# Zhongxu-Wang/ArtSpeech

Measured on AMD Instinct MI355X. Metric: mel frames/sec (whole job; per-GPU = value / n_gpus), acoustic-model inference path, batch 32 x 200-frame utterances, higher is better.
Workload: dtype f32 (f16x3 split-operand MFMA, fp32 accumulate)

## Files before the change

artspeech_amd/_lib.py:

```python
import ctypes
import os

import torch

_HERE = os.path.dirname(os.path.abspath(__file__))
LIB_PATH = os.environ.get("AS_LIB_PATH") or os.path.join(_HERE, "lib", "libartspeech_hip.so")
_lib = None

c_p = ctypes.c_void_p
c_i = ctypes.c_int
c_sz = ctypes.c_size_t
c_f = ctypes.c_float

_SIGNATURES = {
    "as_abi_version": (c_i, []),
    "as_device_status": (c_i, [c_i]),
    "as_device_status_raise_for_test": (c_i, [c_i, c_p]),
    "as_set_range_probe": (c_i, [c_i]),
    "as_prof_enable": (c_i, [c_i]),
    "as_prof_collect": (c_i, [c_p, c_p, c_p, c_p, c_i]),
    "as_prof_hint": (c_i, [ctypes.c_double, ctypes.c_double]),
    "as_prof_bracket_overhead": (c_i, [c_p, c_p]),
    "as_prof_mfma_sustained": (c_i, [c_p, c_p, c_p]),
    "as_mas_workspace_bytes": (c_sz, [c_i, c_i, c_i]),
    "as_mas_f32": (c_i, [c_p, c_p, c_p, c_i, c_i, c_i, c_i, c_p, c_p, c_p, c_p, c_sz, c_p]),
    "as_softmax_mas_f32": (c_i, [c_p, c_p, c_p, c_i, c_i, c_i, c_i, c_i, c_p, c_p, c_p, c_p, c_p, c_sz, c_p]),
}

AS_MAX_TAPS = 25
AS_ABI_VERSION = 10
AS_PROSODY_DIM, AS_PROSODY_TRACKS, AS_PROSODY_DUR, AS_PROSODY_GAIN, AS_PROSODY_OFFSET = 25, 12, 0, 1, 13


class ConvGemmArgs(ctypes.Structure):
    _fields_ = [("Wh", ctypes.c_void_p), ("W", ctypes.c_void_p), ("X", ctypes.c_void_p), ("Xh", ctypes.c_void_p), ("Y", ctypes.c_void_p),
                ("Yh", ctypes.c_void_p), ("bias", ctypes.c_void_p), ("res", ctypes.c_void_p), ("meta", ctypes.c_void_p),
                ("ws", ctypes.c_void_p), ("ws_bytes", ctypes.c_size_t),
                ("M", ctypes.c_int32), ("N", ctypes.c_int32), ("K", ctypes.c_int32), ("T", ctypes.c_int32),
                ("Kp", ctypes.c_int32),
                ("ldx", ctypes.c_int32), ("ldy", ctypes.c_int32), ("ldr", ctypes.c_int32),
                ("act", ctypes.c_int32), ("div_sqrt2", ctypes.c_int32), ("in_act", ctypes.c_int32),
                ("transpose_out", ctypes.c_int32), ("yh_lrelu", ctypes.c_int32), ("n_prod", ctypes.c_int32),
                ("dh", ctypes.c_int32 * AS_MAX_TAPS), ("dw", ctypes.c_int32 * AS_MAX_TAPS),
                ("in_slope", ctypes.c_float), ("act_slope", ctypes.c_float), ("acc_scale", ctypes.c_float),
                ("n_groups", ctypes.c_int32), ("group_cols", ctypes.c_int32), ("range_probe", ctypes.c_int32), ("status", ctypes.c_void_p),
                ("Xh2", ctypes.c_void_p), ("K2", ctypes.c_int32), ("src_col", ctypes.c_void_p), ("N_in", ctypes.c_int32), ("ileave_u", ctypes.c_int32),
                ("slab_tr", ctypes.c_int32), ("n_valid", ctypes.c_void_p)]


_SIGNATURES.update({
    "as_make_meta": (c_i, [c_p, c_p, c_i, c_i, c_i, c_p, c_p]),
    "as_conv_gemm_f32": (c_i, [ctypes.POINTER(ConvGemmArgs), c_p]),
    "as_conv_gemm_workspace_bytes": (c_sz, [ctypes.POINTER(ConvGemmArgs)]),
    "as_conv_gemm_multi_f32": (c_i, [ctypes.POINTER(ConvGemmArgs), c_i, c_p]),
    "as_conv_gemm_multi_tile": (c_i, [ctypes.POINTER(ConvGemmArgs), c_i]),
    "as_conv_gemm_multi_workspace_bytes": (c_sz, [ctypes.POINTER(ConvGemmArgs)]),
    "as_conv_gemm_plan": (c_i, [ctypes.POINTER(ConvGemmArgs), ctypes.POINTER(ctypes.c_int32), ctypes.POINTER(ctypes.c_int32),
                                ctypes.POINTER(ctypes.c_int32)]),
    "as_split_f16x2_bytes": (c_sz, [c_i, c_i]),
    "as_split_f16x2_f32": (c_i, [c_p, c_i, c_i, c_i, c_i, c_f, c_p, c_p]),
    "as_prep_weight_f16x2_bytes": (c_sz, [c_i, c_i, c_i, c_i]),
    "as_prep_weight_f16x2_host": (c_i, [c_p, c_i, c_i, c_i, c_i, c_p, c_p]),
    "as_prep_weight_f16x2_sc_bytes": (c_sz, [c_i, c_i, c_i, c_i, c_i]),
    "as_prep_weight_f16x2_sc_host": (c_i, [c_p, c_p, c_i, c_i, c_i, c_i, c_i, c_p, c_p]),
    "as_embed_groups_f32": (c_i, [c_p, c_i, c_p, c_p, c_i, c_i, c_i, c_i, c_f, c_p, c_i, c_p]),
    "as_channel_layernorm_groups_f32": (c_i, [c_p, c_i, c_i, c_i, c_p, c_p, c_p, c_p, c_i, c_f, c_i, c_p, c_i, c_p]),
    "as_channel_layernorm_split_f32": (c_i, [c_p, c_i, c_i, c_i, c_p, c_p, c_p, c_p, c_i, c_f, c_i, c_p, c_p]),
    "as_relpos_attention_groups_f32": (c_i, [c_p, c_i, c_i, c_i, c_i, c_p, c_p, c_p, c_p, c_i, c_p, c_i, c_i, c_p, c_i, c_p]),
    "as_embed_f32": (c_i, [c_p, c_p, c_i, c_i, c_i, c_f, c_p, c_i, c_p]),
    "as_channel_layernorm_f32": (c_i, [c_p, c_i, c_i, c_i, c_p, c_p, c_f, c_i, c_p, c_i, c_p]),
    "as_adain_f32": (c_i, [c_p, c_i, c_i, c_p, c_i, c_p, c_i, c_p, c_i, c_i, c_p, c_p, c_p, c_i, c_p]),
    "as_adain_split_f32": (c_i, [c_p, c_i, c_i, c_p, c_i, c_p, c_i, c_i, c_i, c_p, c_p]),
    "as_linear_rows_f32": (c_i, [c_p, c_i, c_p, c_p, c_i, c_i, c_i, c_p, c_i, c_p]),
    "as_durations_f32": (c_i, [c_p, c_p, c_p, c_i, c_p, c_p, c_p, c_i, c_p]),
    "as_expand_f32": (c_i, [c_p, c_i, c_i, c_p, c_i, c_i, c_p, c_i, c_p]),
    "as_ref_features_f32": (c_i, [c_p, c_i, c_i, c_p, c_p, c_i, c_i, c_p, c_p, c_i, c_p]),
    "as_crop_f32": (c_i, [c_p, c_i, c_p, c_i, c_p, c_i, c_p, c_i, c_i, c_i, c_p]),
    "as_rows_to_images_f32": (c_i, [c_p, c_i, c_p, c_i, c_i, c_p, c_p, c_i, c_i, c_p]),
    "as_stem_pool_image_f32": (c_i, [c_p, c_p, c_p, c_i, c_p, c_p, c_i, c_i, c_p, c_i, c_p, c_i, c_i, c_i, c_i, c_p, c_i, c_p]),
    "as_dwconv_down_f32": (c_i, [c_p, c_i, c_p, c_p, c_i, c_p, c_i, c_p, c_p, c_i, c_p, c_p, c_i, c_i, c_i, c_i, c_i, c_p]),
    "as_frame_signal_f32": (c_i, [c_p, c_p, c_p, c_i, c_i, c_i, c_i, c_p, c_i, c_p]),
    "as_spec_power_f32": (c_i, [c_p, c_i, c_i, c_i, c_p, c_i, c_p]),
    "as_log_norm_f32": (c_i, [c_p, c_i, c_i, c_i, c_f, c_f, c_f, c_p, c_i, c_p]),
    "as_xl_attention_f32": (c_i, [c_p, c_i, c_i, c_i, c_p, c_i, c_p, c_p, c_f, c_p, c_i, c_i, c_p, c_i, c_p]),
    "as_glu_dwconv_bn_swish_f32": (c_i, [c_p, c_i, c_i, c_p, c_i, c_p, c_p, c_p, c_i, c_p, c_i, c_p]),
    "as_lstm_step0_f32": (c_i, [c_p, c_i, c_i, c_i, c_p, c_i, c_p]),
    "as_bn_lrelu_maxpool_rows_f32": (c_i, [c_p, c_i, c_p, c_i, c_i, c_i, c_i, c_p, c_p, c_f, c_p, c_i, c_i, c_i, c_p]),
    "as_avgpool_down_f32": (c_i, [c_p, c_i, c_p, c_p, c_i, c_p, c_i, c_p, c_p, c_i, c_i, c_p, c_i, c_i, c_i, c_i, c_p]),
    "as_im2col_valid_f32": (c_i, [c_p, c_i, c_p, c_p, c_i, c_p, c_i, c_p, c_p, c_i, c_i, c_i, c_i, c_i, c_i, c_i, c_p]),
    "as_dwconv_down_image_f32": (c_i, [c_p, c_i, c_p, c_p, c_i, c_p, c_p, c_i, c_p, c_p, c_i, c_i, c_i, c_i, c_i, c_p, c_i, c_p]),
    "as_avgpool_down_image_f32": (c_i, [c_p, c_i, c_p, c_p, c_i, c_p, c_i, c_p, c_p, c_i, c_i, c_p, c_i, c_i, c_i, c_i, c_p, c_i, c_i, c_p]),
    "as_im2col_valid_image_f32": (c_i, [c_p, c_i, c_p, c_p, c_p, c_p, c_i, c_i, c_i, c_i, c_i, c_p, c_p]),
    "as_mean_pool_f32": (c_i, [c_p, c_i, c_p, c_i, c_i, c_i, c_p, c_i, c_p]),
    "as_relpos_attention_f32": (c_i, [c_p, c_i, c_i, c_i, c_i, c_p, c_p, c_p, c_i, c_i, c_p, c_i, c_p]),
    "as_relpos_attention_image_f32": (c_i, [c_p, c_i, c_p, c_i, c_i, c_i, c_i, c_p, c_p, c_p, c_p, c_i, c_p, c_i, c_i, c_p, c_i, c_p, c_p]),
    "as_relpos_attention_image_lds_bytes": (c_i, [c_i]),
    "as_bilstm_f32": (c_i, [c_p, c_i, c_p, c_i, c_i, c_p]),
    "as_bilstm_cluster_bytes": (ctypes.c_size_t, [c_i, c_i]),
    "as_bilstm_cluster_f32": (c_i, [c_p, c_i, c_p, c_i, c_i, c_i, c_p, ctypes.c_size_t, c_p]),
    "as_interleave_phases_f32": (c_i, [c_p, c_i, c_p, c_i, c_i, c_i, c_p, c_i, c_p]),
    "as_mean3_f32": (c_i, [c_p, c_p, c_p, c_i, c_i, c_i, c_p, c_i, c_p]),
})


class LnArgs(ctypes.Structure):
    _fields_ = [("gamma", c_p), ("beta", c_p), ("gamma2", c_p), ("beta2", c_p), ("n_split", ctypes.c_int32), ("eps", ctypes.c_float),
                ("relu", ctypes.c_int32), ("yh", c_p)]


class AdainArgs(ctypes.Structure):
    _fields_ = [("x", c_p), ("ldx", ctypes.c_int32), ("C", ctypes.c_int32), ("gb", c_p), ("gb_off", c_p), ("ldgb", ctypes.c_int32),
                ("gb_sc", ctypes.c_int32), ("col_off", c_p), ("src_off", c_p), ("U", ctypes.c_int32), ("N", ctypes.c_int32),
                ("lrelu", ctypes.c_int32), ("yh", c_p), ("pool_w", c_p), ("pool_b", c_p), ("x_up", c_p), ("ld_up", ctypes.c_int32),
                ("col_w", c_p)]


class DownArgs(ctypes.Structure):
    _fields_ = [("kind", ctypes.c_int32), ("x", c_p), ("ldx", ctypes.c_int32), ("in_off", c_p), ("in_w", c_p), ("Hin", ctypes.c_int32),
                ("y", c_p), ("ldy", ctypes.c_int32), ("out_off", c_p), ("out_w", c_p), ("Hout", ctypes.c_int32), ("w", c_p), ("bias", c_p),
                ("kh", ctypes.c_int32), ("pool_h", ctypes.c_int32), ("Kp", ctypes.c_int32), ("res", c_p), ("ldr", ctypes.c_int32),
                ("B", ctypes.c_int32), ("C", ctypes.c_int32), ("max_out", ctypes.c_int32), ("lrelu", ctypes.c_int32), ("yh", c_p),
                ("n_out", ctypes.c_int32)]


class ResPairArgs(ctypes.Structure):
    _fields_ = [("x", c_p), ("ldx", ctypes.c_int32), ("y", c_p), ("ldy", ctypes.c_int32), ("w1", c_p), ("w2", c_p), ("b1", c_p), ("b2", c_p),
                ("scale1", ctypes.c_float), ("scale2", ctypes.c_float), ("C", ctypes.c_int32), ("N", ctypes.c_int32), ("k", ctypes.c_int32),
                ("dil", ctypes.c_int32), ("slope", ctypes.c_float), ("col_off", c_p), ("B", ctypes.c_int32), ("max_w", ctypes.c_int32),
                ("add1", c_p), ("add2", c_p), ("ld_add", ctypes.c_int32), ("out_div", ctypes.c_float), ("yh", c_p), ("yh_slope", ctypes.c_float),
                ("x_u", ctypes.c_int32), ("x_bias", c_p)]


class ModelCfg(ctypes.Structure):
    _fields_ = [("hidden_dim", ctypes.c_int32), ("dim_in", ctypes.c_int32), ("style_dim", ctypes.c_int32), ("n_mels", ctypes.c_int32),
                ("n_token", ctypes.c_int32), ("reserved", ctypes.c_int32), ("stats", ctypes.c_float * 24)]


class Batch(ctypes.Structure):
    _fields_ = [("B", ctypes.c_int32), ("tok_lens", ctypes.POINTER(ctypes.c_int32)), ("ref_lens", ctypes.POINTER(ctypes.c_int32)),
                ("frames", ctypes.POINTER(ctypes.c_int32))]


class ForwardIO(ctypes.Structure):
    _fields_ = [("tokens", c_p), ("mel", c_p), ("ld_mel", ctypes.c_int32), ("f0_raw", c_p), ("ema_raw", c_p), ("ld_ema", ctypes.c_int32),
                ("forced_dur", c_p), ("mel_out", c_p), ("ld_out", ctypes.c_int32), ("duration", c_p), ("dur_i", c_p), ("frame_off", c_p),
                ("style", c_p), ("feat12", c_p), ("ld_feat", ctypes.c_int32), ("t_en", c_p), ("a_en", c_p), ("ld_en", ctypes.c_int32),
                ("F0", c_p), ("N", c_p), ("EMA", c_p), ("ld_pred", ctypes.c_int32), ("frame_cap", ctypes.c_int32), ("segs", c_p),
                ("voices", c_p), ("ld_voice", ctypes.c_int32), ("n_voices", ctypes.c_int32), ("voice_idx", c_p),
                ("prosody", c_p), ("ld_prosody", ctypes.c_int32)]


class HostIO(ctypes.Structure):
    _fields_ = [("tokens", c_p), ("mel", c_p), ("ld_mel", ctypes.c_int32), ("f0_raw", c_p), ("ema_raw", c_p), ("ld_ema", ctypes.c_int32),
                ("forced_dur", c_p), ("mel_out", c_p), ("ld_out", ctypes.c_int32), ("frame_cap", ctypes.c_int32), ("frame_off", c_p),
                ("voices", c_p), ("ld_voice", ctypes.c_int32), ("n_voices", ctypes.c_int32), ("voice_idx", c_p),
                ("prosody", c_p), ("ld_prosody", ctypes.c_int32)]


class TokenProsody(ctypes.Structure):
    _fields_ = [("rows", c_p), ("ld", ctypes.c_int32), ("smooth", ctypes.c_int32)]


(AS_MOD_FORWARD_A, AS_MOD_FORWARD_B, AS_MOD_ENCODER, AS_MOD_STYLE, AS_MOD_DURATION, AS_MOD_ARTS, AS_MOD_DECODER, AS_MOD_FORWARD_B_CAP,
 AS_MOD_VOICE, AS_MOD_FORWARD_A_VOICE) = range(10)
_pB, _pIO = ctypes.POINTER(Batch), ctypes.POINTER(ForwardIO)
_SIGNATURES.update({
    "as_adain_image_f32": (c_i, [ctypes.POINTER(AdainArgs), c_p]),
    "as_conv_gemm_multi_post_f32": (c_i, [ctypes.POINTER(ConvGemmArgs), ctypes.POINTER(AdainArgs), ctypes.POINTER(ctypes.c_int32),
                                          ctypes.POINTER(LnArgs), c_i, c_p]),
    "as_down_multi_f32": (c_i, [ctypes.POINTER(DownArgs), c_i, c_p]),
    "as_down_strip_rule": (c_i, [c_i, c_i, c_i, c_i, c_i, ctypes.POINTER(ctypes.c_int32), ctypes.POINTER(ctypes.c_int32)]),
    "as_respair_f32": (c_i, [ctypes.POINTER(ResPairArgs), c_p]),
    "as_xl_attention_image_f32": (c_i, [c_p, c_i, c_p, c_p, c_i, c_i, c_i, ctypes.c_float, c_p, c_i, c_i, c_p, c_i, c_p, c_p]),
    "as_mean3_image_f32": (c_i, [c_p, c_p, c_p, c_i, c_i, c_i, ctypes.c_float, c_p, c_p]),
    "as_conv_post_f32": (c_i, [c_p, c_i, c_i, c_i, c_p, c_p, c_i, ctypes.c_float, c_i, c_p, c_p, c_p]),
    "as_rows_image_f32": (c_i, [c_p, c_i, c_i, c_i, c_p, c_p]),
    "as_project_cols_f32": (c_i, [c_p, c_i, c_i, c_i, c_p, c_p, c_i, c_p, c_i, c_p]),
    "as_pointwise_small_f32": (c_i, [c_p, c_i, c_i, c_i, c_p, c_p, c_i, c_p, c_i, c_p, c_p, c_i, c_p, c_p]),
    "as_model_create": (c_i, [c_p, c_sz, ctypes.POINTER(ModelCfg), ctypes.POINTER(c_p)]),
    "as_model_destroy": (c_i, [c_p]),
    "as_plan_create": (c_i, [c_p, ctypes.POINTER(c_p)]),
    "as_plan_destroy": (c_i, [c_p]),
    "as_plan_set_serial": (c_i, [c_p, c_i]),
    "as_plan_set_merge": (c_i, [c_p, c_i]),
    "as_plan_set_timing": (c_i, [c_p, c_i]),
    "as_plan_set_operand_mode": (c_i, [c_p, c_i]),
    "as_plan_set_token_prosody": (c_i, [c_p, ctypes.POINTER(TokenProsody)]),
    "as_plan_phase_ms": (c_i, [c_p, ctypes.POINTER(ctypes.c_float), c_i]),
    "as_plan_set_layout_cap": (c_i, [c_p, c_i]),
    "as_plan_layout_flushes": (c_i, [c_p]),
    "as_plan_layout_count": (c_i, [c_p]),
    "as_plan_reset_layouts": (c_i, [c_p]),
    "as_bilstm_cluster_test_hooks": (c_i, [c_i, c_i]),
    "as_module_workspace_bytes": (c_sz, [c_p, c_p, c_i, _pB]),
    "as_encoder_forward": (c_i, [c_p, c_p, c_i, _pB, c_p, c_p, c_i, c_p, c_sz, c_p]),
    "as_style_forward": (c_i, [c_p, c_p, _pB, c_p, c_i, c_p, c_p, c_i, c_p, c_i, c_p, c_p, c_sz, c_p]),
    "as_duration_forward": (c_i, [c_p, c_p, _pB, c_p, c_p, c_i, c_p, c_p, c_sz, c_p]),
    "as_voice_dim": (c_i, [c_p]),
    "as_voice_forward": (c_i, [c_p, c_p, _pB, c_p, c_i, c_p, c_p, c_i, c_p, c_i, c_p, c_sz, c_p]),
    "as_arts_forward": (c_i, [c_p, c_p, _pB, c_p, c_i, c_p, c_p, c_p, c_p, c_i, c_p, c_sz, c_p]),
    "as_decoder_forward": (c_i, [c_p, c_p, _pB, c_p, c_i, c_p, c_p, c_p, c_p, c_i, c_p, c_i, c_p, c_sz, c_p]),
    "as_forward_test_begin": (c_i, [c_p, c_p, _pB, _pIO, c_p, c_sz, c_p]),
    "as_forward_test_finish": (c_i, [c_p, c_p, _pB, _pIO, c_p, c_sz, c_p, c_sz, c_p]),
    "as_forward_test": (c_i, [c_p, c_p, _pB, _pIO, c_p, c_sz, c_p, c_sz, ctypes.POINTER(ctypes.c_int32), c_p]),
    "as_lanes_create": (c_i, [c_p, c_i, ctypes.POINTER(c_p)]),
    "as_lanes_destroy": (c_i, [c_p]),
    "as_lanes_count": (c_i, [c_p]),
    "as_lanes_next": (c_i, [c_p]),
    "as_lanes_stream": (c_p, [c_p, c_i]),
    "as_lanes_submit": (c_i, [c_p, _pB, _pIO, ctypes.POINTER(ctypes.c_int32), ctypes.POINTER(ctypes.c_int32)]),
    "as_lanes_wait": (c_i, [c_p, c_i]),
    "as_lanes_set_coalesce": (c_i, [c_p, c_i]),
    "as_lanes_set_debug": (c_i, [c_p, c_i]),
    "as_lanes_submit_host": (c_i, [c_p, _pB, ctypes.POINTER(HostIO), ctypes.POINTER(ctypes.c_int32)]),
    "as_model_get_cfg": (c_i, [c_p, c_p]),
    "as_lanes_flush": (c_i, [c_p]),
    "as_lanes_merged_calls": (ctypes.c_int64, [c_p, c_i]),
    "as_lanes_set_graph_cap": (c_i, [c_p, c_i]),
    "as_lanes_set_layout_cap": (c_i, [c_p, c_i]),
    "as_lanes_reserve": (c_i, [c_p, c_sz, c_sz]),
    "as_lanes_stats": (c_i, [c_p, c_i, ctypes.POINTER(ctypes.c_int64)]),
})



class VocoderCfg(ctypes.Structure):
    _fields_ = [("num_mels", ctypes.c_int32), ("upsample_initial_channel", ctypes.c_int32), ("n_stages", ctypes.c_int32),
                ("upsample_rates", ctypes.c_int32 * 8), ("upsample_kernel_sizes", ctypes.c_int32 * 8), ("n_stacks", ctypes.c_int32),
                ("resblock_kernel_sizes", ctypes.c_int32 * 4), ("resblock_dilations", (ctypes.c_int32 * 4) * 4), ("n_dilations", ctypes.c_int32)]


class VocoderIO(ctypes.Structure):
    _fields_ = [("mel", c_p), ("ld_mel", ctypes.c_int32), ("wav", c_p), ("pcm", c_p)]


class VocoderCap(ctypes.Structure):
    _fields_ = [("off", c_p), ("mult", ctypes.c_int32), ("cap", ctypes.c_int32), ("max_len", ctypes.c_int32), ("sample_off", c_p)]


_pI32 = ctypes.POINTER(ctypes.c_int32)
_SIGNATURES.update({
    "as_vocoder_cap_workspace_bytes": (c_sz, [c_p, c_p, c_i, c_i, c_i]),
    "as_vocoder_forward_cap": (c_i, [c_p, c_p, c_i, ctypes.POINTER(VocoderCap), ctypes.POINTER(VocoderIO), c_p, c_sz, c_p]),
    "as_vocoder_cap_geometry": (c_i, [c_p, c_i, c_i, c_i, c_i, c_i, _pI32, c_p, c_p, c_p, c_p]),
    "as_split_f16x2_cap_f32": (c_i, [c_p, c_i, c_i, c_i, c_p, c_i, ctypes.c_float, c_p, c_p]),
    "as_mean3_cap_f32": (c_i, [c_p, c_p, c_p, c_i, c_i, c_i, c_p, c_p, c_i, c_p]),
    "as_mean3_image_cap_f32": (c_i, [c_p, c_p, c_p, c_i, c_i, c_i, c_p, ctypes.c_float, c_p, c_p]),
    "as_interleave_phases_cap_f32": (c_i, [c_p, c_i, c_p, c_i, c_i, c_i, c_p, c_p, c_i, c_p]),
    "as_conv_post_pcm_cap_f32": (c_i, [c_p, c_i, c_i, c_i, c_p, c_p, c_i, ctypes.c_float, c_i, c_p, c_p, c_p, c_p, c_p]),
    "as_conv_post_pcm_f32": (c_i, [c_p, c_i, c_i, c_i, c_p, c_p, c_i, ctypes.c_float, c_i, c_p, c_p, c_p, c_p]),
# ... 183 lines not shown
```

artspeech_amd/csrc/conv_gemm_h3.hip:

```cpp
#include "conv_gemm.h"
#include <cstring>
#include <type_traits>

typedef __attribute__((address_space(3))) void lds_void;

template <int I, int N, typename F>
static __device__ __forceinline__ void h3_for(F&& f)
{
    if constexpr (I < N) {
        f(std::integral_constant<int, I>{});
        h3_for<I + 1, N>(f);
    }
}

template <int WM, int WN, int WK, int KT, int NS, int NP, int TM = 2>
struct H3Cfg {
    static constexpr int QP = NP == 1 ? 2 : 4;
    static constexpr int BM = 32 * TM * WM, BN = 64 * WN;
    static constexpr int KBS = WK * KT;
    static constexpr int A_BLK = QP * BM * 16, B_BLK = QP * BN * 16;
    static constexpr int A_ST = KBS * A_BLK;
    static constexpr int STAGE = KBS * (A_BLK + B_BLK);
    static constexpr int RED = (WK - 1) * WM * WN * 32 * TM * 64 * 4;
    static constexpr int LDS = NS * STAGE > RED ? NS * STAGE : RED;
// ... 399 lines not shown
}

int as_split_f16x2_launch(const float* x, int ldx, int K, int N, int lrelu, float slope, uint16_t* xh, hipStream_t stream,
                          const int32_t* n_valid)
{
    if ((double)K * ldx * 4.0 >= 2147483648.0) return AS_EINVAL;
    hipLaunchKernelGGL(split_f16x2_kernel, dim3(as_cdiv(N + 1, 1024), 2 * as_kbx(K)), dim3(256), 0, stream, x, ldx, K, N, n_valid, lrelu, slope,
                       reinterpret_cast<u32x4_t*>(xh));
    AS_CHECK_LAUNCH();
    return AS_OK;
}

extern "C" int as_split_f16x2_f32(const float* x, int ldx, int K, int N, int in_act, float in_slope, uint16_t* xh, as_stream_t stream)
{
    return as_split_f16x2_cap_f32(x, ldx, K, N, nullptr, in_act, in_slope, xh, stream);
}

extern "C" int as_split_f16x2_cap_f32(const float* x, int ldx, int K, int N, const int32_t* n_valid, int in_act, float in_slope, uint16_t* xh,
                                      as_stream_t stream)
{
    if (!x || !xh || K <= 0 || N < 0 || ldx < N || (in_act != 0 && in_act != 2) || !(fabsf(in_slope) <= 3.0e38f)) return AS_EINVAL;
    if ((reinterpret_cast<uintptr_t>(xh) & 15) != 0) return AS_EINVAL;
    if (N == 0) return AS_OK;
    AsProfScope prof__(AS_CLS_OTHER, 0, 8.0 * K * (double)N, (hipStream_t)stream);
    return as_split_f16x2_launch(x, ldx, K, N, in_act == 2, in_slope, xh, (hipStream_t)stream, n_valid);
}

extern "C" size_t as_prep_weight_f16x2_sc_bytes(int G, int Cout, int Cin, int T, int Cin2)
{
    if (G <= 0 || Cout <= 0 || Cin <= 0 || T <= 0 || Cin2 < 0) return 0;
    return (size_t)G * ((size_t)T * as_kbx(Cin) + (Cin2 ? as_kbx(Cin2) : 0)) * 4 * (size_t)Cout * 16;
}
extern "C" size_t as_prep_weight_f16x2_bytes(int G, int Cout, int Cin, int T) { return as_prep_weight_f16x2_sc_bytes(G, Cout, Cin, T, 0); }

extern "C" int as_prep_weight_f16x2_sc_host(const float* w, const float* w2, int G, int Cout, int Cin, int T, int Cin2, uint16_t* wh,
                                            float* scale_out)
{
    if (!w || !wh || !scale_out || G <= 0 || Cout <= 0 || Cin <= 0 || T <= 0 || Cin2 < 0 || ((Cin2 > 0) != (w2 != nullptr))) return AS_EINVAL;
    const size_t n = (size_t)G * Cout * Cin * T, n2 = (size_t)G * Cout * Cin2;
    float mx = 0.f;
    for (size_t i = 0; i < n + n2; ++i) {
        const float x = i < n ? w[i] : w2[i - n];
        const float v = x < 0 ? -x : x;
        if (!(v <= 3.0e38f)) return AS_EINVAL;
        mx = v > mx ? v : mx;
    }
    int e = 0;
    float scale = 1.0f;
    if (mx > 0.f) {
        frexpf(mx, &e);
        scale = ldexpf(1.0f, 14 - e);
    }
    const int KBx = as_kbx(Cin), KBx2 = Cin2 ? as_kbx(Cin2) : 0;
    const size_t blocks = (size_t)T * KBx + KBx2;
    const size_t total = as_prep_weight_f16x2_sc_bytes(G, Cout, Cin, T, Cin2) / 2;
    for (size_t i = 0; i < total; ++i) wh[i] = 0;
    auto put = [&](size_t block, int k, int m, float x) {
        const _Float16 h = (_Float16)x;
        const _Float16 l = (_Float16)(x - (float)h);
        const int kh = (k >> 3) & 1, e8 = k & 7;
        const size_t base = block * 4 * (size_t)Cout * 8;
        uint16_t hb, lb;
        __builtin_memcpy(&hb, &h, 2);
        __builtin_memcpy(&lb, &l, 2);
        wh[base + ((size_t)(0 * 2 + kh) * Cout + m) * 8 + e8] = hb;
        wh[base + ((size_t)(1 * 2 + kh) * Cout + m) * 8 + e8] = lb;
    };
    for (int g = 0; g < G; ++g)
        for (int m = 0; m < Cout; ++m) {
            for (int k = 0; k < Cin; ++k)
                for (int t = 0; t < T; ++t) put((size_t)g * blocks + (size_t)t * KBx + (k >> 4), k, m, w[(((size_t)g * Cout + m) * Cin + k) * T + t] * scale);
            for (int k = 0; k < Cin2; ++k) put((size_t)g * blocks + (size_t)T * KBx + (k >> 4), k, m, w2[((size_t)g * Cout + m) * Cin2 + k] * scale);
        }
    *scale_out = scale;
    return AS_OK;
}
extern "C" int as_prep_weight_f16x2_host(const float* w, int G, int Cout, int Cin, int T, uint16_t* wh, float* scale_out)
{
    return as_prep_weight_f16x2_sc_host(w, nullptr, G, Cout, Cin, T, 0, wh, scale_out);
}

template <bool UP>
__global__ void __launch_bounds__(256)
adain_image_kernel(const AsAdainArgs a)
{
    const int lane = threadIdx.x & 63, wave = __builtin_amdgcn_readfirstlane(threadIdx.x >> 6);
    const int kb = blockIdx.x * 2 + (wave >> 1), kh = wave & 1, u = blockIdx.y;
    const int C = a.C;
    if (kb >= as_kbx(C)) return;
    const size_t NX = operand_image::rows(a.N);
    u32x4_t* xs = reinterpret_cast<u32x4_t*>(a.yh);
    const size_t plane = operand_image::row_of(kb, 0, kh, 0, NX);
    if (u == 0 && lane == 0) oi_zero_column(xs, plane, a.N, NX);
    const int o0 = a.col_off[u], L = a.col_w ? a.col_w[u] : a.col_off[u + 1] - o0;
    if (L <= 0) return;
    const int s0 = a.src_off ? a.src_off[u] : o0;
    const size_t gbase = a.gb_off ? (size_t)a.gb_off[u] : (size_t)u * a.ldgb;
    const int c0 = kb * 16 + kh * 8;
    float g1[8], bt[8], w0[8], w1[8], w2[8], pb[8];
#pragma unroll
    for (int r = 0; r < 8; ++r) {
        const int c = c0 + r < C ? c0 + r : C - 1;
        g1[r] = 1.0f + a.gb[gbase + (size_t)c * a.gb_sc];
        bt[r] = a.gb[gbase + (size_t)(C + c) * a.gb_sc];
        if (UP) { w0[r] = a.pool_w[c * 3 + 0]; w1[r] = a.pool_w[c * 3 + 1]; w2[r] = a.pool_w[c * 3 + 2]; pb[r] = a.pool_b[c]; }
    }
    const float* xr0 = a.x + s0;
    const size_t at0 = plane + (UP ? 2 * (size_t)o0 : (size_t)o0);
    float mean[8], rstd[8];
    auto resident = [&](auto rv_) {
        constexpr int RV = decltype(rv_)::value;
        float v[8][RV];
#pragma unroll
        for (int r = 0; r < 8; ++r) {
            const float* xr = xr0 + (size_t)(c0 + r < C ? c0 + r : C - 1) * a.ldx;
#pragma unroll
            for (int j = 0; j < RV; ++j) v[r][j] = xr[min(lane + 64 * j, L - 1)];
        }
#pragma unroll
        for (int r = 0; r < 8; ++r) {
            float sacc = 0.f;
#pragma unroll
            for (int j = 0; j < RV; ++j)
                if (lane + 64 * j < L) sacc += v[r][j];
            mean[r] = as_wave_sum(sacc) / (float)L;
        }
#pragma unroll
        for (int r = 0; r < 8; ++r) {
            float vacc = 0.f;
#pragma unroll
            for (int j = 0; j < RV; ++j)
                if (lane + 64 * j < L) { const float d = __fsub_rn(v[r][j], mean[r]); vacc = __fmaf_rn(d, d, vacc); }
            rstd[r] = 1.0f / sqrtf(as_wave_sum(vacc) / (float)L + 1e-5f);
        }
        if (UP && a.x_up) {
#pragma unroll
            for (int r = 0; r < 8; ++r) {
                if (c0 + r >= C) continue;
                float* ur = a.x_up + (size_t)(c0 + r) * a.ld_up + 2 * o0;
#pragma unroll
                for (int j = 0; j < RV; ++j) {
                    const int i = lane + 64 * j;
                    if (i < L) { ur[2 * i] = v[r][j]; ur[2 * i + 1] = v[r][j]; }
                }
            }
        }
#pragma unroll
        for (int r = 0; r < 8; ++r)
#pragma unroll
            for (int j = 0; j < RV; ++j)
                v[r][j] = (c0 + r < C && lane + 64 * j < L) ? as_adain_val(v[r][j], mean[r], rstd[r], g1[r], bt[r], a.lrelu) : 0.f;
#pragma unroll
        for (int j = 0; j < RV; ++j) {
            const int i = lane + 64 * j;
            if (64 * j >= L) break;
            if (!UP) {
                float t[8];
#pragma unroll
                for (int r = 0; r < 8; ++r) t[r] = v[r][j];
                u32x4_t h, l;
                split2(t, h, l);
                if (i < L) oi_store(xs, at0 + i, NX, h, l);
            } else {
                float e0[8], e1[8];
#pragma unroll
                for (int r = 0; r < 8; ++r) {
                    const float dn = __shfl_down(v[r][j], 1);
                    const float wr = j + 1 < RV ? __shfl(v[r][j + 1 < RV ? j + 1 : j], 0) : 0.f;
                    const float an = i + 1 < L ? (lane == 63 ? wr : dn) : 0.f;
                    float o0v, o1v;
                    as_convt_pair(v[r][j], an, w0[r], w1[r], w2[r], pb[r], &o0v, &o1v);
                    e0[r] = c0 + r < C ? o0v : 0.f;
                    e1[r] = c0 + r < C ? o1v : 0.f;
                }
                u32x4_t h, l, h2, l2;
                split2(e0, h, l);
                split2(e1, h2, l2);
                if (i < L) {
                    oi_store(xs, at0 + 2 * i, NX, h, l);
                    oi_store(xs, at0 + 2 * i + 1, NX, h2, l2);
                }
            }
        }
    };
    if (L <= 256) { resident(std::integral_constant<int, 4>{}); return; }
    if (L <= 512) { resident(std::integral_constant<int, 8>{}); return; }
    {
        size_t rowoff[8];
// ... 5 lines not shown
        int i = lane;
        for (; i + 192 < L; i += 256) {
            float t[4][8];
#pragma unroll
            for (int q = 0; q < 4; ++q)
#pragma unroll
                for (int r = 0; r < 8; ++r) t[q][r] = xr0[rowoff[r] + i + 64 * q];
#pragma unroll
            for (int q = 0; q < 4; ++q)
#pragma unroll
                for (int r = 0; r < 8; ++r) acc[r] += t[q][r];
        }
        for (; i < L; i += 64)
#pragma unroll
            for (int r = 0; r < 8; ++r) acc[r] += xr0[rowoff[r] + i];
#pragma unroll
        for (int r = 0; r < 8; ++r) { mean[r] = as_wave_sum(acc[r]) / (float)L; acc[r] = 0.f; }
        i = lane;
        for (; i + 192 < L; i += 256) {
            float t[4][8];
#pragma unroll
            for (int q = 0; q < 4; ++q)
#pragma unroll
                for (int r = 0; r < 8; ++r) t[q][r] = xr0[rowoff[r] + i + 64 * q];
#pragma unroll
            for (int q = 0; q < 4; ++q)
#pragma unroll
                for (int r = 0; r < 8; ++r) { const float d = __fsub_rn(t[q][r], mean[r]); acc[r] = __fmaf_rn(d, d, acc[r]); }
        }
        for (; i < L; i += 64)
#pragma unroll
            for (int r = 0; r < 8; ++r) { const float d = __fsub_rn(xr0[rowoff[r] + i], mean[r]); acc[r] = __fmaf_rn(d, d, acc[r]); }
#pragma unroll
        for (int r = 0; r < 8; ++r) rstd[r] = 1.0f / sqrtf(as_wave_sum(acc[r]) / (float)L + 1e-5f);
    }
    for (int i0 = lane; i0 < L; i0 += 128) {
        float xi[2][8], xn[2][8];
#pragma unroll
        for (int q = 0; q < 2; ++q) {
            const int i = min(i0 + 64 * q, L - 1);
#pragma unroll
            for (int r = 0; r < 8; ++r) {
                const float* xr = xr0 + (size_t)(c0 + r < C ? c0 + r : C - 1) * a.ldx;
                xi[q][r] = xr[i];
                if (UP) xn[q][r] = xr[min(i + 1, L - 1)];
            }
        }
#pragma unroll
        for (int q = 0; q < 2; ++q) {
            const int i = i0 + 64 * q;
            if (i >= L) break;
            float a0[8], a1[8];
#pragma unroll
            for (int r = 0; r < 8; ++r) {
                const bool ok = c0 + r < C;
                a0[r] = ok ? as_adain_val(xi[q][r], mean[r], rstd[r], g1[r], bt[r], a.lrelu) : 0.f;
                a1[r] = (UP && ok && i + 1 < L) ? as_adain_val(xn[q][r], mean[r], rstd[r], g1[r], bt[r], a.lrelu) : 0.f;
                if (UP && a.x_up && ok) {
                    float* ur = a.x_up + (size_t)(c0 + r) * a.ld_up + 2 * o0 + 2 * i;
                    ur[0] = xi[q][r];
                    ur[1] = xi[q][r];
                }
            }
            u32x4_t h, l;
            if (!UP) {
                split2(a0, h, l);
                oi_store(xs, at0 + i, NX, h, l);
            } else {
                float e0[8], e1[8];
#pragma unroll
                for (int r = 0; r < 8; ++r) {
                    as_convt_pair(a0[r], a1[r], w0[r], w1[r], w2[r], pb[r], &e0[r], &e1[r]);
                    if (c0 + r >= C) { e0[r] = 0.f; e1[r] = 0.f; }
                }
                split2(e0, h, l);
                oi_store(xs, at0 + 2 * i, NX, h, l);
                split2(e1, h, l);
                oi_store(xs, at0 + 2 * i + 1, NX, h, l);
            }
        }
    }
}

extern "C" int as_adain_image_f32(const AsAdainArgs* args_host, as_stream_t stream)
{
    if (!args_host) return AS_EINVAL;
    const AsAdainArgs& a = *args_host;
    if (!a.x || !a.gb || !a.col_off || !a.yh || a.C <= 0 || a.U <= 0 || a.N < 0 || a.gb_sc <= 0 || (!a.gb_off && a.ldgb <= 0)) return AS_EINVAL;
    if ((a.pool_w == nullptr) != (a.pool_b == nullptr) || (a.x_up && !a.pool_w)) return AS_EINVAL;
    if ((reinterpret_cast<uintptr_t>(a.yh) & 15) != 0) return AS_EINVAL;
    if (a.N == 0) return AS_OK;
    AsProfScope prof__(AS_CLS_ADAIN, 0, 8.0 * a.C * (double)a.N, (hipStream_t)stream);
    if (a.pool_w) hipLaunchKernelGGL(adain_image_kernel<true>, dim3(as_kbx(a.C) / 2, a.U), dim3(256), 0, (hipStream_t)stream, a);
    else hipLaunchKernelGGL(adain_image_kernel<false>, dim3(as_kbx(a.C) / 2, a.U), dim3(256), 0, (hipStream_t)stream, a);
    AS_CHECK_LAUNCH();
    return AS_OK;
}

extern "C" int as_adain_split_f32(const float* x, int ldx, int C, const float* gamma_beta, int ldgb, const int32_t* col_off, int B,
                                  int N, int lrelu, uint16_t* xs, as_stream_t stream)
{
    if (!x || !gamma_beta || !col_off || !xs || C <= 0 || B <= 0 || N < 0 || ldgb < 2 * C) return AS_EINVAL;
    AsAdainArgs a = {};
    a.x = x; a.ldx = ldx; a.C = C; a.gb = gamma_beta; a.ldgb = ldgb; a.gb_sc = 1; a.col_off = col_off; a.U = B; a.N = N; a.lrelu = lrelu; a.yh = xs;
    return as_adain_image_f32(&a, stream);
}

__global__ void __launch_bounds__(256)
rows_image_kernel(const float* __restrict__ x, int ldx, int K, int B, u32x4_t* __restrict__ xh)
{
    const int i = blockIdx.x * 256 + threadIdx.x;
    const int groups = 2 * as_kbx(K);
    if (i >= groups * (B + 1)) return;
    const int g = i / (B + 1), b = i % (B + 1);
    float t[8];
#pragma unroll
    for (int r = 0; r < 8; ++r) t[r] = (b < B && g * 8 + r < K) ? x[(size_t)b * ldx + g * 8 + r] : 0.f;
    u32x4_t h, l;
    split2(t, h, l);
    const size_t NX = operand_image::rows(B);
    oi_store(xh, operand_image::row(g, 0, b, NX), NX, h, l);
}

extern "C" int as_rows_image_f32(const float* x, int ldx, int K, int B, uint16_t* xh, as_stream_t stream)
{
    if (!x || !xh || K <= 0 || B <= 0 || ldx < K || (reinterpret_cast<uintptr_t>(xh) & 15) != 0) return AS_EINVAL;
    AsProfScope prof__(AS_CLS_OTHER, 0, 8.0 * K * (double)B, (hipStream_t)stream);
    hipLaunchKernelGGL(rows_image_kernel, dim3(as_cdiv((long)2 * as_kbx(K) * (B + 1), 256)), dim3(256), 0, (hipStream_t)stream, x, ldx, K, B,
                       reinterpret_cast<u32x4_t*>(xh));
    AS_CHECK_LAUNCH();
    return AS_OK;
}

#define LNS_COLS 32
#define LNS_PARTS 32
#define LNS_MAXG 4
__global__ void __launch_bounds__(1024)
channel_ln_split_kernel(const float* __restrict__ x, int ldx, int C, int N, const float* __restrict__ gamma1,
                        const float* __restrict__ beta1, const float* __restrict__ gamma2, const float* __restrict__ beta2, int n_split,
                        float eps, int relu, u32x4_t* __restrict__ xs, int KBx)
{
    __shared__ float red[LNS_PARTS][LNS_COLS + 1];
    const int col = threadIdx.x % LNS_COLS, part = threadIdx.x / LNS_COLS;
    const int j = blockIdx.x * LNS_COLS + col;
    const bool ok = j < N;
    const int grp = gamma2 ? j / n_split : 0;
    const float* gamma = gamma1 + (ptrdiff_t)grp * (gamma2 - gamma1);
    const float* beta = beta1 + (ptrdiff_t)grp * (beta2 - beta1);
    const int ngroups = 2 * KBx;
    float v[LNS_MAXG][8];
    float s = 0.f;
#pragma unroll
    for (int i = 0; i < LNS_MAXG; ++i)
#pragma unroll
        for (int r = 0; r < 8; ++r) {
            const int c = 8 * (part + i * LNS_PARTS) + r;
            v[i][r] = (ok && c < C) ? x[(size_t)c * ldx + j] : 0.f;
            s += v[i][r];
        }
    red[part][col] = s;
    __syncthreads();
    float tot = 0.f;
#pragma unroll
    for (int q = 0; q < LNS_PARTS; ++q) tot += red[q][col];
    const float mean = tot / (float)C;
    __syncthreads();
    float q2 = 0.f;
#pragma unroll
    for (int i = 0; i < LNS_MAXG; ++i)
#pragma unroll
        for (int r = 0; r < 8; ++r) {
            const int c = 8 * (part + i * LNS_PARTS) + r;
            const float d = __fsub_rn(v[i][r], mean);
            if (c < C) q2 = __fmaf_rn(d, d, q2);
        }
    red[part][col] = q2;
    __syncthreads();
    tot = 0.f;
#pragma unroll
// ... 48 lines not shown
```

artspeech_amd/csrc/elementwise.hip:

```cpp
#include "common.h"
#include <algorithm>
#include <cstring>
#include "artspeech_hip.h"
#include "conv_gemm.h"
#include "down_strips.h"
#include <cstdint>
#include <type_traits>
#define AS_FILE_CLS AS_CLS_OTHER

static __device__ __forceinline__ float lrelu02(float v) { return v > 0.f ? v : 0.2f * v; }

__global__ void make_meta_kernel(const int* __restrict__ widths, const int* __restrict__ col_off, int B, int H,
                                 unsigned long long* __restrict__ meta, unsigned* __restrict__ status)
{
    const int b = blockIdx.y;
    const int W = widths[b];
    const int base = col_off[b];
    if (W > AS_META_MAX_W) {
        if (blockIdx.x == 0 && threadIdx.x == 0) as_status_raise(status, AS_STATUS_BAD_LAYOUT);
        return;
    }
    for (int i = blockIdx.x * blockDim.x + threadIdx.x; i < H * W; i += gridDim.x * blockDim.x) {
        const unsigned long long h = i / W, w = i - (i / W) * W;
        meta[base + i] = AS_META_PACK(h, w, H, W);
    }
}

extern "C" int as_make_meta(const int32_t* widths, const int32_t* col_off, int B, int H, int n_cols_max,
                            uint64_t* meta, as_stream_t stream)
{
    if (!widths || !col_off || !meta || B < 0 || H <= 0 || H > AS_META_MAX_H) return AS_EINVAL;
    if (B == 0) return AS_OK;
    const int gx = n_cols_max > 0 ? as_cdiv(as_cdiv(n_cols_max, B > 0 ? B : 1), 256) : 1;
    AsProfScope prof__(AS_FILE_CLS, 0, 0, (hipStream_t)stream);
    hipLaunchKernelGGL(make_meta_kernel, dim3(gx < 1 ? 1 : (gx > 64 ? 64 : gx), B), dim3(256), 0, (hipStream_t)stream,
                       widths, col_off, B, H, reinterpret_cast<unsigned long long*>(meta), as_status_words_device());
    AS_CHECK_LAUNCH();
    return AS_OK;
}

__global__ void embed_kernel(const int* __restrict__ tok, int n_tok, const float* __restrict__ emb, const float* __restrict__ emb2,
                             int n_split, int C, int N, int V, float scale, float* __restrict__ y, int ldy, unsigned* __restrict__ status)
{
    const int j = blockIdx.x * blockDim.x + threadIdx.x;
    const int c = blockIdx.y;
    if (j >= N) return;
    const int g = emb2 ? j / n_split : 0;
    const int src = j - g * n_split;
    int t = src < n_tok ? tok[src] : 0;
    if ((t < 0 || t >= V) && c == 0) as_status_raise(status, AS_STATUS_BAD_TOKEN);
    t = t < 0 ? 0 : (t >= V ? V - 1 : t);
    const float* e = emb + (ptrdiff_t)g * (emb2 - emb);
    y[(size_t)c * ldy + j] = e[(size_t)t * C + c] * scale;
}

extern "C" int as_embed_groups_f32(const int32_t* tokens, int n_tok, const float* emb, const float* emb2, int n_split, int C, int N, int V,
                                   float scale, float* y, int ldy, as_stream_t stream)
{
    if (!tokens || !emb || !y || C <= 0 || N < 0 || V <= 0 || ldy < N || n_tok < 0 || n_tok > N) return AS_EINVAL;
    if ((emb2 && n_split <= 0) || (n_tok < N && (!emb2 || n_split < n_tok))) return AS_EINVAL;
    if (N == 0) return AS_OK;
    AsProfScope prof__(AS_FILE_CLS, 0, 0, (hipStream_t)stream);
    hipLaunchKernelGGL(embed_kernel, dim3(as_cdiv(N, 64), C), dim3(64), 0, (hipStream_t)stream, tokens, n_tok, emb, emb2, n_split, C, N, V,
                       scale, y, ldy, as_status_words_device());
    AS_CHECK_LAUNCH();
    return AS_OK;
}

extern "C" int as_embed_f32(const int32_t* tokens, const float* emb, int C, int N, int V, float scale, float* y,
                            int ldy, as_stream_t stream)
{
    return as_embed_groups_f32(tokens, N, emb, nullptr, 0, C, N, V, scale, y, ldy, stream);
}

#define LN_COLS 32
#define LN_PARTS 32
#define LN_MAXV 16
__global__ void __launch_bounds__(1024)
channel_ln_kernel(const float* __restrict__ x, int ldx, int C, int N, const float* __restrict__ gamma1,
                  const float* __restrict__ beta1, const float* __restrict__ gamma2, const float* __restrict__ beta2, int n_split,
                  float eps, int relu, float* __restrict__ y, int ldy)
{
    __shared__ float red[LN_PARTS][LN_COLS + 1];
    const int col = threadIdx.x % LN_COLS, part = threadIdx.x / LN_COLS;
    const int j = blockIdx.x * LN_COLS + col;
    const bool ok = j < N;
    const int grp = gamma2 ? j / n_split : 0;
    const float* gamma = gamma1 + (ptrdiff_t)grp * (gamma2 - gamma1);
    const float* beta = beta1 + (ptrdiff_t)grp * (beta2 - beta1);
    float v[LN_MAXV];
    float s = 0.f;
#pragma unroll
    for (int i = 0; i < LN_MAXV; ++i) {
        const int c = part + i * LN_PARTS;
        v[i] = (ok && c < C) ? x[(size_t)c * ldx + j] : 0.f;
        s += v[i];
    }
    for (int c = part + LN_MAXV * LN_PARTS; c < C; c += LN_PARTS) s += ok ? x[(size_t)c * ldx + j] : 0.f;
    red[part][col] = s;
    __syncthreads();
    float tot = 0.f;
#pragma unroll
    for (int q = 0; q < LN_PARTS; ++q) tot += red[q][col];
    const float mean = tot / (float)C;
    __syncthreads();
    float q2 = 0.f;
#pragma unroll
    for (int i = 0; i < LN_MAXV; ++i) {
        const int c = part + i * LN_PARTS;
        const float d = v[i] - mean;
        if (c < C) q2 += d * d;
    }
    for (int c = part + LN_MAXV * LN_PARTS; c < C; c += LN_PARTS) {
        const float d = (ok ? x[(size_t)c * ldx + j] : 0.f) - mean;
        q2 += d * d;
    }
    red[part][col] = q2;
    __syncthreads();
    tot = 0.f;
#pragma unroll
    for (int q = 0; q < LN_PARTS; ++q) tot += red[q][col];
    const float rs = 1.0f / sqrtf(tot / (float)C + eps);
    if (!ok) return;
#pragma unroll
    for (int i = 0; i < LN_MAXV; ++i) {
        const int c = part + i * LN_PARTS;
        if (c < C) {
            float o = (v[i] - mean) * rs * gamma[c] + beta[c];
            if (relu) o = o < 0.f ? 0.f : o;
            y[(size_t)c * ldy + j] = o;
        }
    }
    for (int c = part + LN_MAXV * LN_PARTS; c < C; c += LN_PARTS) {
        float o = (x[(size_t)c * ldx + j] - mean) * rs * gamma[c] + beta[c];
        if (relu) o = o < 0.f ? 0.f : o;
        y[(size_t)c * ldy + j] = o;
    }
}

extern "C" int as_channel_layernorm_groups_f32(const float* x, int ldx, int C, int N, const float* gamma, const float* beta,
                                               const float* gamma2, const float* beta2, int n_split, float eps, int relu, float* y,
                                               int ldy, as_stream_t stream)
{
    if (!x || !y || !gamma || !beta || C <= 0 || N < 0 || ldx < N || ldy < N || ((gamma2 == nullptr) != (beta2 == nullptr)) ||
        (gamma2 && n_split <= 0))
        return AS_EINVAL;
    if (N == 0) return AS_OK;
    AsProfScope prof__(AS_CLS_LN, 8.0 * C * N, 8.0 * C * N, (hipStream_t)stream);
    hipLaunchKernelGGL(channel_ln_kernel, dim3(as_cdiv(N, LN_COLS)), dim3(1024), 0, (hipStream_t)stream, x, ldx, C, N, gamma,
// ... 300 lines not shown
            else h = mid - 1;
        }
        ub = l;
    }
    int local = 0;
    for (int i = lo; i < hi; ++i) {
        int d;
        if (forced) d = forced[i];
        else {
            float v = dur_f[i];
            if (pros) {
                while (ub + 1 < B && tok_off[ub + 1] <= i) ++ub;
                v = v * pros[(size_t)ub * ldr + AS_PROSODY_DUR];
            }
            const bool fin = fabsf(v) <= 3.0e38f;
            if (!fin) as_status_raise(status, AS_STATUS_F16_RANGE);
            const float r = fin ? rintf(v) : 1.f;
            d = (int)(r < 1.f ? 1.f : fminf(r, 16384.f));
        }
        dur_i[i] = d;
        local += d;
    }
    sums[t] = local;
    __syncthreads();
    for (int off = 1; off < 1024; off <<= 1) {
        const int v = t >= off ? sums[t - off] : 0;
        __syncthreads();
        sums[t] += v;
        __syncthreads();
    }
    int f = sums[t] - local;
    if (t == 0) frame_off[B] = sums[1023];
    int b = 0;
    if (lo < hi || ntok == 0) {
        for (b = 0; b < B; ++b) {
            const int first = tok_off[b];
            if (first >= lo && first < hi) {
                int fb = f;
                for (int i = lo; i < first; ++i) fb += dur_i[i];
                frame_off[b] = fb;
            }
        }
    }
    if (t == 0)
        for (b = 0; b < B; ++b)
            if (tok_off[b] >= ntok) frame_off[b] = sums[1023];
    if (!tok_of_frame) return;
    for (int i = lo; i < hi; ++i) {
        const int d = dur_i[i];
        for (int r = 0; r < d; ++r, ++f)
            if (f < max_frames) tok_of_frame[f] = i;
    }
}

int as_durations_prosody_launch(const float* dur_f32, const int32_t* forced_dur, const int32_t* tok_off, int B, const float* pros, int ld_pros,
                                int32_t* dur_i32, int32_t* frame_off, int32_t* tok_of_frame, int max_frames, hipStream_t stream)
{
    if ((!dur_f32 && !forced_dur) || !tok_off || !dur_i32 || !frame_off || B < 0 || B > 1024) return AS_EINVAL;
    if (pros && (forced_dur || B < 1 || ld_pros < AS_PROSODY_DIM)) return AS_EINVAL;
    AsProfScope prof__(AS_FILE_CLS, 0, 0, stream);
    hipLaunchKernelGGL(durations_kernel, dim3(1), dim3(1024), 0, stream, dur_f32, forced_dur, tok_off, B,
                       dur_i32, frame_off, tok_of_frame, max_frames, as_status_words_device(), pros, ld_pros);
    AS_CHECK_LAUNCH();
    return AS_OK;
}

extern "C" int as_durations_f32(const float* dur_f32, const int32_t* forced_dur, const int32_t* tok_off, int B,
                                int32_t* dur_i32, int32_t* frame_off, int32_t* tok_of_frame, int max_frames,
                                as_stream_t stream)
{
    return as_durations_prosody_launch(dur_f32, forced_dur, tok_off, B, nullptr, 0, dur_i32, frame_off, tok_of_frame, max_frames,
                                       (hipStream_t)stream);
}

__global__ void expand_kernel(const float* __restrict__ x, int ldx, int C, const int* __restrict__ tok_of_frame,
                              int n_frames, int rep, float* __restrict__ y, int ldy)
{
    const int j = blockIdx.x * blockDim.x + threadIdx.x;
    const int c = blockIdx.y;
    if (j >= n_frames * rep) return;
    y[(size_t)c * ldy + j] = x[(size_t)c * ldx + tok_of_frame[j / rep]];
}

extern "C" int as_expand_f32(const float* x, int ldx, int C, const int32_t* tok_of_frame, int n_frames, int repeat,
                             float* y, int ldy, as_stream_t stream)
{
    if (!x || !y || !tok_of_frame || C <= 0 || n_frames < 0 || repeat < 1 || ldy < n_frames * repeat) return AS_EINVAL;
    if (n_frames == 0) return AS_OK;
    AsProfScope prof__(AS_FILE_CLS, 0, 0, (hipStream_t)stream);
    hipLaunchKernelGGL(expand_kernel, dim3(as_cdiv((long)n_frames * repeat, 256), C), dim3(256), 0, (hipStream_t)stream,
                       x, ldx, C, tok_of_frame, n_frames, repeat, y, ldy);
    AS_CHECK_LAUNCH();
    return AS_OK;
}

__global__ void __launch_bounds__(256)
ref_features_kernel(const float* __restrict__ mel, int ldm, int n_mels, const float* __restrict__ f0_raw,
                    const float* __restrict__ ema_raw, int lde, int N, const float* __restrict__ stats,
                    float* __restrict__ feat, int ldf)
{
    __shared__ float part[8][32];
    const int col = threadIdx.x & 31, sl = threadIdx.x >> 5;
    const int j = blockIdx.x * 32 + col;
    const int jc = j < N ? j : N - 1;
    constexpr int RMAX = 16;
    float v[RMAX];
#pragma unroll
    for (int r = 0; r < RMAX; ++r) {
        const int m = sl + 8 * r;
        v[r] = mel[(size_t)(m < n_mels ? m : 0) * ldm + jc];
    }
    float ss = 0.f;
#pragma unroll
    for (int r = 0; r < RMAX; ++r) {
        if (sl + 8 * r < n_mels) {
            const float e = expf(v[r] * 4.0f + -4.0f);
            ss += e * e;
        }
    }
    for (int m = sl + 8 * RMAX; m < n_mels; m += 8) {
        const float e = expf(mel[(size_t)m * ldm + jc] * 4.0f + -4.0f);
        ss += e * e;
    }
    part[sl][col] = ss;
    __syncthreads();
    if (j >= N) return;
    if (sl == 0) {
        float tot = 0.f;
#pragma unroll
        for (int q = 0; q < 8; ++q) tot += part[q][col];
        feat[j] = (logf(sqrtf(tot)) - stats[0]) / stats[1];
    } else if (sl == 1) {
        feat[(size_t)ldf + j] = (f0_raw[j] - stats[2]) / stats[3];
    } else {
        for (int c = sl - 2; c < 10; c += 6) feat[(size_t)(2 + c) * ldf + j] = (ema_raw[(size_t)c * lde + j] - stats[4 + c]) / stats[14 + c];
    }
}

extern "C" int as_ref_features_f32(const float* mel, int ldm, int n_mels, const float* f0_raw, const float* ema_raw,
                                   int lde, int N, const float* stats24, float* feat, int ldf, as_stream_t stream)
{
    if (!mel || !f0_raw || !ema_raw || !stats24 || !feat || N < 0 || n_mels <= 0 || ldm < N || lde < N || ldf < N) return AS_EINVAL;
    if (N == 0) return AS_OK;
    AsProfScope prof__(AS_FILE_CLS, 0, 0, (hipStream_t)stream);
    hipLaunchKernelGGL(ref_features_kernel, dim3(as_cdiv(N, 32)), dim3(256), 0, (hipStream_t)stream, mel, ldm, n_mels,
                       f0_raw, ema_raw, lde, N, stats24, feat, ldf);
    AS_CHECK_LAUNCH();
    return AS_OK;
}

__global__ void crop_kernel(const float* __restrict__ src, int lds, const int* __restrict__ src_off, int start,
                            float* __restrict__ dst, int ldd, const int* __restrict__ dst_off, int C)
{
    const int b = blockIdx.y, c = blockIdx.z;
    const int L = dst_off[b + 1] - dst_off[b];
    for (int i = blockIdx.x * blockDim.x + threadIdx.x; i < L; i += gridDim.x * blockDim.x)
        dst[(size_t)c * ldd + dst_off[b] + i] = src[(size_t)c * lds + src_off[b] + start + i];
}

extern "C" int as_crop_f32(const float* src, int lds, const int32_t* src_off, int start, float* dst, int ldd,
                           const int32_t* dst_off, int B, int C, int max_len, as_stream_t stream)
{
    if (!src || !dst || !src_off || !dst_off || B < 0 || C <= 0) return AS_EINVAL;
    if (B == 0 || max_len <= 0) return AS_OK;
    AsProfScope prof__(AS_FILE_CLS, 0, 0, (hipStream_t)stream);
    hipLaunchKernelGGL(crop_kernel, dim3(as_cdiv(max_len, 256), B, C), dim3(256), 0, (hipStream_t)stream, src, lds,
                       src_off, start, dst, ldd, dst_off, C);
    AS_CHECK_LAUNCH();
    return AS_OK;
}

__global__ void rows_to_images_kernel(const float* __restrict__ src, int lds, const int* __restrict__ src_off, int start,
                                      float* __restrict__ dst, const int* __restrict__ img_off, int H)
{
    const int b = blockIdx.y, h = blockIdx.z;
    const int Wb = (img_off[b + 1] - img_off[b]) / H;
    for (int i = blockIdx.x * blockDim.x + threadIdx.x; i < Wb; i += gridDim.x * blockDim.x)
        dst[(size_t)img_off[b] + (size_t)h * Wb + i] = src[(size_t)h * lds + src_off[b] + start + i];
}

extern "C" int as_rows_to_images_f32(const float* src, int lds, const int32_t* src_off, int start, int H, float* dst,
                                     const int32_t* img_off, int B, int max_w, as_stream_t stream)
{
    if (!src || !dst || !src_off || !img_off || B < 0 || H <= 0) return AS_EINVAL;
    if (B == 0 || max_w <= 0) return AS_OK;
    AsProfScope prof__(AS_FILE_CLS, 0, 0, (hipStream_t)stream);
    hipLaunchKernelGGL(rows_to_images_kernel, dim3(as_cdiv(max_w, 256), B, H), dim3(256), 0, (hipStream_t)stream, src, lds,
                       src_off, start, dst, img_off, H);
    AS_CHECK_LAUNCH();
    return AS_OK;
}

__global__ void bn_lrelu_maxpool_rows_kernel(const float* __restrict__ x, int ldx, const int* __restrict__ tok_off, int H, int k,
                                             const float* __restrict__ scale, const float* __restrict__ shift, float slope,
                                             float* __restrict__ y, int ldy, int to_channels)
{
    const int b = blockIdx.y, c = blockIdx.z;
    const int t0 = tok_off[b], Wb = tok_off[b + 1] - t0, Hout = H / k;
    const float* xr = x + (size_t)c * ldx + (size_t)H * t0;
    const float sc = scale[c], sh = shift[c];
    for (int i = blockIdx.x * blockDim.x + threadIdx.x; i < Hout * Wb; i += gridDim.x * blockDim.x) {
        const int ho = i / Wb, w = i - ho * Wb;
        float m = -INFINITY;
        for (int r = 0; r < k; ++r) {
            float v = xr[(size_t)(ho * k + r) * Wb + w] * sc + sh;
            v = v > 0.f ? v : slope * v;
            m = fmaxf(m, v);
        }
        if (to_channels) y[(size_t)(c * Hout + ho) * ldy + t0 + w] = m;
        else y[(size_t)c * ldy + (size_t)Hout * t0 + i] = m;
    }
}

extern "C" int as_bn_lrelu_maxpool_rows_f32(const float* x, int ldx, const int32_t* tok_off, int B, int C, int H, int k,
                                            const float* scale, const float* shift, float slope, float* y, int ldy,
                                            int to_channels, int total_frames, as_stream_t stream)
{
    if (!x || !y || !tok_off || !scale || !shift || B < 0 || C <= 0 || H <= 0 || k <= 0 || k > H) return AS_EINVAL;
    if (B == 0 || total_frames <= 0) return AS_OK;
    AsProfScope prof__(AS_FILE_CLS, 0, 4.0 * C * (double)total_frames * (H + H / k), (hipStream_t)stream);
    const int per_utt = as_cdiv((long)(H / k) * total_frames, B);
    int gx = as_cdiv(per_utt, 256);
    gx = gx < 1 ? 1 : gx > 64 ? 64 : gx;
    hipLaunchKernelGGL(bn_lrelu_maxpool_rows_kernel, dim3(gx, B, C), dim3(256), 0, (hipStream_t)stream, x, ldx, tok_off, H, k, scale,
                       shift, slope, y, ldy, to_channels);
    AS_CHECK_LAUNCH();
    return AS_OK;
}

typedef float f32x2u __attribute__((ext_vector_type(2), aligned(4)));

struct DownWalk {
    int i, ho, wo, Wo, dq, dr, end, last_row;
    __device__ __forceinline__ DownWalk(int r0, int r1, int Wo_) : Wo(Wo_)
    {
        const int q = (int)threadIdx.x / Wo;
        ho = r0 + q; wo = (int)threadIdx.x - q * Wo; i = r0 * Wo + (int)threadIdx.x;
        end = r1 * Wo; last_row = r1 - 1;
        dq = 256 / Wo; dr = 256 - dq * Wo;
    }
    __device__ __forceinline__ void step()
    {
        i += 256; ho += dq; wo += dr;
        if (wo >= Wo) { wo -= Wo; ++ho; }
    }
    __device__ __forceinline__ bool live() const { return i < end; }
    __device__ __forceinline__ int row() const { return live() ? ho : last_row; }
    __device__ __forceinline__ int col() const { return live() ? wo : Wo - 1; }
    __device__ __forceinline__ int trips(int r0) const
    {
        const int first = r0 * Wo + (__builtin_amdgcn_readfirstlane((int)threadIdx.x) & ~63);
        return max(0, (end - first + 255) >> 8);
    }
};

static __device__ __forceinline__ void down_zero_column(u32x4_t* __restrict__ yh, size_t plane, size_t NX, int Nout, int b, int strip)
{
    if (yh && b == 0 && strip == 0 && threadIdx.x < 2) oi_zero_column(yh, plane, (size_t)threadIdx.x, Nout, NX);
}

template <class Pos, class Half, class Where, class Load, class Sums, class Put>
static __device__ __forceinline__ void down_walk_halves(DownWalk& wk, int r0, const Where& where, const Load& load, const Sums& sums, const Put& put)
{
    int n = wk.trips(r0);
    if (n <= 0) return;
    Pos p, pn;
    Half d0, d1;
    where(p);
    pn = p;
    load(d0, p, 0);
    const auto trip = [&](auto last) __attribute__((always_inline)) {
// ... 511 lines not shown
    if (!x || !col || !in_off || !in_w || !out_off || !out_w || K <= 0 || stride <= 0 || B < 0 || C <= 0) return AS_EINVAL;
    if (B == 0 || max_out <= 0) return AS_OK;
    AsProfScope prof__(AS_FILE_CLS, 0, 0, (hipStream_t)stream);
    hipLaunchKernelGGL(im2col_valid_kernel, dim3(C * K * K), dim3(256), 0, (hipStream_t)stream, x, ldx, in_off, in_w, Hin, col,
                       ldc, out_off, out_w, Hout, K, stride, lrelu, B);
    AS_CHECK_LAUNCH();
    return AS_OK;
}

__global__ void __launch_bounds__(256)
im2col_valid_image_kernel(const float* __restrict__ x, int ldx, const int* __restrict__ in_off, const int* __restrict__ in_w,
                          const int* __restrict__ out_off, const int* __restrict__ out_w, int K, int stride, int act, int B, int rows,
                          u32x4_t* __restrict__ yh)
{
    const int g = blockIdx.x;
    const int total = out_off[B];
    const size_t NX = operand_image::rows(total), plane = operand_image::row(g, 0, 0, NX);
    if (threadIdx.x < 2) oi_zero_column(yh, plane, (size_t)threadIdx.x, total, NX);
    for (int j = threadIdx.x; j < total; j += blockDim.x) {
        int b = 0;
        while (b + 1 < B && out_off[b + 1] <= j) ++b;
        const int i = j - out_off[b], Wo = out_w[b], Wi = in_w[b];
        const int ho = i / Wo, wo = i - ho * Wo;
        float t[8];
#pragma unroll
        for (int r = 0; r < 8; ++r) {
            const int ck = g * 8 + r;
            float v = 0.f;
            if (ck < rows) {
                const int c = ck / (K * K), a = (ck / K) % K, d = ck % K;
                v = x[(size_t)c * ldx + in_off[b] + (size_t)(ho * stride + a) * Wi + wo * stride + d];
                if (act) v = lrelu02(v);
            }
            t[r] = v;
        }
        oi_store(yh, plane + j, NX, t);
    }
}

extern "C" int as_im2col_valid_image_f32(const float* x, int ldx, const int32_t* in_off, const int32_t* in_w, const int32_t* out_off,
                                         const int32_t* out_w, int K, int stride, int lrelu, int B, int C, uint16_t* yh, as_stream_t stream)
{
    if (!x || !yh || !in_off || !in_w || !out_off || !out_w || K <= 0 || stride <= 0 || B <= 0 || C <= 0 ||
        (reinterpret_cast<uintptr_t>(yh) & 15) != 0)
        return AS_EINVAL;
    AsProfScope prof__(AS_FILE_CLS, 0, 0, (hipStream_t)stream);
    hipLaunchKernelGGL(im2col_valid_image_kernel, dim3(2 * as_kbx(C * K * K)), dim3(256), 0, (hipStream_t)stream, x, ldx, in_off, in_w, out_off,
                       out_w, K, stride, lrelu, B, C * K * K, reinterpret_cast<u32x4_t*>(yh));
    AS_CHECK_LAUNCH();
    return AS_OK;
}

__global__ void __launch_bounds__(256)
mean_pool_kernel(const float* __restrict__ x, int ldx, const int* __restrict__ col_off, int B, int C, int act,
                 float* __restrict__ y, int ldy)
{
    const int lane = threadIdx.x & 63;
    const int row = blockIdx.x * 4 + (threadIdx.x >> 6);
    if (row >= C * B) return;
    const int c = row / B, b = row - c * B;
    const int o0 = col_off[b], L = col_off[b + 1] - o0;
    float s = 0.f;
    for (int i = lane; i < L; i += 64) {
        float v = x[(size_t)c * ldx + o0 + i];
        if (act) v = lrelu02(v);
        s += v;
    }
    s = as_wave_sum(s);
    if (lane == 0) y[(size_t)b * ldy + c] = s / (float)L;
}

extern "C" int as_mean_pool_f32(const float* x, int ldx, const int32_t* col_off, int B, int C, int lrelu, float* y,
                                int ldy, as_stream_t stream)
{
    if (!x || !y || !col_off || B < 0 || C <= 0 || ldy < C) return AS_EINVAL;
    if (B == 0) return AS_OK;
    AsProfScope prof__(AS_FILE_CLS, 0, 0, (hipStream_t)stream);
    hipLaunchKernelGGL(mean_pool_kernel, dim3(as_cdiv((long)C * B, 4)), dim3(256), 0, (hipStream_t)stream, x, ldx, col_off,
                       B, C, lrelu, y, ldy);
    AS_CHECK_LAUNCH();
    return AS_OK;
}

__global__ void __launch_bounds__(256)
dyn_geometry_kernel(const AsDynGeo g)
{
    const int z = blockIdx.z, b = blockIdx.y, B = g.B, cap1 = g.cap1;
    const int total_raw = g.frame_off[B];
    if (z == 8) {
        if (b == 0) {
            if (g.tof)
                for (int f = max(total_raw, 0) + (int)(blockIdx.x * blockDim.x + threadIdx.x); f < cap1; f += gridDim.x * blockDim.x) g.tof[f] = 0;
            if (blockIdx.x == 0 && threadIdx.x == 0 && total_raw > cap1) as_status_raise(g.status, AS_STATUS_CAPACITY);
        }
        if (blockIdx.x == 0 && threadIdx.x == 0) {
            int s = 0;
            while (s + 1 < g.n_seg && b >= g.seg_first[s + 1]) ++s;
            const int first = g.seg_first[s], o_first = min(g.frame_off[first], cap1);
            int32_t* fo = g.seg_frame_off[s];
            if (fo) fo[b - first] = min(g.frame_off[b], cap1) - o_first;
            if (b + 1 == g.seg_first[s + 1]) {
                const int len = min(g.frame_off[b + 1], cap1) - o_first;
                if (fo) fo[b + 1 - first] = len;
                if (len > g.seg_cap[s]) as_status_raise(g.status, AS_STATUS_CAPACITY);
            }
        }
        return;
    }
    const int li = z == 0 ? 0 : (z == 1 ? 1 : (z < 5 ? 2 : 3));
    const int grp = z < 2 ? 0 : (z < 5 ? z - 2 : z - 5);
    const int sc = (li == 1 || li == 3) ? 2 : 1;
    const int o = min(g.frame_off[b], cap1), e = min(g.frame_off[b + 1], cap1);
    const int W = sc * (e - o), base = grp * sc * cap1 + sc * o, u = grp * B + b;
    if (blockIdx.x == 0 && threadIdx.x == 0) {
        if (g.w[li]) g.w[li][u] = W;
        if (g.off[li]) {
            g.off[li][u] = base;
            if (b == B - 1 && (li < 2 || grp == 2)) g.off[li][u + 1] = base + W;
        }
        if (li == 2 && g.src3) g.src3[u] = o;
        if (b == 0 && grp == 0 && g.nvalid[li]) *g.nvalid[li] = sc * min(max(total_raw, 0), cap1);
    }
    unsigned long long* meta = g.meta[li];
    if (!meta) return;
    for (int i = blockIdx.x * blockDim.x + threadIdx.x; i < W; i += gridDim.x * blockDim.x)
        meta[base + i] = AS_META_PACK(0ull, (unsigned long long)i, 1ull, (unsigned long long)W);
}

int as_dyn_geometry_launch(const AsDynGeo& g, hipStream_t stream)
{
    if (!g.frame_off || g.B < 1 || g.B > 1024 || g.cap1 < 1 || g.n_seg < 1 || g.n_seg > 16) return AS_EINVAL;
    AsProfScope prof__(AS_FILE_CLS, 0, 0, stream);
    const int gx = std::min(64, std::max(1, as_cdiv(as_cdiv(2L * g.cap1, g.B), 256)));
    hipLaunchKernelGGL(dyn_geometry_kernel, dim3(gx, g.B, 9), dim3(256), 0, stream, g);
    AS_CHECK_LAUNCH();
    return AS_OK;
}

__global__ void __launch_bounds__(256)
seg_scatter_kernel(const AsSegScatter a)
{
    const int s = blockIdx.z, r = blockIdx.y;
    const int first = a.seg_first[s], last = a.seg_first[s + 1];
    const int o = 2 * a.frame_off[first], n = min(2 * (a.frame_off[last] - a.frame_off[first]), 2 * a.seg_cap[s]);
    const float* src = a.src + (size_t)r * a.ld_src + o;
    float* dst = a.dst[s] + (size_t)r * a.ld_dst[s];
    for (int i = blockIdx.x * blockDim.x + threadIdx.x; i < n; i += gridDim.x * blockDim.x) dst[i] = src[i];
}

int as_seg_scatter_launch(const AsSegScatter& a, hipStream_t stream)
{
    if (!a.src || !a.frame_off || a.rows < 1 || a.n_seg < 1 || a.n_seg > 16) return AS_EINVAL;
    AsProfScope prof__(AS_FILE_CLS, 0, 0, stream);
    int cap = 1;
    for (int s = 0; s < a.n_seg; ++s) cap = std::max(cap, 2 * a.seg_cap[s]);
    hipLaunchKernelGGL(seg_scatter_kernel, dim3(std::min(64, as_cdiv(cap, 256)), a.rows, a.n_seg), dim3(256), 0, stream, a);
    AS_CHECK_LAUNCH();
    return AS_OK;
}
```

artspeech_amd/csrc/model.hip:

```cpp
#include "common.h"
#include "conv_gemm.h"
#include "play_order.h"
#include "runtime.h"
#include <algorithm>
#include <climits>
#include <cmath>
#include <cstdint>
#include <cstdio>
#include <cstring>
#include <functional>
#include <map>
#include <memory>
#include <new>
#include <string>
#include <unordered_map>
#include <vector>

using namespace asrt;

namespace {

constexpr int N_HEADS = 4;
constexpr int WINDOW = 4;
constexpr int ACT_NONE = 0, ACT_RELU = 1, ACT_LRELU = 2;
// ... 786 lines not shown
    ConvOpt q1;
    q1.bias = m.bias_stack(sfx(".conv1"));
    q1.group_cols = gc2;
    q1.post_n = &o.n2; q1.post_lay = lay2; q1.post_yh = xs2;
    conv_h_new(c, w1, xs, din, lay2, k3, q1);
    if (has_sc && !fold) {
        ConvOpt q;
        q.group_cols = gc2;
        float* dst = out;
        const int ldd = ldo;
        const GemmW* wsc = m.conv_stack(sfx(".conv1x1"));
        if (X.h && !o.upsample) conv_h(c, wsc, X.h, din, lay2, k1, dst, ldd, q);
        else conv_x(c, wsc, sc, ldsc, din, lay2, k1, dst, ldd, q);
        sc = dst;
        ldsc = ldd;
    }
    ConvOpt q2;
    q2.bias = m.bias_stack(sfx(".conv2"));
    if (fold) {
        q2.x2h = X.h;
        q2.K2 = din;
    } else {
        q2.res = sc;
        q2.ldr = ldsc;
    }
    q2.div_sqrt2 = true;
    q2.group_cols = gc2;
    if (o.want_yh) {
        q2.want_yh = true;
        q2.yh = o.yh ? o.yh : c.image(dout, N2);
    }
    if (o.next_n1) {
        q2.post_n = o.next_n1; q2.post_lay = lay2;
        q2.post_yh = c.image(dout, N2);
    }
    conv_h(c, w2, xs2, dout, lay2, k3, out, ldo, q2);
    Y.p = out; Y.C = dout; Y.ld = ldo; Y.lay = lay2; Y.h = q2.yh; Y.pre = q2.post_yh;
    return Y;
}

struct EncSpec {
    std::string prefix;
    int layers;
};
struct EncOut {
    float* y[4] = {nullptr, nullptr, nullptr, nullptr};
    int ld[4] = {0, 0, 0, 0};
};
template <class Done>
bool rel_encoder_multi(Ctx& c, const std::vector<EncSpec>& enc, const int32_t* tokens, const Lay* lay1, EncOut* out, Done&& done)
{
    const as_model& m = c.m;
    const int G = (int)enc.size();
    if (G < 1 || G > 4 || !lay1) { c.fail(AS_EINVAL); return false; }
    for (int g = 1; g < G; ++g)
        if (enc[g].layers > enc[g - 1].layers) { c.fail(AS_EINVAL); return false; }
    const HostT* emb_h = m.host(enc[0].prefix + ".emb.weight");
    if (!emb_h) { c.fail(AS_EINVAL); return false; }
    const int V = emb_h->dim(0), C = emb_h->dim(1), N1 = lay1->N;
    const int pad = G > 1 ? (128 - N1 % 128) % 128 : 0, gc = N1 + pad, bg = lay1->B + (pad ? 1 : 0);
    std::vector<const Lay*> lays(G + 1, nullptr);
    {
        std::vector<int> w;
        for (int k = 1; k <= G; ++k) {
            if (k > 1 && pad) w.push_back(pad);
            w.insert(w.end(), lay1->w.begin(), lay1->w.end());
            lays[k] = c.lay(w);
            if (!lays[k]) return false;
        }
    }
    const int ld = std::max(lays[G]->N, 1);
    auto names = [&](const std::string& sfx, int k) {
        std::vector<std::string> n;
        for (int g = 0; g < k; ++g) n.push_back(enc[g].prefix + sfx);
        return n;
    };
    auto stack2 = [&](const std::string& sfx, int k, const float** second) {
        const HostT* h0 = m.host(enc[0].prefix + sfx);
        const float* s0 = m.vec_stack(names(sfx, k));
        *second = (k > 1 && s0 && h0) ? s0 + h0->v.size() : nullptr;
        return s0;
    };
    float* x = c.f32((size_t)C * ld);
    {
        const float* e2 = nullptr;
        const float* e1 = stack2(".emb.weight", G, &e2);
        if (lays[G]->N > 0) RUN(c, as_embed_groups_f32(tokens, N1, e1, e2, gc, C, lays[G]->N, V, sqrtf((float)C), x, ld, c.s));
    }
    auto ln_image = [&](const float* xin, const std::string& ln, bool relu, int k) {
        const int N = lays[k]->N;
        uint16_t* xs = c.image(C, N);
        const float *g2 = nullptr, *b2 = nullptr;
        const float *g1 = stack2(ln + ".gamma", k, &g2), *b1 = stack2(ln + ".beta", k, &b2);
        if (N > 0) RUN(c, as_channel_layernorm_split_f32(xin, ld, C, N, g1, b1, g2, b2, gc, 1e-4f, relu, xs, c.s));
        return xs;
    };
    auto ln_post = [&](ConvOpt& q, const std::string& ln, bool relu, int k) {
        const int N = lays[k]->N;
        uint16_t* xs = c.image(C, N);
        const float *g2 = nullptr, *b2 = nullptr;
        const float *g1 = stack2(ln + ".gamma", k, &g2), *b1 = stack2(ln + ".beta", k, &b2);
        q.ln.gamma = g1; q.ln.beta = b1; q.ln.gamma2 = g2; q.ln.beta2 = b2; q.ln.n_split = gc; q.ln.eps = 1e-4f; q.ln.relu = relu ? 1 : 0;
        q.ln.yh = N > 0 ? xs : nullptr;
        return xs;
    };
    auto cw = [&](const std::string& name, int k) { return m.conv_stack(names(name, k)); };
    auto cb = [&](const std::string& name, int k) { return m.bias_stack(names(name, k)); };
    auto opt = [&](const std::string& bias_of, int k) {
        ConvOpt o;
        o.bias = cb(bias_of, k);
        o.group_cols = k > 1 ? gc : 0;
        return o;
    };
    const Taps k5 = taps_1d(5), k1 = taps_1d(1), k9 = taps_1d(9);
    float* h = c.f32((size_t)C * ld);
    const std::string e = ".encoder";
    uint16_t* xs_next = nullptr;
    {
        ConvOpt q0 = opt(".pre.conv_layers.0", G);
        xs_next = ln_post(q0, ".pre.norm_layers.0", true, G);
        conv_x(c, cw(".pre.conv_layers.0", G), x, ld, C, lays[G], k5, h, ld, q0);
        for (int i = 0; i < 3; ++i) {
            uint16_t* xs = xs_next;
            const std::string nxt = i < 2 ? ".pre.conv_layers." + std::to_string(i + 1) : std::string(".pre.proj");
            ConvOpt q = opt(nxt, G);
            if (i == 2) { q.res = x; q.ldr = ld; }
            xs_next = i < 2 ? ln_post(q, ".pre.norm_layers." + std::to_string(i + 1), true, G)
                            : (enc[0].layers > 0 ? ln_post(q, e + ".norm_layers_1.0", false, G) : nullptr);
            float* hn = c.f32((size_t)C * ld);
            conv_h(c, cw(nxt, G), xs, C, lays[G], i < 2 ? k5 : k1, hn, ld, q);
            h = hn;
        }
    }
    x = h;
    auto finish = [&](int g0, int g1) {
        const int Nk = (g1 - g0 - 1) * gc + N1;
        float* y = c.f32((size_t)C * std::max(Nk, 1));
        std::vector<std::string> ng, nb;
        for (int g = g0; g < g1; ++g) { ng.push_back(enc[g].prefix + e + ".last_ln.gamma"); nb.push_back(enc[g].prefix + e + ".last_ln.beta"); }
        const float *lg = m.vec_stack(ng), *lb = m.vec_stack(nb);
        const float *lg2 = g1 - g0 > 1 && lg ? lg + C : nullptr, *lb2 = g1 - g0 > 1 && lb ? lb + C : nullptr;
        if (Nk > 0) RUN(c, as_channel_layernorm_groups_f32(x + (size_t)g0 * gc, ld, C, Nk, lg, lb, lg2, lb2, gc, 1e-4f, 0, y, Nk, c.s));
        for (int g = g0; g < g1; ++g) {
            out->y[g] = y + (size_t)(g - g0) * gc;
            out->ld[g] = std::max(Nk, 1);
        }
        for (int g = g0; g < g1; ++g) done(g);
    };
    int k = G;
    int xs_k = G;
    for (int i = 0; i < enc[0].layers; ++i) {
        int kn = 0;
        while (kn < G && enc[kn].layers > i) ++kn;
        if (kn < k) { finish(kn, k); k = kn; }
        const Lay* lay = lays[k];
        const int N = lay->N;
        const std::string a = e + ".attn_layers." + std::to_string(i), f = e + ".ffn_layers." + std::to_string(i);
        const float* bqkv = nullptr;
        const GemmW* wqkv = m.qkv(names(a, k), &bqkv);
        ConvOpt o;
        o.bias = bqkv;
        o.group_cols = k > 1 ? gc : 0;
        const bool img = C / N_HEADS == 128;
        if (img) {
            o.want_yh = true;
            o.yh = c.image(3 * C, N);
        }
        uint16_t* xs1 = (xs_next && xs_k == k) ? xs_next : ln_image(x, e + ".norm_layers_1." + std::to_string(i), false, k);
        xs_next = nullptr;
        float* qkv = conv_h_new(c, wqkv, xs1, C, lay, k1, o);
        float* att = img ? nullptr : c.f32((size_t)C * std::max(N, 1));
        uint16_t* att_h = img ? c.image(C, N) : nullptr;
        const float *ek2 = nullptr, *ev2 = nullptr;
        const float *ek = stack2(a + ".emb_rel_k", k, &ek2), *ev = stack2(a + ".emb_rel_v", k, &ev2);
        if (N > 0 && img)
            RUN(c, as_relpos_attention_image_f32(qkv, N, o.yh, N, C, N_HEADS, WINDOW, ek, ev, ek2, ev2, bg, lay->d_off, lay->B, lay->max_w, nullptr,
                                                 0, att_h, c.s));
        else if (N > 0)
            RUN(c, as_relpos_attention_groups_f32(qkv, N, C, N_HEADS, WINDOW, ek, ev, ek2, ev2, bg, lay->d_off, lay->B, lay->max_w, att, N, c.s));
        ConvOpt oo = opt(a + ".conv_o", k);
        oo.res = x;
        oo.ldr = ld;
        uint16_t* xs2 = ln_post(oo, e + ".norm_layers_2." + std::to_string(i), false, k);
        float* xo = c.f32((size_t)C * ld);
        if (img) conv_h(c, cw(a + ".conv_o", k), att_h, C, lay, k1, xo, ld, oo);
        else conv_x(c, cw(a + ".conv_o", k), att, N, C, lay, k1, xo, ld, oo);
        x = xo;
        const GemmW* w1 = cw(f + ".conv_1", k);
        if (!w1) { c.fail(AS_EINVAL); return false; }
        uint16_t* yh = c.image(w1->M, N);
        ConvOpt o1 = opt(f + ".conv_1", k);
        o1.act = ACT_RELU;
        o1.want_yh = true;
        o1.yh = yh;
        conv_h(c, w1, xs2, C, lay, k9, nullptr, N, o1);
        ConvOpt o2 = opt(f + ".conv_2", k);
        o2.res = x;
        o2.ldr = ld;
        {
            int kn2 = 0;
            while (kn2 < G && enc[kn2].layers > i + 1) ++kn2;
            if (i + 1 < enc[0].layers && kn2 == k) { xs_next = ln_post(o2, e + ".norm_layers_1." + std::to_string(i + 1), false, k); xs_k = k; }
        }
        float* xf = c.f32((size_t)C * ld);
// ... 84 lines not shown
    } else {
        float* r3 = conv_h_new(c, w2, r2h, cin, lay2, taps, o2);
        out = c.f32((size_t)w2->M * N2);
        c.hint(0, 4.0 * cin * ((double)lay->N + (want_image ? 3.0 : 2.0) * lay2->N));
        {
            AsDownArgs a = down_args(1, X.p, X.ld, lay, lay2, cin);
            a.y = out; a.ldy = lay2->N; a.pool_h = half ? 2 : 1; a.res = r3; a.ldr = lay2->N;
            if (want_image) { a.yh = outh; a.lrelu = 1; }
            down(c, a, __LINE__);
        }
    }
    Y.p = out; Y.C = w2->M; Y.ld = lay2->N; Y.lay = lay2; Y.h = outh;
    return Y;
}

Act tower_stem(Ctx& c, const std::string& name, const float* X, int ldx, const Lay* lay, const Taps& taps, bool image_only)
{
    Act x;
    const GemmW* w0 = c.m.conv(name);
    if (!w0 || !lay) { c.fail(AS_EINVAL); return x; }
    ConvOpt o;
    o.bias = c.m.bias(name);
    o.want_yh = true;
    o.yh = c.image(w0->M, lay->N);
    o.yh_lrelu = true;
    if (image_only && w0->K == 1 && w0->w32 && (taps.n == 9 || taps.n == 3)) {
        conv_x(c, w0, X, ldx, w0->K, lay, taps, nullptr, lay->N, o);
        x.stem_x = X; x.stem_w = w0; x.stem_b = o.bias; x.stem_kh = taps.n == 9 ? 3 : 1;
    } else {
        x.p = conv_x_new(c, w0, X, ldx, w0->K, lay, taps, o);
    }
    x.C = w0->M; x.ld = lay->N; x.lay = lay; x.h = o.yh;
    return x;
}

void tower2d(Ctx& c, const std::string& p, const float* X, const Lay* lay, const std::vector<bool>& halves, int last_idx, int last_stride,
             const std::string& linear, float* y, int ldy)
{
    const as_model& m = c.m;
    if (!lay) { c.fail(AS_EINVAL); return; }
    Act x = tower_stem(c, p + ".0", X, lay->N, lay, taps_2d(3, 3), m.has(p + ".1.conv1x1.weight"));
    if (!x.lay) return;
    for (size_t i = 0; i < halves.size(); ++i) {
        x = resblk_down(c, p + "." + std::to_string(i + 1), x, halves[i], false, true);
        if (!x.lay) return;
    }
    const int K = 5, C = x.C;
    const Lay* lout = c.valid_conv(x.lay, K, last_stride);
    if (!lout) return;
    if (lout->H < 1 || *std::min_element(lout->w.begin(), lout->w.end()) < 1) {
        c.fail(AS_EINVAL);
        return;
    }
    const std::string ln = p + "." + std::to_string(last_idx);
    const GemmW* wl = m.conv(ln);
    if (!wl || wl->T != K * K || wl->K != C) { c.fail(AS_EINVAL); return; }
    const Lay* lin = x.lay;
    std::string key = "valid:" + std::to_string(K) + ":" + std::to_string(last_stride) + ":" + std::to_string(lin->H);
    for (int v : lin->w) key += ":" + std::to_string(v);
    const int32_t* tab = c.itable(lout, key, [&]() {
        std::vector<int32_t> t((size_t)lout->N * 3 + 1, 0);
        const size_t mo = ((size_t)lout->N + 1) & ~(size_t)1;
        for (int b = 0, j = 0; b < lout->B; ++b)
            for (int ho = 0; ho < lout->H; ++ho)
                for (int wo = 0; wo < lout->w[b]; ++wo, ++j) {
                    const int h = ho * last_stride, w = wo * last_stride;
                    t[j] = lin->off[b] + h * lin->w[b] + w;
                    const uint64_t md = AS_META_PACK(h, w, lin->H, lin->w[b]);
                    memcpy(&t[mo + 2 * (size_t)j], &md, 8);
                }
        return t;
    });
    ConvOpt o2;
    o2.bias = m.bias(ln);
    o2.act = ACT_LRELU;
    o2.src_col = tab;
    o2.src_meta = tab ? reinterpret_cast<const uint64_t*>(tab + (((size_t)lout->N + 1) & ~(size_t)1)) : nullptr;
    o2.N_in = lin->N;
    Taps tv;
    tv.n = K * K;
    for (int a = 0; a < K; ++a)
        for (int d = 0; d < K; ++d) { tv.dh[a * K + d] = a; tv.dw[a * K + d] = d; }
    float* z = conv_h_new(c, wl, x.h, C, lout, tv, o2);
    float* pooled = c.f32((size_t)lay->B * wl->M);
    RUN(c, as_mean_pool_f32(z, lout->N, lout->d_off, lay->B, wl->M, 0, pooled, wl->M, c.s));
    const HostT* lw = m.host(linear + ".weight");
    if (!lw) return;
    const float *lww = m.vec(linear + ".weight"), *lwb = m.vec(linear + ".bias");
    RUN(c, as_linear_rows_f32(pooled, wl->M, lww, lwb, lay->B, lw->dim(0), lw->dim(1), y, ldy, c.s));
}

void tower1d(Ctx& c, const std::string& p, const float* X, int ldx, const Lay* lay, const std::string& linear, float* y, int ldy)
{
    const as_model& m = c.m;
    if (!lay) { c.fail(AS_EINVAL); return; }
    Act x = tower_stem(c, p + ".0", X, ldx, lay, taps_1d(3), m.has(p + ".1.conv1x1.weight"));
    if (!x.lay) return;
    for (int i = 1; i <= 4; ++i) {
        x = resblk_down(c, p + "." + std::to_string(i), x, false, true, i < 4);
        if (!x.lay) return;
    }
    float* pooled = c.f32((size_t)lay->B * x.C);
    RUN(c, as_mean_pool_f32(x.p, x.ld, x.lay->d_off, lay->B, x.C, 1, pooled, x.C, c.s));
    const HostT* lw = m.host(linear + ".weight");
    if (!lw) return;
    const float *lww = m.vec(linear + ".weight"), *lwb = m.vec(linear + ".bias");
    RUN(c, as_linear_rows_f32(pooled, x.C, lww, lwb, lay->B, lw->dim(0), lw->dim(1), y, ldy, c.s));
}

struct StyleIn {
    float* crop = nullptr;
    const Lay *l1 = nullptr, *lm = nullptr, *le = nullptr;
    float *mel_img = nullptr, *ema_img = nullptr;
};

StyleIn style_inputs(Ctx& c, const float* feat12, int ldf, const float* mel, int ldm, const Lay* ref)
{
    StyleIn s;
    const int n_mels = c.m.cfg.n_mels;
    std::vector<int> w(ref->w);
    for (int& v : w) v = v > 0 ? v - 1 : 0;
    s.l1 = c.lay(w);
    s.lm = c.lay(w, n_mels);
    s.le = c.lay(w, 10);
    if (!s.l1 || !s.lm || !s.le) return s;
    const int N1 = std::max(s.l1->N, 1);
    s.crop = c.f32((size_t)2 * N1);
    RUN(c, as_crop_f32(feat12, ldf, ref->d_off, 0, s.crop, s.l1->N, s.l1->d_off, ref->B, 2, s.l1->max_cols(), c.s));
    s.mel_img = c.f32((size_t)std::max(s.lm->N, 1));
    s.ema_img = c.f32((size_t)std::max(s.le->N, 1));
    RUN(c, as_rows_to_images_f32(mel, ldm, ref->d_off, 0, n_mels, s.mel_img, s.lm->d_off, ref->B, s.l1->max_cols(), c.s));
    RUN(c, as_rows_to_images_f32(feat12 + (size_t)2 * ldf, ldf, ref->d_off, 0, 10, s.ema_img, s.le->d_off, ref->B, s.l1->max_cols(), c.s));
    return s;
}

StyleIn ref_style_inputs(Ctx& c, const float* mel, int ldm, const float* f0_raw, const float* ema_raw, int lde, float* feat12, int ldf,
                         const Lay* ref)
{
    const float* stats = c.m.vec("__stats24");
    const int n_mels = c.m.cfg.n_mels;
    RUN(c, as_ref_features_f32(mel, ldm, n_mels, f0_raw, ema_raw, lde, ref->N, stats, feat12, ldf, c.s));
    return style_inputs(c, feat12, ldf, mel, ldm, ref);
}

void style_tower(Ctx& c, int which, const StyleIn& s, float* style, int lds = 0)
{
    const std::string p = "style_encoder";
    const int sd = c.m.cfg.style_dim;
    if (lds <= 0) lds = 2 * sd;
    if (which == 0) tower2d(c, p + ".Mel_block", s.mel_img, s.lm, {true, true, true, true}, 6, 1, p + ".Mellinear", style, lds);
    else if (which == 1) tower2d(c, p + ".EMA_block", s.ema_img, s.le, {false, false, true}, 5, 2, p + ".EMAlinear", style ? style + sd : nullptr, lds);
    else if (which == 2) tower1d(c, p + ".ENF0_block", s.crop, s.l1->N, s.l1, p + ".ENF0linear", style ? style + sd + sd / 2 : nullptr, lds);
}

void duration_style(Ctx& c, const float* ema_ext, int lde, const Lay* ref, float* ds , int ldd = 0 )
{
    const std::string p = "durationPredictor";
    const Lay* limg = c.lay(ref->w, 10);
    if (!limg) return;
    float* img = c.f32((size_t)std::max(limg->N, 1));
    RUN(c, as_rows_to_images_f32(ema_ext, lde, ref->d_off, 0, 10, img, limg->d_off, ref->B, ref->max_cols(), c.s));
    tower2d(c, p + ".dur_block", img, limg, {false, false, true}, 5, 2, p + ".dur_linear", ds, ldd > 0 ? ldd : c.m.cfg.style_dim / 4);
}

float* duration_tail(Ctx& c, float* d, const float* ds, const Lay* tok, float* dst = nullptr)
{
    const as_model& m = c.m;
    const std::string p = "durationPredictor";
    const int C = m.cfg.hidden_dim, S = m.cfg.style_dim / 4;
    std::vector<as_model::NormSpec> norms;
    for (int i = 0; i < 3; ++i)
        for (const char* n : {".norm1", ".norm2"}) norms.push_back({p + ".duration." + std::to_string(i) + n, 0, S});
    const FcOut fc = adain_fc_all(c, "duration", norms, ds, S, S, tok->B);
    Act x;
    x.p = d; x.C = C; x.ld = tok->N; x.lay = tok;
    for (int i = 0; i < 3; ++i) {
        BlkOpt o;
        o.names = {p + ".duration." + std::to_string(i)};
        o.n1 = fc.norm(o.names[0] + ".norm1");
        o.n2 = fc.norm(o.names[0] + ".norm2");
        o.want_yh = i == 2;
        const Norm nn = i < 2 ? fc.norm(p + ".duration." + std::to_string(i + 1) + ".norm1") : Norm();
        if (i < 2) o.next_n1 = &nn;
        x = adain_resblk1d(c, x, o);
        if (!x.lay) return nullptr;
    }
    const LstmW* L = m.lstm(p + ".LSTM");
    if (!L || !L->wih) { c.fail(AS_EINVAL); return nullptr; }
    const int H = L->H, Nn = std::max(tok->N, 1);
    float* gx = c.f32((size_t)Nn * 8 * H);
    ConvOpt q;
    q.bias = L->bias;
    q.transpose_out = true;
    conv_h(c, L->wih, x.h, x.C, tok, taps_1d(1), gx, 8 * H, q);
    float* h = c.f32((size_t)2 * H * Nn);
    BiLstmJob job;
    job.gx_tm = gx; job.whh_t = L->whh_t; job.out = h; job.ldg = 8 * H; job.ldo = tok->N;
    if (tok->N > 0 && c.go()) {
        size_t xb = 0;
        void* xchg = c.lstm_xchg(1, tok->B, &xb);
        RUN(c, as_bilstm_cluster_f32(&job, 1, tok->d_off, tok->B, H, tok->max_w, xchg, xb, c.s));
        if (c.go() && tok->max_w >= 200) c.long_launch();
    }
    float* y = c.f32(Nn);
    if (dst) y = dst;
    const float *pw = m.vec(p + ".duration_proj.linear_layer.weight"), *pb = m.vec(p + ".duration_proj.linear_layer.bias");
    RUN(c, as_project_cols_f32(h, tok->N, 2 * H, tok->N, pw, pb, 1, y, tok->N, c.s));
    return y;
}

std::vector<as_model::NormSpec> style_norms(const as_model& m)
{
    const int sd = m.cfg.style_dim;
    std::vector<as_model::NormSpec> v;
    const char* br[3] = {"F0", "N", "EMA"};
    const int off[3] = {sd + sd / 2, sd + sd / 2 + sd / 4, sd}, len[3] = {sd / 4, sd / 4, sd / 2};
    for (const char* n : {".norm1", ".norm2"}) v.push_back({std::string("artsPredictor.shared") + n, 0, 2 * sd});
    for (int blk = 0; blk < 3; ++blk)
        for (const char* n : {".norm1", ".norm2"})
            for (int g = 0; g < 3; ++g)
                v.push_back({std::string("artsPredictor.") + br[g] + "." + std::to_string(blk) + n, blk == 0 ? 0 : off[g], blk == 0 ? 2 * sd : len[g]});
    for (const char* n : {".norm1", ".norm2"}) v.push_back({std::string("decoder.encode") + n, 0, 2 * sd});
    for (int i = 0; i < 6; ++i)
        for (const char* n : {".norm1", ".norm2"})
            v.push_back({"decoder.decode." + std::to_string(i) + n, 0, i < 3 ? 2 * sd : sd});
    return v;
}

void arts_predictor(Ctx& c, const float* a_en, int lda, const Lay* lay, const FcOut& fc, float* fne, int ldp, const float* pros = nullptr,
                    int ld_pros = 0)
{
    const as_model& m = c.m;
    const std::string p = "artsPredictor";
    const int C = m.cfg.hidden_dim, B = lay->B, N1 = lay->N;
    const char* br[3] = {"F0", "N", "EMA"};
    Act a;
    a.p = const_cast<float*>(a_en); a.C = C; a.ld = lda; a.lay = lay;
    {
        BlkOpt o;
        o.names = {p + ".shared"};
        o.n1 = fc.norm(p + ".shared.norm1");
        o.n2 = fc.norm(p + ".shared.norm2");
        a = adain_resblk1d(c, a, o);
        if (!a.lay) return;
    }
    std::vector<int> w3;
    for (int g = 0; g < 3; ++g) w3.insert(w3.end(), lay->w.begin(), lay->w.end());
    const Lay* layG1 = lay->dyn ? c.dyn_lay(2, lay->dyn_B, lay->cap1) : c.lay(w3);
    const Lay* layG2 = layG1 ? c.scaled(layG1, 2) : nullptr;
    const Lay* lay2 = c.scaled(lay, 2);
    if (!layG1 || !layG2 || !lay2) return;
    const int N2 = lay2->N, NG2 = layG2->N, Nn = std::max(NG2, 1);
    const int32_t* src_off = c.itable(layG1, "src3", [&]() {
        std::vector<int32_t> t(3 * B);
        for (int g = 0; g < 3; ++g)
            for (int b = 0; b < B; ++b) t[g * B + b] = lay->off[b];
        return t;
    });
    auto gb_table = [&](int rows_per_group) {
        return c.itable(layG1, "gb3:" + std::to_string(rows_per_group), [&]() {
            std::vector<int32_t> t(3 * B);
            for (int g = 0; g < 3; ++g)
                for (int b = 0; b < B; ++b) t[g * B + b] = g * rows_per_group * B + b;
            return t;
        });
    };
    auto gnorm = [&](int blk, const char* n, int Cn) {
        Norm x = fc.norm(p + "." + br[0] + "." + std::to_string(blk) + n);
        x.gb_off = gb_table(2 * Cn);
        return x;
    };
    auto names = [&](int blk) { std::vector<std::string> v; for (int g = 0; g < 3; ++g) v.push_back(p + "." + br[g] + "." + std::to_string(blk)); return v; };
    Act x;
    {
        const std::vector<std::string> nm = names(0);
        auto sfx = [&](const char* s) { std::vector<std::string> v(nm); for (auto& n : v) n += s; return v; };
        const GemmW *w1 = m.conv_stack(sfx(".conv1")), *w2 = m.conv_stack(sfx(".conv2"));
        if (!w1 || !w2) { c.fail(AS_EINVAL); return; }
        uint16_t* xs = c.image(C, NG2);
        float* up = c.f32((size_t)C * Nn);
        const Norm n1 = gnorm(0, ".norm1", C);
        for (int g = 0; g < 3; ++g) {
            const float *pw = m.vec(nm[g] + ".pool.weight"), *pb = m.vec(nm[g] + ".pool.bias");
            if (!c.go() || NG2 == 0) continue;
            AsAdainArgs q;
            memset(&q, 0, sizeof(q));
            q.x = a.p; q.ldx = a.ld; q.C = C;
            q.gb = n1.gb; q.gb_off = n1.gb_off + g * B; q.ldgb = 1; q.gb_sc = n1.gb_sc;
            q.col_off = layG1->d_off + g * B; q.src_off = src_off + g * B; q.U = B; q.N = NG2; q.lrelu = 1; q.yh = xs;
            q.col_w = layG1->dyn ? layG1->d_w + g * B : nullptr;
            q.pool_w = pw; q.pool_b = pb; q.x_up = up; q.ld_up = NG2;
            RUN(c, as_adain_image_f32(&q, c.s));
        }
        ConvOpt q1;
        q1.bias = m.bias_stack(sfx(".conv1"));
        q1.group_cols = 2 * N1;
        uint16_t* xs2 = c.image(w1->M, NG2);
        const Norm n2 = gnorm(0, ".norm2", w1->M);
        q1.post_n = &n2; q1.post_lay = layG2; q1.post_yh = xs2;
        conv_h_new(c, w1, xs, C, layG2, taps_1d(3), q1);
        ConvOpt q2;
        q2.bias = m.bias_stack(sfx(".conv2"));
        q2.res = up;
        q2.ldr = NG2;
        q2.div_sqrt2 = true;
        q2.group_cols = 2 * N1;
        q2.want_yh = true;
        q2.yh = c.image(w2->M, NG2);
        const Norm nn = gnorm(1, ".norm1", w2->M);
        q2.post_n = &nn; q2.post_lay = layG2; q2.post_yh = c.image(w2->M, NG2);
        x.p = conv_h_new(c, w2, xs2, w1->M, layG2, taps_1d(3), q2);
        x.C = w2->M; x.ld = NG2; x.lay = layG2; x.h = q2.yh; x.pre = q2.post_yh;
    }
    for (int blk = 1; blk <= 2; ++blk) {
        BlkOpt o;
        o.names = names(blk);
        o.group_cols = 2 * N1;
        const GemmW* w1 = m.conv_stack({o.names[0] + ".conv1", o.names[1] + ".conv1", o.names[2] + ".conv1"});
        if (!w1) { c.fail(AS_EINVAL); return; }
        o.n1 = gnorm(blk, ".norm1", x.C);
        o.n2 = gnorm(blk, ".norm2", w1->M);
        o.want_yh = true;
        Norm nn;
        if (blk == 1) {
            nn = gnorm(2, ".norm1", w1->M);
            o.next_n1 = &nn;
        }
        x = adain_resblk1d(c, x, o);
        if (!x.lay) return;
    }
    std::vector<std::string> ln;
    for (int g = 0; g < 3; ++g) ln.push_back(p + "." + br[g] + "_LSTM");
    const float* lb = nullptr;
    const GemmW* wih = m.lstm_wih_stack(ln, &lb);
    const LstmW* L0 = m.lstm(ln[0]);
    if (!wih || !L0) { c.fail(AS_EINVAL); return; }
    const int H = L0->H;
    float* gx = c.f32((size_t)Nn * 8 * H);
    ConvOpt q;
    q.bias = lb;
    q.transpose_out = true;
    q.group_cols = 2 * N1;
    conv_h(c, wih, x.h, x.C, layG2, taps_1d(1), gx, 8 * H, q);
    float* hs = c.f32((size_t)2 * H * Nn);
    BiLstmJob jobs[3];
    for (int g = 0; g < 3; ++g) {
        const LstmW* L = m.lstm(ln[g]);
        if (!L) { c.fail(AS_EINVAL); return; }
        jobs[g].gx_tm = gx + (size_t)g * N2 * 8 * H; jobs[g].whh_t = L->whh_t; jobs[g].out = hs + (size_t)g * N2; jobs[g].ldg = 8 * H; jobs[g].ldo = NG2;
    }
    if (N2 > 0) RUN(c, as_bilstm_f32(jobs, 3, lay2->d_off, B, H, c.s));
    const int rows[3] = {0, 1, 2}, M[3] = {1, 1, 10};
    for (int g = 0; g < 3; ++g) {
        const float *pw = m.vec(p + "." + br[g] + "_proj.weight"), *pb = m.vec(p + "." + br[g] + "_proj.bias");
        if (pros)
            RUN(c, as_project_cols_prosody_launch(hs + (size_t)g * N2, NG2, 2 * H, N2, pw, pb, M[g], fne + (size_t)rows[g] * ldp, ldp, pros, ld_pros,
                                                  lay2->d_off, B, rows[g], c.s));
        else
            RUN(c, as_project_cols_f32(hs + (size_t)g * N2, NG2, 2 * H, N2, pw, pb, M[g], fne + (size_t)rows[g] * ldp, ldp, c.s));
    }
}

void copy_rows(Ctx& c, float* dst, int ldd, const float* src, int lds, int rows, int cols)
{
    if (c.go() && rows > 0 && cols > 0 &&
        hipMemcpy2DAsync(dst, (size_t)ldd * 4, src, (size_t)lds * 4, (size_t)cols * 4, rows, hipMemcpyDeviceToDevice, c.s) != hipSuccess)
        c.fail((int)hipErrorUnknown);
}

enum class Tracks { ToCaller, FromCaller };
void track_rows(Ctx& c, Tracks dir, float* fne, int N2, const float* F0, const float* N, const float* EMA, int ldp)
{
    const float* theirs[3] = {F0, N, EMA};
    const int row0[3] = {0, 1, 2}, rows[3] = {1, 1, 10};
    for (int i = 0; i < 3; ++i) {
        float* ours = fne + (size_t)row0[i] * N2;
        if (!theirs[i]) continue;
        if (dir == Tracks::FromCaller) copy_rows(c, ours, N2, theirs[i], ldp, rows[i], N2);
        else copy_rows(c, const_cast<float*>(theirs[i]), ldp, ours, N2, rows[i], N2);
    }
}

struct DecPre {
    uint16_t *x0h = nullptr, *cath = nullptr, *cath2 = nullptr;
    float* catb = nullptr;
    bool ok = false;
};
DecPre decoder_pre(Ctx& c, float* x0, const Lay* lay2)
{
    const as_model& m = c.m;
    const std::string p = "decoder";
    DecPre d;
    const int C = m.cfg.hidden_dim, N2 = lay2->N, Nn2 = std::max(N2, 1), bott = 2 * C, cat = bott + 64 + 128;
    const size_t blk_bytes = (size_t)4 * (N2 + 1) * 16;
    if (C % 64 || (C + 128) % 64) { c.fail(AS_EINVAL); return d; }
    d.x0h = c.image(C + 128, N2);
    d.catb = c.f32((size_t)cat * Nn2);
    d.cath = c.image(cat, N2);
    d.cath2 = c.image(cat, N2);
    RUN(c, as_split_f16x2_f32(x0, N2, C, N2, 0, 0.f, d.x0h, c.s));
    ConvOpt q;
    q.bias = m.bias(p + ".asr_res.0");
    q.want_yh = true;
    q.yh = d.cath ? reinterpret_cast<uint16_t*>(reinterpret_cast<char*>(d.cath) + (size_t)(bott / 16) * blk_bytes) : nullptr;
    conv_h(c, m.conv(p + ".asr_res.0"), d.x0h, C, lay2, taps_1d(1), d.catb ? d.catb + (size_t)bott * N2 : nullptr, N2, q);
    d.ok = c.rc == 0;
    return d;
}

void decoder(Ctx& c, const DecPre& dp, float* x0, const Lay* lay2, const float* fne, int ldp, const FcOut& fc, float* mel, int ldo)
{
    const as_model& m = c.m;
    const std::string p = "decoder";
    const int C = m.cfg.hidden_dim, N2 = lay2->N, bott = 2 * C, cat = bott + 64 + 128;
    const Taps k1 = taps_1d(1);
    const size_t blk_bytes = (size_t)4 * (N2 + 1) * 16;
    auto at_block = [&](uint16_t* img, int kb) { return img ? reinterpret_cast<uint16_t*>(reinterpret_cast<char*>(img) + (size_t)kb * blk_bytes) : nullptr; };
    if (!dp.ok) { c.fail(AS_EINVAL); return; }
    uint16_t *x0h = dp.x0h, *cath = dp.cath, *cath2 = dp.cath2;
    float* catb = dp.catb;
    const float *fb = nullptr, *w32 = nullptr;
    const GemmW* wf = m.fne(&fb, &w32);
    if (!wf) { c.fail(AS_EINVAL); return; }
    {
        if (wf->K > 16) { c.fail(AS_EINVAL); return; }
        RUN(c, as_pointwise_small_f32(fne, ldp, wf->K, N2, w32, fb, wf->M, x0 + (size_t)C * N2, N2, at_block(x0h, C / 16),
                                      catb + (size_t)(bott + 64) * N2, N2, at_block(cath, (bott + 64) / 16), c.s));
    }
    Act x;
    x.p = x0; x.C = C + 128; x.ld = N2; x.lay = lay2; x.h = x0h;
    {
        BlkOpt o;
        o.names = {p + ".encode"};
        o.n1 = fc.norm(p + ".encode.norm1");
        o.n2 = fc.norm(p + ".encode.norm2");
        o.out = catb; o.ldo = N2;
        o.want_yh = true; o.yh = cath;
        adain_resblk1d(c, x, o);
    }
    if (c.go() && hipMemcpyAsync(at_block(cath2, bott / 16), at_block(cath, bott / 16), (size_t)((cat - bott) / 16) * blk_bytes,
                                 hipMemcpyDeviceToDevice, c.s) != hipSuccess)
        c.fail((int)hipErrorUnknown);
    Act xc;
    xc.p = catb; xc.C = cat; xc.ld = N2; xc.lay = lay2; xc.h = cath;
    for (int i = 0; i < 2; ++i) {
        BlkOpt o;
        o.names = {p + ".decode." + std::to_string(i)};
        o.n1 = fc.norm(o.names[0] + ".norm1");
        o.n2 = fc.norm(o.names[0] + ".norm2");
        o.out = catb; o.ldo = N2;
        o.want_yh = true;
        o.yh = i == 0 ? cath2 : cath;
        xc.h = i == 0 ? cath : cath2;
        adain_resblk1d(c, xc, o);
    }
    xc.h = cath;
    Act y;
    for (int i = 2; i <= 5; ++i) {
        BlkOpt o;
        o.names = {p + ".decode." + std::to_string(i)};
        o.n1 = fc.norm(o.names[0] + ".norm1");
        o.n2 = fc.norm(o.names[0] + ".norm2");
        o.want_yh = i == 5;
        const Norm nn = i < 5 ? fc.norm(p + ".decode." + std::to_string(i + 1) + ".norm1") : Norm();
        if (i < 5) o.next_n1 = &nn;
        y = adain_resblk1d(c, i == 2 ? xc : y, o);
        if (!y.lay) return;
    }
    ConvOpt q;
    q.bias = m.bias(p + ".to_out.0");
    q.probe = true;
    conv_h(c, m.conv(p + ".to_out.0"), y.h, y.C, lay2, k1, mel, ldo, q);
}

struct PhaseA {
    FcOut fc;
    bool has_fc = false;
    float *feat12 = nullptr, *style = nullptr, *a_en = nullptr, *t_en = nullptr, *duration = nullptr;
    int ld_en = 0;
    int32_t *dur_i = nullptr, *frame_off = nullptr;
    float* dur_s = nullptr;
    int32_t* tok_start = nullptr;
    int32_t* fit_dur = nullptr;
// ... 107 lines not shown
        }
        if (!bp.dur_late) {
            f.branch(bp.dur);
            dur_block();
        }
    }
    if (bp.fc >= 0) {
        if (A.ref) f.after(bp.fc, {bp.tower[0], bp.tower[1], bp.tower[2]});
        f.branch(bp.fc);
        A.fc = adain_fc_all(c, "style", style_norms(m), A.style, sd2, sd2, B);
        A.has_fc = true;
    }
    f.back();
    EncOut eo;
    std::unique_ptr<Fork> f2;
    rel_encoder_multi(c, path_encoders(), io->tokens, A.tok, &eo, [&](int g) {
        if (g != ENC_DUR) return;
        if (bp.dur_late) {
            f2.reset(new Fork(c, 1, bp.dur));
            f2->branch(0);
            dur_block();
        } else {
            f.wait_main(bp.dur);
            f.branch(bp.dur);
        }
        A.duration = duration_tail(c, eo.y[ENC_DUR], ds, A.tok, io->duration);
        f.back();
    });
    A.a_en = eo.y[ENC_ARTS];
    A.t_en = eo.y[ENC_TEXT];
    A.ld_en = eo.ld[ENC_ARTS];
    if (f2) f2->join();
    f.join();
    if (c.go()) c.p.mark(2, c.s);
    if (!batch->frames && io->frame_cap <= 0)
        durations_launch(c, tp, A, io, A.dur_i, A.frame_off, nullptr, 0);
    return A;
}

int segments_status(const as_segments* segs, int B, int N1, bool wants_pred)
{
    long sum = 0;
    if (segs->n < 1 || segs->n > AS_MAX_SEGMENTS || segs->first[0] != 0 || segs->first[segs->n] != B) return AS_EINVAL;
    for (int i = 0; i < segs->n; ++i) {
        if (segs->first[i + 1] <= segs->first[i] || segs->cap[i] < 1 || !segs->mel_out[i]) return AS_EINVAL;
        if (segs->ld_out[i] < 2 * segs->cap[i]) return AS_ENOSPC;
        sum += segs->cap[i];
    }
    return sum != N1 || wants_pred ? AS_EINVAL : AS_OK;
}

bool dyn_geometry(Ctx& c, const as_segments* segs, const Lay* lay1, const Lay* lay2, int B, int frame_cap, int32_t* frame_off, int32_t* tof)
{
    const Lay *lg1 = c.dyn_lay(2, B, frame_cap), *lg2 = lg1 ? c.scaled(lg1, 2) : nullptr;
    if (!lg1 || !lg2) return false;
    if (!c.go()) return true;
    const int N1 = lay1->N;
    AsDynGeo g;
    memset(&g, 0, sizeof(g));
    g.frame_off = frame_off; g.B = B; g.cap1 = N1;
    g.n_seg = segs ? segs->n : 1;
    for (int i = 0; i < g.n_seg; ++i) {
        g.seg_first[i] = segs ? segs->first[i] : 0;
        g.seg_cap[i] = segs ? segs->cap[i] : N1;
        g.seg_frame_off[i] = segs ? segs->frame_off[i] : nullptr;
    }
    g.seg_first[g.n_seg] = B;
    const Lay* ls[4] = {lay1, lay2, lg1, lg2};
    for (int i = 0; i < 4; ++i) {
        g.w[i] = ls[i]->d_w; g.off[i] = ls[i]->d_off; g.nvalid[i] = ls[i]->d_nvalid;
        g.meta[i] = reinterpret_cast<unsigned long long*>(ls[i]->d_meta);
    }
    auto t3 = lg1->tabs.find("src3");
    g.src3 = t3 != lg1->tabs.end() ? t3->second : nullptr;
    g.tof = tof;
    g.status = as_status_words_device();
    RUN(c, as_dyn_geometry_launch(g, c.s));
    return true;
}

DecPre text_half(Ctx& c, const PhaseA& A, const int32_t* tof, int N1, float* x0, const Lay* lay2)
{
    const int C = c.m.cfg.hidden_dim, N2 = lay2->N;
    c.hint(0, 4.0 * C * ((double)A.tok->N + N2));
    RUN(c, as_expand_f32(A.t_en, A.ld_en, C, tof, N1, 2, x0, N2, c.s));
    return decoder_pre(c, x0, lay2);
}

void seg_scatter(Ctx& c, const as_segments* segs, const float* src, int ld_src, int rows, const int32_t* frame_off, int B)
{
    if (!c.go()) return;
    AsSegScatter sc;
    memset(&sc, 0, sizeof(sc));
    sc.src = src; sc.ld_src = ld_src; sc.rows = rows; sc.n_seg = segs->n; sc.frame_off = frame_off;
    for (int i = 0; i < segs->n; ++i) {
        sc.seg_first[i] = segs->first[i]; sc.seg_cap[i] = segs->cap[i];
        sc.dst[i] = segs->mel_out[i]; sc.ld_dst[i] = segs->ld_out[i];
    }
    sc.seg_first[segs->n] = B;
    RUN(c, as_seg_scatter_launch(sc, c.s));
}

void forward_b(Ctx& c, const PhaseA& A, const as_batch* batch, const as_forward_io* io)
{
    const as_model& m = c.m;
    const int C = m.cfg.hidden_dim, B = batch->B, n_mels = m.cfg.n_mels;
    const bool dyn = !batch->frames;
    const as_segments* segs = dyn ? io->segs : nullptr;
    const Lay* lay1 = dyn ? c.dyn_lay(0, B, io->frame_cap) : c.lay(vec_of(batch->frames, B));
    if (!lay1) return;
    const Lay* lay2 = c.scaled(lay1, 2);
    if (!lay2) return;
    const int N1 = lay1->N, N2 = lay2->N;
    int fits = AS_OK;
    if (segs) fits = segments_status(segs, B, N1, io->F0 != nullptr);
    else if (io->ld_out < N2 || (io->F0 && io->ld_pred < N2)) fits = AS_ENOSPC;
    if (fits != AS_OK) { c.fail(fits); return; }
    int32_t* tof = c.i32((size_t)std::max(N1, 1));
    int32_t* dur_i = c.i32((size_t)std::max(A.tok->N, 1));
    int32_t* frame_off = c.i32(B + 1);
    float* mel_packed = dyn ? c.f32((size_t)n_mels * std::max(N2, 1)) : nullptr;
    const as_token_prosody tp = c.p.tok_pros;
    const int ntok = A.tok->N;
    float* dur_s = A.dur_s;
    int32_t* tok_start = A.tok_start;
    if (tp.rows && (segs || !dur_s || !tok_start)) { c.fail(AS_EINVAL); return; }
    if (io->dur_i) dur_i = io->dur_i;
    if (io->frame_off && !segs) frame_off = io->frame_off;
    if (c.p.fit.n_spans && segs) { c.fail(AS_EINVAL); return; }
    durations_launch(c, tp, A, io, dur_i, frame_off, tof, N1);
    if (tp.rows) RUN(c, as_token_starts_launch(dur_i, ntok, tok_start, c.s));
    if (dyn && !dyn_geometry(c, segs, lay1, lay2, B, io->frame_cap, frame_off, tof)) return;
    float* a_ex = c.f32((size_t)C * std::max(N1, 1));
    float* fne = c.f32((size_t)12 * std::max(N2, 1));
    float* x0 = c.f32((size_t)(C + 128) * std::max(N2, 1));
    const FcOut fc = A.has_fc ? A.fc : adain_fc_all(c, "style", style_norms(m), A.style, 2 * m.cfg.style_dim, 2 * m.cfg.style_dim, B);
    const bool rec = c.records();
    DecPre dp;
    {
        std::unique_ptr<Fork> f;
        if (rec) {
            f.reset(new Fork(c, 1, 0));
            f->branch(0);
            dp = text_half(c, A, tof, N1, x0, lay2);
            f->back();
        }
        c.hint(0, 4.0 * C * ((double)A.tok->N + N1));
        RUN(c, as_expand_f32(A.a_en, A.ld_en, C, tof, N1, 1, a_ex, N1, c.s));
        arts_predictor(c, a_ex, N1, lay1, fc, fne, N2, io->prosody, io->ld_prosody);
        if (tp.rows) {
            const int32_t* tok_off = A.tok->d_off;
            const float* rows = tp.rows;
            const int ld_rows = tp.ld, smooth = tp.smooth;
            RUN(c, as_token_tracks_launch(fne, N2, N2, tof, N1, frame_off, tok_off, B, ntok, tok_start, rows, ld_rows, smooth, c.s));
        }
        if (f) f->join();
    }
    if (c.go()) c.p.mark(3, c.s);
    if (!rec) dp = text_half(c, A, tof, N1, x0, lay2);
    decoder(c, dp, x0, lay2, fne, N2, fc, segs ? mel_packed : io->mel_out, segs ? N2 : io->ld_out);
    if (segs) seg_scatter(c, segs, mel_packed, N2, n_mels, frame_off, B);
    if (c.go()) c.p.mark(4, c.s);
    track_rows(c, Tracks::ToCaller, fne, N2, io->F0, io->N, io->EMA, io->ld_pred);
}

void outputs_a(Ctx& c, const PhaseA& A, const as_forward_io* io)
{
    if (!c.go()) return;
    const int C = c.m.cfg.hidden_dim, Nt = A.tok->N, Nr = A.ref ? A.ref->N : 0;
// ... 16 lines not shown
    return io->tokens && (!need_out || io->mel_out) && io->ld_voice >= voice_dim(*m) && io->n_voices >= 1 && !io->feat12;
}

struct Any {
    template <class T> operator T*() const { return reinterpret_cast<T*>(16); }
};
constexpr Any ANY;
constexpr int ANY_LD = 1 << 30;

int encoder_module(Ctx& c, const as_batch* batch, int which, const int32_t* tokens, float* out, int ldo)
{
    const Lay* lay = c.lay(vec_of(batch->tok_lens, batch->B));
    if (!lay || ldo < lay->N) return AS_EINVAL;
    EncOut eo;
    rel_encoder_multi(c, path_encoders(), tokens, lay, &eo, [](int) {});
    const int g = which == 0 ? ENC_TEXT : (which == 1 ? ENC_ARTS : ENC_DUR);
    copy_rows(c, out, ldo, eo.y[g], eo.ld[g], c.m.cfg.hidden_dim, lay->N);
    return AS_OK;
}

int style_module(Ctx& c, const as_batch* batch, const float* mel, int ldm, const float* f0_raw, const float* ema_raw, int lde, float* feat12,
                 int ldf, float* style)
{
    const Lay* ref = c.lay(vec_of(batch->ref_lens, batch->B));
    if (!ref || ldm < ref->N || lde < ref->N || ldf < ref->N) return AS_EINVAL;
    const StyleIn si = ref_style_inputs(c, mel, ldm, f0_raw, ema_raw, lde, feat12, ldf, ref);
    if (si.l1) for (int t = 0; t < 3; ++t) style_tower(c, t, si, style);
    return AS_OK;
}

int voice_module(Ctx& c, const as_batch* batch, const float* mel, int ldm, const float* f0_raw, const float* ema_raw, int lde, float* voice, int ldv)
{
    const Lay* ref = c.lay(vec_of(batch->ref_lens, batch->B));
    if (!ref || ldm < ref->N || lde < ref->N || ldv < voice_dim(c.m)) return AS_EINVAL;
    const int sd2 = 2 * c.m.cfg.style_dim;
    float* feat12 = c.f32((size_t)12 * std::max(ref->N, 1));
    const StyleIn si = ref_style_inputs(c, mel, ldm, f0_raw, ema_raw, lde, feat12, ref->N, ref);
    if (!si.l1) return AS_OK;
    for (int t = 0; t < 3; ++t) style_tower(c, t, si, voice, ldv);
    duration_style(c, feat12 ? feat12 + (size_t)2 * ref->N : nullptr, ref->N, ref, voice ? voice + sd2 : nullptr, ldv);
    return AS_OK;
}

int duration_module(Ctx& c, const as_batch* batch, const int32_t* tokens, const float* ema_ext, int lde, float* duration)
{
    const Lay *tok = c.lay(vec_of(batch->tok_lens, batch->B)), *ref = c.lay(vec_of(batch->ref_lens, batch->B));
    if (!tok || !ref || lde < ref->N) return AS_EINVAL;
    float* ds = c.f32((size_t)batch->B * (c.m.cfg.style_dim / 4));
    duration_style(c, ema_ext, lde, ref, ds);
    EncOut eo;
    rel_encoder_multi(c, path_encoders(), tokens, tok, &eo, [](int) {});
    duration_tail(c, eo.y[ENC_DUR], ds, tok, duration);
    return AS_OK;
}

int arts_module(Ctx& c, const as_batch* batch, const float* a_ens, int lda, const float* style, float* F0, float* N, float* EMA, int ldp)
{
    const Lay* lay = c.lay(vec_of(batch->frames, batch->B));
    if (!lay || lda < lay->N || ldp < 2 * lay->N) return AS_EINVAL;
    const int N2 = 2 * lay->N, sd2 = 2 * c.m.cfg.style_dim;
    const FcOut fc = adain_fc_all(c, "style", style_norms(c.m), style, sd2, sd2, batch->B);
    float* fne = c.f32((size_t)12 * std::max(N2, 1));
    arts_predictor(c, a_ens, lda, lay, fc, fne, N2);
    track_rows(c, Tracks::ToCaller, fne, N2, F0, N, EMA, ldp);
    return AS_OK;
}

int decoder_module(Ctx& c, const as_batch* batch, const float* asr, int lda, const float* style, const float* F0, const float* N,
                   const float* EMA, int ldp, float* mel, int ldo)
{
    const Lay* lay = c.lay(vec_of(batch->frames, batch->B));
    if (!lay) return AS_EINVAL;
    const Lay* lay2 = c.scaled(lay, 2);
    if (!lay2 || lda < lay->N || ldp < lay2->N || ldo < lay2->N) return AS_EINVAL;
    int32_t* ident = c.i32((size_t)std::max(lay->N, 1));
    if (c.go() && lay->N > 0) {
        std::vector<int32_t> h(lay->N);
        for (int i = 0; i < lay->N; ++i) h[i] = i;
        if (hipMemcpyAsync(ident, h.data(), (size_t)lay->N * 4, hipMemcpyHostToDevice, c.s) != hipSuccess || hipStreamSynchronize(c.s) != hipSuccess)
            c.fail((int)hipErrorUnknown);
    }
    const int C = c.m.cfg.hidden_dim, N2 = lay2->N, sd2 = 2 * c.m.cfg.style_dim;
    float* x0 = c.f32((size_t)(C + 128) * std::max(N2, 1));
    RUN(c, as_expand_f32(asr, lda, C, ident, lay->N, 2, x0, N2, c.s));
    float* fne = c.f32((size_t)12 * std::max(N2, 1));
    track_rows(c, Tracks::FromCaller, fne, N2, F0, N, EMA, ldp);
    const FcOut fc = adain_fc_all(c, "style", style_norms(c.m), style, sd2, sd2, batch->B);
    decoder(c, decoder_pre(c, x0, lay2), x0, lay2, fne, N2, fc, mel, ldo);
    return AS_OK;
}

const as_forward_io* dummy_io()
{
    static const as_forward_io io = [] {
        as_forward_io d;
        memset(&d, 0, sizeof(d));
        d.tokens = ANY;
        d.mel = d.f0_raw = d.ema_raw = ANY;
        d.mel_out = ANY;
        d.ld_mel = d.ld_ema = d.ld_out = d.ld_pred = ANY_LD;
        return d;
    }();
    return &io;
}
const as_forward_io* dummy_voice_io()
{
    static const as_forward_io io = [] {
        as_forward_io d = *dummy_io();
        d.mel = d.f0_raw = d.ema_raw = nullptr;
        d.voices = ANY;
        d.ld_voice = ANY_LD;
        d.n_voices = 1;
        return d;
    }();
    return &io;
}

size_t count_module(const as_model* m, as_plan* p, int module, const as_batch* batch)
{
    static const struct { int module; bool tok, ref, frames; } need[] = {
        {AS_MOD_FORWARD_A, 1, 1, 0}, {AS_MOD_FORWARD_B, 1, 0, 1}, {AS_MOD_ENCODER, 1, 0, 0},       {AS_MOD_STYLE, 0, 1, 0},
        {AS_MOD_DURATION, 1, 1, 0},  {AS_MOD_ARTS, 0, 0, 1},      {AS_MOD_DECODER, 0, 0, 1},       {AS_MOD_FORWARD_B_CAP, 1, 0, 1},
        {AS_MOD_VOICE, 0, 1, 0},     {AS_MOD_FORWARD_A_VOICE, 1, 0, 0}};
    static_assert(sizeof(need) / sizeof(need[0]) == AS_MOD_FORWARD_A_VOICE + 1, "one row per AS_MOD_* value");
    const auto* nd = std::find_if(std::begin(need), std::end(need), [&](const auto& r) { return r.module == module; });
    if (nd == std::end(need) || !batch_ok(batch, nd->tok, nd->ref, nd->frames)) return 0;
    Ctx c(*m, *p, nullptr, nullptr, 0, Pass::Count);
    int rc = AS_OK;
    switch (module) {
    case AS_MOD_ENCODER: rc = encoder_module(c, batch, 0, ANY, ANY, ANY_LD); break;
    case AS_MOD_STYLE: rc = style_module(c, batch, ANY, ANY_LD, ANY, ANY, ANY_LD, ANY, ANY_LD, ANY); break;
    case AS_MOD_DURATION: rc = duration_module(c, batch, ANY, ANY, ANY_LD, ANY); break;
    case AS_MOD_ARTS: rc = arts_module(c, batch, ANY, ANY_LD, ANY, ANY, ANY, ANY, ANY_LD); break;
    case AS_MOD_DECODER: rc = decoder_module(c, batch, ANY, ANY_LD, ANY, ANY, ANY, ANY, ANY_LD, ANY, ANY_LD); break;
    case AS_MOD_FORWARD_A: forward_a(c, batch, dummy_io()); break;
    case AS_MOD_VOICE: rc = voice_module(c, batch, ANY, ANY_LD, ANY, ANY, ANY_LD, ANY, ANY_LD); break;
    case AS_MOD_FORWARD_A_VOICE: forward_a(c, batch, dummy_voice_io()); break;
    default: {
        as_forward_io io = batch->ref_lens ? *dummy_io() : *dummy_voice_io();
        as_batch b = *batch;
        if (module == AS_MOD_FORWARD_B_CAP) {
            long cap = 0;
            for (int i = 0; i < b.B; ++i) cap += std::max(b.frames[i], 0);
            if (cap < 1 || cap > (1 << 28)) return 0;
            io.frame_cap = (int32_t)cap;
            b.frames = nullptr;
        }
        Ctx ca(*m, *p, nullptr, nullptr, 0, Pass::Count);
        const PhaseA A = forward_a(ca, &b, &io);
        if (ca.rc || !A.ok()) return 0;
        forward_b(c, A, &b, &io);
    }
    }
    return rc || c.rc ? 0 : c.peak + 256;
}

struct Call {
    Ctx c;
    Call(const as_model* m, as_plan* p, void* ws, size_t bytes, as_stream_t stream, Pass pass, bool trim)
        : c(*m, *p, static_cast<hipStream_t>(stream), ws, bytes, pass)
    {
        const int r = enter(*p, c.s, ws, pass, trim);
        if (r != AS_OK) c.fail(r);
    }
    int done(int r = AS_OK) const { return r ? r : (c.rc ? c.rc : c.m.err); }
};

}

static int model_create(const void* blob_host, size_t blob_bytes, const as_model_cfg* cfg, as_model** out)
{
// ... 285 lines not shown
```

artspeech_amd/ops.py:

```python
import ctypes
import os

import torch

from . import _lib
from ._lib import check, ptr, stream

AS_MAX_TAPS = _lib.AS_MAX_TAPS
META_MAX_H, META_MAX_W = 1023, 4194303
KTILE = 16
ACT_NONE, ACT_RELU, ACT_LRELU, ACT_TANH, ACT_ABS, ACT_SWISH = 0, 1, 2, 3, 4, 5


ConvGemmArgs = _lib.ConvGemmArgs


def _ld(t):
    if t.dim() != 2 or t.stride(1) != 1:
        raise _lib.HipLibraryError("expected a 2-D tensor with contiguous rows")
    return t.stride(0)


def _p(t):
    if t is None:
# ... 93 lines not shown
        import math
        _, e = math.frexp(mx)
        scale = math.ldexp(1.0, 14 - e)
    ws = w4.float() * scale
    h = ws.half()
    l = (ws - h.float()).half()
    kx = kbx(K) * 16
    parts = torch.stack([h, l], 0)
    if kx != K:
        parts = torch.cat([parts, parts.new_zeros(2, G, M, kx - K, T)], dim=3)
    img = parts.reshape(2, G, M, kx // 16, 2, 8, T).permute(1, 6, 3, 0, 4, 2, 5)
    return img.contiguous().view(torch.int16).reshape(G, T, kx // 16, 4, M, 8), scale


def prep_weight(w, device=None, stack=None, sc=None):
    ws = [w] + list(stack or [])
    cout, cin = w.shape[0], w.shape[1]
    w4 = torch.stack([x.reshape(cout, cin, -1).float() for x in ws], 0).cpu()
    T = w4.shape[3]
    kp = (cin + KTILE - 1) // KTILE * KTILE
    if sc is not None:
        scs = list(sc) if isinstance(sc, (list, tuple)) else [sc]
        w2 = torch.stack([x.reshape(cout, -1).float() for x in scs], 0).cpu().contiguous()
        G, cin2 = len(ws), w2.shape[2]
        assert w2.shape[0] == G
        L = _lib.lib()
        nbytes = L.as_prep_weight_f16x2_sc_bytes(G, cout, cin, T, cin2)
        img = torch.empty(nbytes // 2, dtype=torch.int16)
        scale = ctypes.c_float()
        w4c = w4.contiguous()
        check(L.as_prep_weight_f16x2_sc_host(w4c.data_ptr(), w2.data_ptr(), G, cout, cin, T, cin2, img.data_ptr(), ctypes.byref(scale)),
              "as_prep_weight_f16x2_sc_host")
        return GemmWeight(img.to(device) if device is not None else img, scale.value, (T, kp, cout), G, None)
    img, scale = split_f16x2_weight(w4)
    w32 = None
    if cin == 1 and len(ws) == 1:
        w32 = torch.cat([w4[0].permute(2, 1, 0), w4.new_zeros(T, kp - cin, cout)], dim=1).contiguous()
    if device is not None:
        img = img.to(device)
        w32 = w32.to(device) if w32 is not None else None
    return GemmWeight(img, scale, (T, kp, cout), len(ws), w32)


def strided_source(lay_in, lay_out, stride, device):
    cols, metas = [], []
    for b in range(lay_out.B):
        Wi, Wo = lay_in.widths_host[b], lay_out.widths_host[b]
        for ho in range(lay_out.H):
            for wo in range(Wo):
                h, w = ho * stride, wo * stride
                cols.append(lay_in.off_host[b] + h * Wi + w)
                metas.append(h | (lay_in.H << 10) | (w << 20) | (Wi << 42))
    return torch.tensor(cols, dtype=torch.int32, device=device), torch.tensor(metas, dtype=torch.int64, device=device)


def taps_1d(k):
    return [(0, t - k // 2) for t in range(k)]


def taps_2d(kh, kw):
    return [(a - kh // 2, d - kw // 2) for a in range(kh) for d in range(kw)]


def new_image(K, N, device):
    return torch.empty(max(_lib.lib().as_split_f16x2_bytes(K, N) // 2, 8), dtype=torch.int16, device=device)


def split_act(X, lay, in_act=0, in_slope=0.2):
    K, N = X.shape[0], lay.N
    xs = new_image(K, N, X.device)
    check(_lib.lib().as_split_f16x2_f32(_p(X), _ld(X), K, N, in_act, in_slope, _p(xs), stream()), "as_split_f16x2_f32")
    return xs


def adain_split(X, gb, lay, lrelu=True):
    C = X.shape[0]
    xs = new_image(C, lay.N, X.device)
    check(_lib.lib().as_adain_split_f32(_p(X), _ld(X), C, _p(gb), _ld(gb), _p(lay.col_off), lay.B, lay.N, int(lrelu), _p(xs), stream()),
          "as_adain_split_f32")
    return xs


def adain_image(X, lay, gb, gb_sc, N_out, ldgb=1, gb_off=None, src_off=None, pool_w=None, pool_b=None, x_up=None, col_w=None, col_off=None,
                out=None):
    C = X.shape[0]
    xs = new_image(C, N_out, X.device) if out is None else out
    a = _lib.AdainArgs()
    a.x, a.ldx, a.C = _p(X), _ld(X), C
    a.gb, a.gb_off, a.ldgb, a.gb_sc = _p(gb), _p(gb_off), ldgb, gb_sc
    U = lay.B if col_off is None else (col_w.numel() if col_w is not None else col_off.numel() - 1)
    a.col_off, a.src_off, a.U, a.N, a.lrelu, a.yh = _p(lay.col_off if col_off is None else col_off), _p(src_off), U, N_out, 1, _p(xs)
    a.pool_w, a.pool_b, a.x_up, a.ld_up = _p(pool_w), _p(pool_b), _p(x_up), (_ld(x_up) if x_up is not None else 0)
    a.col_w = _p(col_w)
    check(_lib.lib().as_adain_image_f32(ctypes.byref(a), stream()), "as_adain_image_f32")
    return xs


def rows_image(x):
    B, K = x.shape
    xh = new_image(K, B, x.device)
    check(_lib.lib().as_rows_image_f32(_p(x), _ld(x), K, B, _p(xh), stream()), "as_rows_image_f32")
    return xh


def project_cols(X, N, w, bias, Y):
    M, K = w.shape
    check(_lib.lib().as_project_cols_f32(_p(X), _ld(X), K, N, _p(w), _p(bias), M, _p(Y), _ld(Y), stream()), "as_project_cols_f32")
    return Y


def conv_gemm(Wt, X, lay, Y, taps, bias=None, res=None, act=0, div_sqrt2=False, in_act=0, transpose_out=False,
              use_meta=True, in_slope=0.2, act_slope=0.2, xs=None, K=None, group_cols=0, yh=None, yh_lrelu=False, n_prod=None, plan_out=None,
              x2s=None, K2=0, src_col=None, src_meta=None, N_in=0, defer=None, ileave=0, n_valid=None, ws_bytes=None):
    T, Kp, M = Wt.shape
    if X is None:
        if xs is None or K is None:
            raise ValueError("conv_gemm: X may be omitted only with xs= and K=")
    else:
        K = X.shape[0]
    if Kp % KTILE or not (Kp - KTILE < K <= Kp):
        raise ValueError(f"conv_gemm: weight rows {Kp} do not match input channels {K} (use ops.prep_weight)")
    if (Wt.G > 1) != (group_cols > 0):
        raise ValueError("conv_gemm: stacked weights need group_cols (and only they)")
    a = ConvGemmArgs()
    a.Kp = Kp
    a.Wh, a.W, a.X, a.Xh, a.Y, a.Yh, a.bias, a.res = _p(Wt.wh), _p(Wt.w32), _p(X), _p(xs), _p(Y), _p(yh), _p(bias), _p(res)
    a.acc_scale = 1.0 / Wt.scale
    a.n_groups, a.group_cols = Wt.G, group_cols
    a.meta = _p(lay.meta) if (use_meta and not (T == 1 and taps[0] == (0, 0))) else None
    a.M, a.N, a.K, a.T = M, lay.N, K, T
    a.ldx, a.ldy = (_ld(X) if X is not None else lay.N), (_ld(Y) if Y is not None else lay.N)
    a.ldr = _ld(res) if res is not None else 0
    a.act, a.div_sqrt2, a.in_act, a.transpose_out = act, int(div_sqrt2), in_act, int(transpose_out)
    a.yh_lrelu = int(yh_lrelu)
    a.Xh2, a.K2 = _p(x2s), K2
    if src_col is not None:
        a.src_col, a.N_in, a.meta = _p(src_col), N_in, _p(src_meta)
    a.n_prod = n_prod if n_prod is not None else (1 if GEMM_IMPL == "h1" else 3)
    a.ileave_u = int(ileave)
    if n_valid is not None:
        if n_valid.dtype != torch.int32:
            raise ValueError("conv_gemm: n_valid is a device int32 tensor")
        a.n_valid = _p(n_valid)
    a.in_slope, a.act_slope = in_slope, act_slope
    assert len(taps) == T
    for i, (dh, dw) in enumerate(taps):
        a.dh[i], a.dw[i] = dh, dw
    L = _lib.lib()
    if ws_bytes is None:
        ws_bytes = "multi" if defer is not None else "single"
    if isinstance(ws_bytes, str):
        nbytes = (L.as_conv_gemm_multi_workspace_bytes if ws_bytes == "multi" else L.as_conv_gemm_workspace_bytes)(ctypes.byref(a))
    else:
        nbytes = int(ws_bytes)
    if nbytes:
        ws = torch.empty(nbytes // 4 + 4, dtype=torch.float32, device=(Y if Y is not None else yh).device)
        a.ws, a.ws_bytes = ws.data_ptr(), nbytes
    if plan_out is not None:
        k, t, sl = ctypes.c_int32(), ctypes.c_int32(), ctypes.c_int32()
        check(L.as_conv_gemm_plan(ctypes.byref(a), ctypes.byref(k), ctypes.byref(t), ctypes.byref(sl)), "as_conv_gemm_plan")
        plan_out.update(kind=k.value, tile=t.value, slices=sl.value)
    if defer is not None:
        defer.append((a, [Wt, X, xs, Y, yh, bias, res, x2s, src_col, src_meta, lay, (ws if nbytes else None), n_valid]))
        return Y if Y is not None else yh
    check(L.as_conv_gemm_f32(ctypes.byref(a), stream()), "as_conv_gemm_f32")
    return Y if Y is not None else yh


def conv_gemm_multi(deferred, tile_out=None):
    n = len(deferred)
    arr = (ConvGemmArgs * n)(*[d[0] for d in deferred])
    L = _lib.lib()
    if tile_out is not None:
        tile_out.append(L.as_conv_gemm_multi_tile(arr, n))
    check(L.as_conv_gemm_multi_f32(arr, n, stream()), "as_conv_gemm_multi_f32")


def conv_gemm_multi_post(deferred, posts, lns=None):
    n = len(deferred)
    arr = (ConvGemmArgs * n)(*[d[0] for d in deferred])
    pa = (_lib.AdainArgs * n)()
    la = (_lib.LnArgs * n)()
    mw = (ctypes.c_int32 * n)()
    for i, q in enumerate(lns or []):
        if q is None:
            continue
        la[i].gamma, la[i].beta, la[i].yh, la[i].relu, la[i].eps = _p(q[0]), _p(q[1]), _p(q[2]), int(q[3]), 1e-4
        if len(q) > 4:
            la[i].gamma2, la[i].beta2, la[i].n_split = _p(q[4]), _p(q[5]), int(q[6])
    for i, q in enumerate(posts or [None] * n):
        if q is None:
            continue
        gb, gb_sc, lay, img = q[:4]
        gb_off = q[4] if len(q) > 4 else None
        pa[i].gb, pa[i].gb_off, pa[i].ldgb, pa[i].gb_sc = _p(gb), _p(gb_off), 1, gb_sc
        pa[i].col_off, pa[i].U, pa[i].lrelu, pa[i].yh = _p(lay.col_off), lay.B, 1, _p(img)
        mw[i] = q[5] if len(q) > 5 else (max(lay.widths_host) if hasattr(lay, "widths_host") else int(lay.widths.max()))
    check(_lib.lib().as_conv_gemm_multi_post_f32(arr, pa, mw, la, n, stream()), "as_conv_gemm_multi_post_f32")


def embed(tokens_i32, emb, scale, Y, group2=None, n_cols=None):
    V, C = emb.shape
    emb2, n_split = group2 if group2 is not None else (None, 0)
    n_tok = tokens_i32.numel()
    check(_lib.lib().as_embed_groups_f32(_p(tokens_i32), n_tok, _p(emb), _p(emb2), n_split, C, n_tok if n_cols is None else n_cols, V, scale,
                                         _p(Y), _ld(Y), stream()), "as_embed_groups_f32")
    return Y


def channel_layernorm(X, N, gamma, beta, Y, relu=False, eps=1e-4, group2=None):
    g2, b2, n_split = group2 if group2 is not None else (None, None, 0)
    check(_lib.lib().as_channel_layernorm_groups_f32(_p(X), _ld(X), X.shape[0], N, _p(gamma), _p(beta), _p(g2), _p(b2), n_split, eps,
                                                     int(relu), _p(Y), _ld(Y), stream()), "as_channel_layernorm_groups_f32")
    return Y


def adain(X, gb, lay, Y, lrelu=True, pool_w=None, pool_b=None, x_up=None):
    C = X.shape[0]
    check(_lib.lib().as_adain_f32(_p(X), _ld(X), C, _p(gb), _ld(gb), _p(lay.col_off), lay.B, _p(Y), _ld(Y), int(lrelu),
                                  _p(pool_w), _p(pool_b), _p(x_up), _ld(x_up) if x_up is not None else 0, stream()),
          "as_adain_f32")
    return Y


def linear_rows(x, w, bias, y=None):
    B, K = x.shape
    M = w.shape[0]
    if y is None:
        y = torch.empty((B, M), dtype=torch.float32, device=x.device)
    check(_lib.lib().as_linear_rows_f32(_p(x), _ld(x), _p(w), _p(bias), B, M, K, _p(y), _ld(y), stream()),
          "as_linear_rows_f32")
    return y


def durations(dur_f32, forced, tok_lay, max_frames):
    dev = tok_lay.device
    dur_i = torch.empty(max(tok_lay.N, 1), dtype=torch.int32, device=dev)
    frame_off = torch.empty(tok_lay.B + 1, dtype=torch.int32, device=dev)
    tof = torch.empty(max(max_frames, 1), dtype=torch.int32, device=dev) if max_frames > 0 else None
    check(_lib.lib().as_durations_f32(_p(dur_f32), _p(forced), _p(tok_lay.col_off), tok_lay.B, _p(dur_i), _p(frame_off),
                                      _p(tof), max_frames, stream()), "as_durations_f32")
    return dur_i, frame_off, tof


def expand(X, tok_of_frame, n_frames, repeat, Y):
    check(_lib.lib().as_expand_f32(_p(X), _ld(X), X.shape[0], _p(tok_of_frame), n_frames, repeat, _p(Y), _ld(Y), stream()),
          "as_expand_f32")
    return Y


def ref_features(mel, f0_raw, ema_raw, N, stats24, feat):
    check(_lib.lib().as_ref_features_f32(_p(mel), _ld(mel), mel.shape[0], _p(f0_raw), _p(ema_raw), _ld(ema_raw), N,
                                         _p(stats24), _p(feat), _ld(feat), stream()), "as_ref_features_f32")
    return feat


def crop(src, src_lay, start, dst, dst_lay):
    check(_lib.lib().as_crop_f32(_p(src), _ld(src), _p(src_lay.col_off), start, _p(dst), _ld(dst), _p(dst_lay.col_off),
                                 dst_lay.B, src.shape[0], dst_lay.max_cols, stream()), "as_crop_f32")
    return dst


def bn_lrelu_maxpool_rows(X, tok_lay, H, k, scale, shift, slope, Y, to_channels=False):
    check(_lib.lib().as_bn_lrelu_maxpool_rows_f32(_p(X), _ld(X), _p(tok_lay.col_off), tok_lay.B, X.shape[0], H, k, _p(scale), _p(shift),
                                                  slope, _p(Y), _ld(Y), int(to_channels), tok_lay.N, stream()),
          "as_bn_lrelu_maxpool_rows_f32")
    return Y


def rows_to_images(src, src_lay, start, H, img_lay):
    dst = img_lay.new(1)
    check(_lib.lib().as_rows_to_images_f32(_p(src), _ld(src), _p(src_lay.col_off), start, H, _p(dst), _p(img_lay.col_off),
                                           img_lay.B, src_lay.max_cols, stream()), "as_rows_to_images_f32")
    return dst


def interleave_phases(Z, bias, C, u, n_in, Y):
    check(_lib.lib().as_interleave_phases_f32(_p(Z), _ld(Z), _p(bias), C, u, n_in, _p(Y), _ld(Y), stream()),
          "as_interleave_phases_f32")
    return Y


def mean3(A, B, C3, n, Y):
    check(_lib.lib().as_mean3_f32(_p(A), _p(B), _p(C3), _ld(A), A.shape[0], n, _p(Y), _ld(Y), stream()), "as_mean3_f32")
    return Y


def conv_post(X, lay, w, bias, in_slope, tanh_out=True, pcm=False):
    Y = lay.new(1)
    if pcm:
        P = torch.empty(max(lay.N, 1), dtype=torch.int16, device=X.device)
        check(_lib.lib().as_conv_post_pcm_f32(_p(X), _ld(X), X.shape[0], lay.N, _p(w), _p(bias), w.shape[1], float(in_slope), int(tanh_out),
                                              _p(lay.meta), _p(Y), _p(P), stream()), "as_conv_post_pcm_f32")
        return Y, P
    check(_lib.lib().as_conv_post_f32(_p(X), _ld(X), X.shape[0], lay.N, _p(w), _p(bias), w.shape[1], float(in_slope), int(tanh_out),
                                      _p(lay.meta), _p(Y), stream()), "as_conv_post_f32")
    return Y


def respair(X, lay, w1, b1, w2, b2, k, dil, slope, Y=None, add=None, image_slope=None):
    a = _lib.ResPairArgs()
    if isinstance(X, tuple):
        X, xb, u = X
        C = xb.shape[0]
        a.x_u, a.x_bias = int(u), _p(xb)
    else:
        C = X.shape[0]
    if image_slope is not None:
        yh = new_image(C, lay.N, X.device)
        a.yh, a.yh_slope = _p(yh), float(image_slope)
    else:
        if Y is None:
            Y = lay.new(C)
        a.y, a.ldy = _p(Y), _ld(Y)
    a.x, a.ldx = _p(X), _ld(X)
    a.w1, a.w2, a.b1, a.b2 = _p(w1.wh), _p(w2.wh), _p(b1), _p(b2)
    a.scale1, a.scale2 = 1.0 / w1.scale, 1.0 / w2.scale
    a.C, a.N, a.k, a.dil, a.slope = C, lay.N, int(k), int(dil), float(slope)
    a.col_off, a.B, a.max_w = _p(lay.col_off), lay.B, lay.max_cols
    if add is not None:
        a.add1, a.add2, a.ld_add, a.out_div = _p(add[0]), _p(add[1]), _ld(add[0]), 3.0
    check(_lib.lib().as_respair_f32(ctypes.byref(a), stream()), "as_respair_f32")
    return Y if image_slope is None else yh


def mean3_image(A, B, C3, n, slope):
    xh = new_image(A.shape[0], n, A.device)
    check(_lib.lib().as_mean3_image_f32(_p(A), _p(B), _p(C3), _ld(A), A.shape[0], n, float(slope), _p(xh), stream()), "as_mean3_image_f32")
    return xh


def down_args(kind, X, lin, lout, Y=None, yh=None, w=None, bias=None, kh=0, pool_h=0, Kp=0, res=None, lrelu=False):
    a = _lib.DownArgs()
    a.kind, a.x, a.ldx = kind, _p(X), (_ld(X) if X.dim() > 1 else 0)
    a.in_off, a.in_w, a.Hin = _p(lin.col_off), _p(lin.widths), lin.H
    a.out_off, a.out_w, a.Hout = _p(lout.col_off), _p(lout.widths), lout.H
    a.y, a.ldy, a.yh, a.n_out = _p(Y), (_ld(Y) if Y is not None else 0), _p(yh), lout.N
    a.w, a.bias, a.kh, a.pool_h, a.Kp = _p(w), _p(bias), kh, pool_h, Kp
    a.res, a.ldr, a.lrelu = _p(res), (_ld(res) if res is not None else 0), int(lrelu)
    a.B, a.C, a.max_out = lin.B, (X.shape[0] if kind != 2 else bias.shape[0]), lout.max_cols
    return a


def down_multi(args):
    arr = (_lib.DownArgs * max(len(args), 1))(*args)
    check(_lib.lib().as_down_multi_f32(arr, len(args), stream()), "as_down_multi_f32")


def dwconv_down(X, lin, Y, lout, w, bias, kh, lrelu):
    check(_lib.lib().as_dwconv_down_f32(_p(X), _ld(X), _p(lin.col_off), _p(lin.widths), lin.H, _p(Y), _ld(Y),
                                        _p(lout.col_off), _p(lout.widths), lout.H, _p(w), _p(bias), kh, lin.B,
                                        X.shape[0], lout.max_cols, int(lrelu), stream()), "as_dwconv_down_f32")
    return Y


def avgpool_down(X, lin, Y, lout, pool_h, res=None):
    check(_lib.lib().as_avgpool_down_f32(_p(X), _ld(X), _p(lin.col_off), _p(lin.widths), lin.H, _p(Y), _ld(Y),
                                         _p(lout.col_off), _p(lout.widths), lout.H, pool_h, _p(res),
                                         _ld(res) if res is not None else 0, lin.B, X.shape[0], lout.max_cols, stream()),
          "as_avgpool_down_f32")
    return Y


def dwconv_down_image(X, lin, lout, w, bias, kh, lrelu):
    yh = new_image(X.shape[0], lout.N, X.device)
    check(_lib.lib().as_dwconv_down_image_f32(_p(X), _ld(X), _p(lin.col_off), _p(lin.widths), lin.H, _p(lout.col_off), _p(lout.widths), lout.H,
                                              _p(w), _p(bias), kh, lin.B, X.shape[0], lout.max_cols, int(lrelu), _p(yh), lout.N, stream()),
          "as_dwconv_down_image_f32")
    return yh


def avgpool_down_image(X, lin, Y, lout, pool_h, res=None, yh_lrelu=False):
    yh = new_image(X.shape[0], lout.N, X.device)
    check(_lib.lib().as_avgpool_down_image_f32(_p(X), _ld(X), _p(lin.col_off), _p(lin.widths), lin.H, _p(Y), _ld(Y) if Y is not None else 0,
                                               _p(lout.col_off), _p(lout.widths), lout.H, pool_h, _p(res), _ld(res) if res is not None else 0,
                                               lin.B, X.shape[0], lout.max_cols, _p(yh), lout.N, int(yh_lrelu), stream()),
          "as_avgpool_down_image_f32")
    return yh


def stem_pool_image(x1, lin, lout, pool_h, Wt, bias, kh):
    C = Wt.shape[2]
    yh = new_image(C, lout.N, x1.device)
    check(_lib.lib().as_stem_pool_image_f32(_p(x1), _p(lin.col_off), _p(lin.widths), lin.H, _p(lout.col_off), _p(lout.widths), lout.H, pool_h,
                                            _p(Wt.w32), Wt.shape[1], _p(bias), kh, lin.B, C, lout.max_cols, _p(yh), lout.N, stream()),
          "as_stem_pool_image_f32")
    return yh


def im2col_valid_image(X, lin, lout, K, stride, lrelu):
    yh = new_image(X.shape[0] * K * K, lout.N, X.device)
    check(_lib.lib().as_im2col_valid_image_f32(_p(X), _ld(X), _p(lin.col_off), _p(lin.widths), _p(lout.col_off), _p(lout.widths), K, stride,
                                               int(lrelu), lin.B, X.shape[0], _p(yh), stream()), "as_im2col_valid_image_f32")
    return yh


def im2col_valid(X, lin, col, lout, K, stride, lrelu):
    check(_lib.lib().as_im2col_valid_f32(_p(X), _ld(X), _p(lin.col_off), _p(lin.widths), lin.H, _p(col), _ld(col),
                                         _p(lout.col_off), _p(lout.widths), lout.H, K, stride, int(lrelu), lin.B,
                                         X.shape[0], lout.max_cols, stream()), "as_im2col_valid_f32")
    return col


def mean_pool(X, lay, lrelu, y=None):
    C = X.shape[0]
    if y is None:
        y = torch.empty((lay.B, C), dtype=torch.float32, device=X.device)
    check(_lib.lib().as_mean_pool_f32(_p(X), _ld(X), _p(lay.col_off), lay.B, C, int(lrelu), _p(y), _ld(y), stream()),
          "as_mean_pool_f32")
    return y


def channel_layernorm_split(X, lay, gamma, beta, relu=False, eps=1e-4, group2=None, out=None):
    L = _lib.lib()
    C = X.shape[0]
    g2, b2, n_split = group2 if group2 is not None else (None, None, 0)
    xs = new_image(C, lay.N, X.device) if out is None else out
    check(L.as_channel_layernorm_split_f32(_p(X), _ld(X), C, lay.N, _p(gamma), _p(beta), _p(g2), _p(b2), n_split, eps, int(relu), _p(xs),
                                           stream()), "as_channel_layernorm_split_f32")
    return xs


def relpos_attention(qkv, C, heads, window, ek, ev, lay, out, group2=None):
    ek2, ev2, b_split = group2 if group2 is not None else (None, None, 0)
    check(_lib.lib().as_relpos_attention_groups_f32(_p(qkv), _ld(qkv), C, heads, window, _p(ek), _p(ev), _p(ek2), _p(ev2), b_split,
                                                    _p(lay.col_off), lay.B, lay.max_w, _p(out), _ld(out), stream()),
          "as_relpos_attention_groups_f32")
    return out


def relpos_attention_image(qkv, qkv_h, C, heads, window, ek, ev, lay, out=None, out_h=None, group2=None):
    ek2, ev2, b_split = group2 if group2 is not None else (None, None, 0)
    check(_lib.lib().as_relpos_attention_image_f32(_p(qkv), _ld(qkv), _p(qkv_h), lay.N, C, heads, window, _p(ek), _p(ev), _p(ek2), _p(ev2), b_split,
                                                   _p(lay.col_off), lay.B, lay.max_w, _p(out), _ld(out) if out is not None else 0, _p(out_h),
                                                   stream()), "as_relpos_attention_image_f32")
    return out if out is not None else out_h


def xl_attention(qkv, C, heads, pos, u_bias, v_bias, inv_scale, lay, out):
    check(_lib.lib().as_xl_attention_f32(_p(qkv), _ld(qkv), C, heads, _p(pos), _ld(pos), _p(u_bias), _p(v_bias), inv_scale,
                                         _p(lay.col_off), lay.B, lay.max_w, _p(out), _ld(out), stream()), "as_xl_attention_f32")
    return out


def xl_attention_image(qkv4, qkv4_h, pos_h, C, heads, inv_scale, lay, out=None, image=False):
    oh = new_image(C, lay.N, qkv4.device) if image else None
    check(_lib.lib().as_xl_attention_image_f32(_p(qkv4), _ld(qkv4), _p(qkv4_h), _p(pos_h), lay.N, C, heads, inv_scale, _p(lay.col_off), lay.B,
                                               lay.max_w, _p(out), _ld(out) if out is not None else 0, _p(oh), stream()),
          "as_xl_attention_image_f32")
    return oh if image else out


def glu_dwconv_bn_swish(A, C, w, scale, shift, lay, Y):
    check(_lib.lib().as_glu_dwconv_bn_swish_f32(_p(A), _ld(A), C, _p(w), w.shape[1], _p(scale), _p(shift), _p(lay.col_off), lay.B,
                                                _p(Y), _ld(Y), stream()), "as_glu_dwconv_bn_swish_f32")
    return Y


def lstm_step0(gx, H, N, out):
    check(_lib.lib().as_lstm_step0_f32(_p(gx), _ld(gx), H, N, _p(out), _ld(out), stream()), "as_lstm_step0_f32")
    return out


def bilstm(jobs, lay, H, xchg=None):
    arr = (_lib.BiLstmJob * len(jobs))()
    for i, (gx_tm, whh_t, out) in enumerate(jobs):
        arr[i].gx_tm, arr[i].whh_t, arr[i].out = _p(gx_tm), _p(whh_t), _p(out)
        arr[i].ldg, arr[i].ldo = _ld(gx_tm), _ld(out)
    if xchg is not None:
        check(_lib.lib().as_bilstm_cluster_f32(arr, len(jobs), _p(lay.col_off), lay.B, H, lay.max_w, _p(xchg), xchg.numel() * xchg.element_size(),
                                               stream()), "as_bilstm_cluster_f32")
    else:
        check(_lib.lib().as_bilstm_f32(arr, len(jobs), _p(lay.col_off), lay.B, H, stream()), "as_bilstm_f32")
    return [j[2] for j in jobs]


def bilstm_exchange_buffer(n_jobs, B, device):
    return torch.zeros(_lib.lib().as_bilstm_cluster_bytes(n_jobs, B) // 8, dtype=torch.int64, device=device)
```

include/artspeech_hip.h:

```cpp
#ifndef ARTSPEECH_HIP_H
#define ARTSPEECH_HIP_H
#include <stddef.h>
#include <stdint.h>
#ifdef __cplusplus
extern "C" {
#endif

typedef void* as_stream_t;

#define AS_ABI_VERSION 10
int as_abi_version(void);

#define AS_EDEVICE (-3)
enum { AS_STATUS_LSTM_TIMEOUT = 0, AS_STATUS_MAS_TIMEOUT = 1, AS_STATUS_BAD_TOKEN = 2, AS_STATUS_F16_RANGE = 3, AS_STATUS_BAD_LAYOUT = 4,
       AS_STATUS_CAPACITY = 5, AS_STATUS_BAD_VOICE = 6, AS_STATUS_KINDS = 7 };
int as_device_status(int clear);
int as_device_status_raise_for_test(int kind, as_stream_t stream);
int as_set_range_probe(int on);
#define AS_PROBE_THIS 2

int as_prof_enable(int on);
int as_prof_collect(double* ms, double* flops, double* bytes, int32_t* launches, int n_classes);
int as_prof_hint(double flops, double bytes);
int as_prof_bracket_overhead(as_stream_t stream, double* overhead_ms);
int as_prof_mfma_sustained(as_stream_t stream, double* tflops_registers, double* tflops_lds_fed);

size_t as_mas_workspace_bytes(int B, int Tx, int Ty);
int as_mas_f32(const float* value, const int32_t* t_x, const int32_t* t_y, int B, int Tx, int Ty,
               int tie_mode, float* path, int32_t* dur, int32_t* rows,
               void* workspace, size_t workspace_bytes, as_stream_t stream);
int as_softmax_mas_f32(const float* feat, const int32_t* t_x, const int32_t* t_y, int B, int Tx, int Ty, int softmax_dim,
                       int tie_mode, float* attn, float* path, int32_t* dur, int32_t* rows, void* workspace,
                       size_t workspace_bytes, as_stream_t stream);

#define AS_META_MAX_H 1023
#define AS_META_MAX_W 4194303
#define AS_META_PACK(h, w, H, W) \
    ((uint64_t)(h) | ((uint64_t)(H) << 10) | ((uint64_t)(w) << 20) | ((uint64_t)(W) << 42))
#define AS_META_h(md) ((int)((md) & 1023u))
#define AS_META_H(md) ((int)(((md) >> 10) & 1023u))
#define AS_META_w(md) ((int)(((md) >> 20) & 4194303u))
#define AS_META_W(md) ((int)((md) >> 42))
int as_make_meta(const int32_t* widths, const int32_t* col_off, int B, int H, int n_cols_max,
                 uint64_t* meta, as_stream_t stream);

#define AS_MAX_TAPS 25
typedef struct ConvGemmArgs {
    const uint16_t* Wh;
    const float* W;
    const float* X;
    const uint16_t* Xh;
    float* Y;
    uint16_t* Yh;
    const float* bias;
    const float* res;
    const uint64_t* meta;
    void* ws;
    size_t ws_bytes;
    int32_t M, N, K, T;
    int32_t Kp;
    int32_t ldx, ldy, ldr;
    int32_t act;
    int32_t div_sqrt2;
    int32_t in_act;
    int32_t transpose_out;
    int32_t yh_lrelu;
    int32_t n_prod;
    int32_t dh[AS_MAX_TAPS];
    int32_t dw[AS_MAX_TAPS];
    float in_slope, act_slope;
    float acc_scale;
    int32_t n_groups, group_cols;
    int32_t range_probe;
    uint32_t* status;
    const uint16_t* Xh2;
    int32_t K2;
    const int32_t* src_col;
    int32_t N_in;
    int32_t ileave_u;
    int32_t slab_tr;
    const int32_t* n_valid;
} ConvGemmArgs;
#define AS_SLOPE_PATH 0.2f
int as_conv_gemm_f32(const ConvGemmArgs* args_host, as_stream_t stream);
#define AS_MAX_MULTI 6
int as_conv_gemm_multi_f32(const ConvGemmArgs* list_host, int n, as_stream_t stream);
int as_conv_gemm_multi_tile(const ConvGemmArgs* list_host, int n);
size_t as_conv_gemm_multi_workspace_bytes(const ConvGemmArgs* args_host);
int as_conv_gemm_plan(const ConvGemmArgs* args_host, int32_t* kind, int32_t* tile, int32_t* slices);
size_t as_conv_gemm_workspace_bytes(const ConvGemmArgs* args_host);
size_t as_split_f16x2_bytes(int K, int N);
int as_split_f16x2_f32(const float* x, int ldx, int K, int N, int in_act, float in_slope, uint16_t* xh, as_stream_t stream);
int as_split_f16x2_cap_f32(const float* x, int ldx, int K, int N, const int32_t* n_valid, int in_act, float in_slope, uint16_t* xh,
                           as_stream_t stream);
size_t as_prep_weight_f16x2_bytes(int G, int Cout, int Cin, int T);
int as_prep_weight_f16x2_host(const float* w_host, int G, int Cout, int Cin, int T, uint16_t* wh_host, float* scale_out);
size_t as_prep_weight_f16x2_sc_bytes(int G, int Cout, int Cin, int T, int Cin2);
int as_prep_weight_f16x2_sc_host(const float* w_host, const float* w2_host, int G, int Cout, int Cin, int T, int Cin2, uint16_t* wh_host,
                                 float* scale_out);

int as_embed_f32(const int32_t* tokens, const float* emb, int C, int N, int V, float scale, float* y, int ldy,
                 as_stream_t stream);
int as_embed_groups_f32(const int32_t* tokens, int n_tok, const float* emb, const float* emb2, int n_split, int C, int N, int V,
                        float scale, float* y, int ldy, as_stream_t stream);
int as_channel_layernorm_groups_f32(const float* x, int ldx, int C, int N, const float* gamma, const float* beta, const float* gamma2,
                                    const float* beta2, int n_split, float eps, int relu, float* y, int ldy, as_stream_t stream);
int as_channel_layernorm_split_f32(const float* x, int ldx, int C, int N, const float* gamma, const float* beta, const float* gamma2,
                                   const float* beta2, int n_split, float eps, int relu, uint16_t* xs, as_stream_t stream);
int as_relpos_attention_groups_f32(const float* qkv, int ld, int C, int heads, int window, const float* emb_rel_k,
                                   const float* emb_rel_v, const float* emb_rel_k2, const float* emb_rel_v2, int b_split,
                                   const int32_t* col_off, int B, int max_len, float* out, int ldo, as_stream_t stream);
int as_relpos_attention_image_f32(const float* qkv, int ld, const uint16_t* qkv_h, int n_total, int C, int heads, int window,
                                  const float* emb_rel_k, const float* emb_rel_v, const float* emb_rel_k2, const float* emb_rel_v2,
                                  int b_split, const int32_t* col_off, int B, int max_len, float* out, int ldo, uint16_t* out_h,
                                  as_stream_t stream);
int as_relpos_attention_image_lds_bytes(int max_len);
int as_channel_layernorm_f32(const float* x, int ldx, int C, int N, const float* gamma, const float* beta, float eps,
                             int relu, float* y, int ldy, as_stream_t stream);
int as_adain_f32(const float* x, int ldx, int C, const float* gamma_beta, int ldgb, const int32_t* col_off, int B,
                 float* y, int ldy, int lrelu, const float* pool_w, const float* pool_b, float* x_up, int ld_up,
                 as_stream_t stream);
int as_adain_split_f32(const float* x, int ldx, int C, const float* gamma_beta, int ldgb, const int32_t* col_off, int B, int N,
                       int lrelu, uint16_t* xs, as_stream_t stream);
typedef struct AsAdainArgs {
    const float* x;
    int32_t ldx, C;
    const float* gb;
    const int32_t* gb_off;
    int32_t ldgb, gb_sc;
    const int32_t* col_off;
    const int32_t* src_off;
    int32_t U, N;
    int32_t lrelu;
    uint16_t* yh;
    const float* pool_w;
    const float* pool_b;
    float* x_up;
    int32_t ld_up;
    const int32_t* col_w;
} AsAdainArgs;
int as_adain_image_f32(const AsAdainArgs* args_host, as_stream_t stream);
typedef struct AsLnArgs {
    const float *gamma, *beta, *gamma2, *beta2;
    int32_t n_split;
    float eps;
    int32_t relu;
    uint16_t* yh;
} AsLnArgs;
int as_conv_gemm_multi_post_f32(const ConvGemmArgs* list_host, const AsAdainArgs* post_host, const int32_t* post_max_w,
                                const AsLnArgs* post_ln_host, int n, as_stream_t stream);
int as_rows_image_f32(const float* x, int ldx, int K, int B, uint16_t* xh, as_stream_t stream);
int as_project_cols_f32(const float* x, int ldx, int K, int N, const float* w, const float* bias, int M, float* y, int ldy,
                        as_stream_t stream);
int as_pointwise_small_f32(const float* x, int ldx, int K, int N, const float* w, const float* bias, int M, float* y1, int ld1,
                           uint16_t* yh1, float* y2, int ld2, uint16_t* yh2, as_stream_t stream);
int as_linear_rows_f32(const float* x, int ldx, const float* w, const float* bias, int B, int M, int K, float* y,
                       int ldy, as_stream_t stream);
int as_durations_f32(const float* dur_f32, const int32_t* forced_dur, const int32_t* tok_off, int B, int32_t* dur_i32,
                     int32_t* frame_off, int32_t* tok_of_frame, int max_frames, as_stream_t stream);
int as_expand_f32(const float* x, int ldx, int C, const int32_t* tok_of_frame, int n_frames, int repeat, float* y,
                  int ldy, as_stream_t stream);
int as_ref_features_f32(const float* mel, int ldm, int n_mels, const float* f0_raw, const float* ema_raw, int lde,
                        int N, const float* stats24, float* feat, int ldf, as_stream_t stream);
int as_crop_f32(const float* src, int lds, const int32_t* src_off, int start, float* dst, int ldd,
                const int32_t* dst_off, int B, int C, int max_len, as_stream_t stream);
int as_rows_to_images_f32(const float* src, int lds, const int32_t* src_off, int start, int H, float* dst,
                          const int32_t* img_off, int B, int max_w, as_stream_t stream);
int as_dwconv_down_f32(const float* x, int ldx, const int32_t* in_off, const int32_t* in_w, int Hin, float* y, int ldy,
                       const int32_t* out_off, const int32_t* out_w, int Hout, const float* w, const float* bias,
                       int kh, int B, int C, int max_out, int lrelu, as_stream_t stream);
int as_bn_lrelu_maxpool_rows_f32(const float* x, int ldx, const int32_t* tok_off, int B, int C, int H, int k, const float* scale,
                                 const float* shift, float slope, float* y, int ldy, int to_channels, int total_frames,
                                 as_stream_t stream);
int as_avgpool_down_f32(const float* x, int ldx, const int32_t* in_off, const int32_t* in_w, int Hin, float* y, int ldy,
                        const int32_t* out_off, const int32_t* out_w, int Hout, int pool_h, const float* res, int ldr,
                        int B, int C, int max_out, as_stream_t stream);
int as_im2col_valid_f32(const float* x, int ldx, const int32_t* in_off, const int32_t* in_w, int Hin, float* col,
                        int ldc, const int32_t* out_off, const int32_t* out_w, int Hout, int K, int stride, int lrelu,
                        int B, int C, int max_out, as_stream_t stream);
int as_dwconv_down_image_f32(const float* x, int ldx, const int32_t* in_off, const int32_t* in_w, int Hin, const int32_t* out_off,
                             const int32_t* out_w, int Hout, const float* w, const float* bias, int kh, int B, int C, int max_out,
                             int lrelu, uint16_t* yh, int n_out, as_stream_t stream);
int as_avgpool_down_image_f32(const float* x, int ldx, const int32_t* in_off, const int32_t* in_w, int Hin, float* y, int ldy,
                              const int32_t* out_off, const int32_t* out_w, int Hout, int pool_h, const float* res, int ldr, int B,
                              int C, int max_out, uint16_t* yh, int n_out, int yh_lrelu, as_stream_t stream);
int as_stem_pool_image_f32(const float* x, const int32_t* in_off, const int32_t* in_w, int Hin, const int32_t* out_off,
                           const int32_t* out_w, int Hout, int pool_h, const float* w, int Kp, const float* bias, int kh, int B, int C,
                           int max_out, uint16_t* yh, int n_out, as_stream_t stream);
typedef struct AsDownArgs {
    int32_t kind;
    const float* x; int32_t ldx;
    const int32_t* in_off; const int32_t* in_w; int32_t Hin;
    float* y; int32_t ldy;
    const int32_t* out_off; const int32_t* out_w; int32_t Hout;
    const float* w; const float* bias;
    int32_t kh, pool_h, Kp;
    const float* res; int32_t ldr;
    int32_t B, C, max_out, lrelu;
    uint16_t* yh; int32_t n_out;
} AsDownArgs;
int as_down_multi_f32(const AsDownArgs* list_host, int n, as_stream_t stream);
int as_down_strip_rule(int kind, int Hout, int max_wo, int B, int groups, int32_t* strips, int32_t* rows);
int as_im2col_valid_image_f32(const float* x, int ldx, const int32_t* in_off, const int32_t* in_w, const int32_t* out_off,
                              const int32_t* out_w, int K, int stride, int lrelu, int B, int C, uint16_t* yh, as_stream_t stream);
int as_mean_pool_f32(const float* x, int ldx, const int32_t* col_off, int B, int C, int lrelu, float* y, int ldy,
                     as_stream_t stream);

int as_frame_signal_f32(const float* wave, const int32_t* wav_off, const int32_t* frame_off, int B, int max_frames, int n_fft, int hop,
                        float* X, int ldx, as_stream_t stream);
int as_spec_power_f32(const float* Y, int ldy, int F, int N, float* P, int ldp, as_stream_t stream);
int as_log_norm_f32(const float* x, int ldx, int C, int N, float eps, float mean, float std, float* y, int ldy, as_stream_t stream);

int as_xl_attention_f32(const float* qkv, int ld, int C, int heads, const float* pos, int ldp, const float* u_bias,
                        const float* v_bias, float inv_scale, const int32_t* col_off, int B, int max_len, float* out, int ldo,
                        as_stream_t stream);
int as_xl_attention_image_f32(const float* qkv, int ld, const uint16_t* qkv_h, const uint16_t* pos_h, int n_total, int C, int heads,
                              float inv_scale, const int32_t* col_off, int B, int max_len, float* out, int ldo, uint16_t* out_h,
                              as_stream_t stream);
int as_glu_dwconv_bn_swish_f32(const float* a, int lda, int C, const float* w, int k, const float* scale, const float* shift,
                               const int32_t* col_off, int B, float* y, int ldy, as_stream_t stream);
int as_lstm_step0_f32(const float* gx, int ldg, int H, int N, float* h, int ldh, as_stream_t stream);

int as_relpos_attention_f32(const float* qkv, int ld, int C, int heads, int window, const float* emb_rel_k,
                            const float* emb_rel_v, const int32_t* col_off, int B, int max_len, float* out, int ldo,
                            as_stream_t stream);

#define AS_MAX_LSTM_JOBS 4
typedef struct BiLstmJob {
    const float* gx_tm;
    const float* whh_t;
    float* out;
    int32_t ldg, ldo;
} BiLstmJob;
int as_bilstm_f32(const BiLstmJob* jobs_host, int n_jobs, const int32_t* col_off, int B, int H, as_stream_t stream);
size_t as_bilstm_cluster_bytes(int n_jobs, int B);
int as_bilstm_cluster_f32(const BiLstmJob* jobs_host, int n_jobs, const int32_t* col_off, int B, int H, int max_len, void* xchg,
                          size_t xchg_bytes, as_stream_t stream);

int as_bilstm_cluster_test_hooks(int drop_member, int spin_limit);

int as_interleave_phases_f32(const float* z, int ldz, const float* bias, int C, int u, int Nin, float* y, int ldy,
                             as_stream_t stream);
int as_mean3_f32(const float* a, const float* b, const float* c, int ld, int C, int N, float* y, int ldy, as_stream_t stream);
int as_mean3_image_f32(const float* a, const float* b, const float* c, int ld, int C, int N, float slope, uint16_t* xh, as_stream_t stream);
int as_conv_post_f32(const float* x, int ldx, int C, int N, const float* w, const float* bias, int k, float in_slope, int tanh_out,
                     const uint64_t* meta, float* y, as_stream_t stream);
int as_conv_post_pcm_f32(const float* x, int ldx, int C, int N, const float* w, const float* bias, int k, float in_slope, int tanh_out,
                         const uint64_t* meta, float* y, int16_t* pcm, as_stream_t stream);
typedef struct AsResPairArgs {
    const float* x; int32_t ldx;
    float* y; int32_t ldy;
    const uint16_t* w1; const uint16_t* w2;
    const float* b1; const float* b2;
    float scale1, scale2;
    int32_t C, N, k, dil;
    float slope;
    const int32_t* col_off; int32_t B, max_w;
    const float* add1; const float* add2; int32_t ld_add; float out_div;
    uint16_t* yh; float yh_slope;
    int32_t x_u; const float* x_bias;
} AsResPairArgs;
int as_respair_f32(const AsResPairArgs* a, as_stream_t stream);
int as_interleave_phases_cap_f32(const float* z, int ldz, const float* bias, int C, int u, int Nin, const int32_t* n_valid, float* y, int ldy,
                                 as_stream_t stream);
int as_mean3_cap_f32(const float* a, const float* b, const float* c, int ld, int C, int N, const int32_t* n_valid, float* y, int ldy,
                     as_stream_t stream);
int as_mean3_image_cap_f32(const float* a, const float* b, const float* c, int ld, int C, int N, const int32_t* n_valid, float slope,
                           uint16_t* xh, as_stream_t stream);
int as_conv_post_pcm_cap_f32(const float* x, int ldx, int C, int N, const float* w, const float* bias, int k, float in_slope, int tanh_out,
                             const uint64_t* meta, const int32_t* n_valid, float* y, int16_t* pcm, as_stream_t stream);
int as_vocoder_cap_geometry(const int32_t* off, int B, int mult, int cap, int max_len, int n_rates, const int32_t* rates_host, int32_t* tab,
                            uint64_t* meta, int32_t* sample_off, as_stream_t stream);

typedef struct as_model as_model;
typedef struct as_plan as_plan;
#define AS_ENOSPC (-2)

typedef struct as_model_cfg {
    int32_t hidden_dim;
    int32_t dim_in;
    int32_t style_dim;
    int32_t n_mels;
    int32_t n_token;
    int32_t reserved;
    float stats[24];
} as_model_cfg;

int as_model_create(const void* blob_host, size_t blob_bytes, const as_model_cfg* cfg, as_model** out);
int as_model_destroy(as_model* m);
// ... 258 lines not shown
```

Before: 1.821 million.

## Fuse embed/expand with operand-image writes, batch style crops, pool+linear, adain sets

```diff
diff --git a/artspeech_amd/_lib.py b/artspeech_amd/_lib.py
--- a/artspeech_amd/_lib.py
+++ b/artspeech_amd/_lib.py
@@ -64,6 +64,7 @@
     "as_prep_weight_f16x2_sc_bytes": (c_sz, [c_i, c_i, c_i, c_i, c_i]),
     "as_prep_weight_f16x2_sc_host": (c_i, [c_p, c_p, c_i, c_i, c_i, c_i, c_i, c_p, c_p]),
     "as_embed_groups_f32": (c_i, [c_p, c_i, c_p, c_p, c_i, c_i, c_i, c_i, c_f, c_p, c_i, c_p]),
+    "as_embed_groups_image_f32": (c_i, [c_p, c_i, c_p, c_p, c_i, c_i, c_i, c_i, c_f, c_p, c_i, c_p, c_p]),
     "as_channel_layernorm_groups_f32": (c_i, [c_p, c_i, c_i, c_i, c_p, c_p, c_p, c_p, c_i, c_f, c_i, c_p, c_i, c_p]),
     "as_channel_layernorm_split_f32": (c_i, [c_p, c_i, c_i, c_i, c_p, c_p, c_p, c_p, c_i, c_f, c_i, c_p, c_p]),
     "as_relpos_attention_groups_f32": (c_i, [c_p, c_i, c_i, c_i, c_i, c_p, c_p, c_p, c_p, c_i, c_p, c_i, c_i, c_p, c_i, c_p]),
@@ -74,9 +75,11 @@
     "as_linear_rows_f32": (c_i, [c_p, c_i, c_p, c_p, c_i, c_i, c_i, c_p, c_i, c_p]),
     "as_durations_f32": (c_i, [c_p, c_p, c_p, c_i, c_p, c_p, c_p, c_i, c_p]),
     "as_expand_f32": (c_i, [c_p, c_i, c_i, c_p, c_i, c_i, c_p, c_i, c_p]),
+    "as_expand_image_f32": (c_i, [c_p, c_i, c_i, c_p, c_i, c_i, c_p, c_i, c_p, c_p]),
     "as_ref_features_f32": (c_i, [c_p, c_i, c_i, c_p, c_p, c_i, c_i, c_p, c_p, c_i, c_p]),
     "as_crop_f32": (c_i, [c_p, c_i, c_p, c_i, c_p, c_i, c_p, c_i, c_i, c_i, c_p]),
     "as_rows_to_images_f32": (c_i, [c_p, c_i, c_p, c_i, c_i, c_p, c_p, c_i, c_i, c_p]),
+    "as_style_cuts_f32": (c_i, [c_p, c_i, c_i, c_p, c_i, c_p, c_p, c_i, c_i, c_p, c_p, c_p, c_i, c_i, c_p, c_p, c_p, c_i, c_i, c_i, c_p]),
     "as_stem_pool_image_f32": (c_i, [c_p, c_p, c_p, c_i, c_p, c_p, c_i, c_i, c_p, c_i, c_p, c_i, c_i, c_i, c_i, c_p, c_i, c_p]),
     "as_dwconv_down_f32": (c_i, [c_p, c_i, c_p, c_p, c_i, c_p, c_i, c_p, c_p, c_i, c_p, c_p, c_i, c_i, c_i, c_i, c_i, c_p]),
     "as_frame_signal_f32": (c_i, [c_p, c_p, c_p, c_i, c_i, c_i, c_i, c_p, c_i, c_p]),
@@ -92,6 +95,7 @@
     "as_avgpool_down_image_f32": (c_i, [c_p, c_i, c_p, c_p, c_i, c_p, c_i, c_p, c_p, c_i, c_i, c_p, c_i, c_i, c_i, c_i, c_p, c_i, c_i, c_p]),
     "as_im2col_valid_image_f32": (c_i, [c_p, c_i, c_p, c_p, c_p, c_p, c_i, c_i, c_i, c_i, c_i, c_p, c_p]),
     "as_mean_pool_f32": (c_i, [c_p, c_i, c_p, c_i, c_i, c_i, c_p, c_i, c_p]),
+    "as_pool_linear_f32": (c_i, [c_p, c_i, c_p, c_i, c_i, c_i, c_p, c_p, c_i, c_p, c_i, c_p]),
     "as_relpos_attention_f32": (c_i, [c_p, c_i, c_i, c_i, c_i, c_p, c_p, c_p, c_i, c_i, c_p, c_i, c_p]),
     "as_relpos_attention_image_f32": (c_i, [c_p, c_i, c_p, c_i, c_i, c_i, c_i, c_p, c_p, c_p, c_p, c_i, c_p, c_i, c_i, c_p, c_i, c_p, c_p]),
     "as_relpos_attention_image_lds_bytes": (c_i, [c_i]),
@@ -166,6 +170,7 @@
 _pB, _pIO = ctypes.POINTER(Batch), ctypes.POINTER(ForwardIO)
 _SIGNATURES.update({
     "as_adain_image_f32": (c_i, [ctypes.POINTER(AdainArgs), c_p]),
+    "as_adain_image_sets_f32": (c_i, [ctypes.POINTER(AdainArgs), c_i, c_p]),
     "as_conv_gemm_multi_post_f32": (c_i, [ctypes.POINTER(ConvGemmArgs), ctypes.POINTER(AdainArgs), ctypes.POINTER(ctypes.c_int32),
                                           ctypes.POINTER(LnArgs), c_i, c_p]),
     "as_down_multi_f32": (c_i, [ctypes.POINTER(DownArgs), c_i, c_p]),
diff --git a/artspeech_amd/csrc/conv_gemm_h3.hip b/artspeech_amd/csrc/conv_gemm_h3.hip
--- a/artspeech_amd/csrc/conv_gemm_h3.hip
+++ b/artspeech_amd/csrc/conv_gemm_h3.hip
@@ -505,7 +505,7 @@
 
 template <bool UP>
 __global__ void __launch_bounds__(256)
-adain_image_kernel(const AsAdainArgs a)
+adain_image_kernel(const AsAdainArgs a, const int pool_u)
 {
     const int lane = threadIdx.x & 63, wave = __builtin_amdgcn_readfirstlane(threadIdx.x >> 6);
     const int kb = blockIdx.x * 2 + (wave >> 1), kh = wave & 1, u = blockIdx.y;
@@ -521,12 +521,15 @@
     const size_t gbase = a.gb_off ? (size_t)a.gb_off[u] : (size_t)u * a.ldgb;
     const int c0 = kb * 16 + kh * 8;
     float g1[8], bt[8], w0[8], w1[8], w2[8], pb[8];
+    const int set = (UP && pool_u > 0) ? u / pool_u : 0;
+    const float* pool_w = UP ? a.pool_w + (size_t)set * C * 3 : nullptr;
+    const float* pool_b = UP ? a.pool_b + (size_t)set * C : nullptr;
 #pragma unroll
     for (int r = 0; r < 8; ++r) {
         const int c = c0 + r < C ? c0 + r : C - 1;
         g1[r] = 1.0f + a.gb[gbase + (size_t)c * a.gb_sc];
         bt[r] = a.gb[gbase + (size_t)(C + c) * a.gb_sc];
-        if (UP) { w0[r] = a.pool_w[c * 3 + 0]; w1[r] = a.pool_w[c * 3 + 1]; w2[r] = a.pool_w[c * 3 + 2]; pb[r] = a.pool_b[c]; }
+        if (UP) { w0[r] = pool_w[c * 3 + 0]; w1[r] = pool_w[c * 3 + 1]; w2[r] = pool_w[c * 3 + 2]; pb[r] = pool_b[c]; }
     }
     const float* xr0 = a.x + s0;
     const size_t at0 = plane + (UP ? 2 * (size_t)o0 : (size_t)o0);
@@ -698,19 +701,25 @@
     }
 }
 
-extern "C" int as_adain_image_f32(const AsAdainArgs* args_host, as_stream_t stream)
+extern "C" int as_adain_image_sets_f32(const AsAdainArgs* args_host, int pool_u, as_stream_t stream)
 {
     if (!args_host) return AS_EINVAL;
     const AsAdainArgs& a = *args_host;
     if (!a.x || !a.gb || !a.col_off || !a.yh || a.C <= 0 || a.U <= 0 || a.N < 0 || a.gb_sc <= 0 || (!a.gb_off && a.ldgb <= 0)) return AS_EINVAL;
     if ((a.pool_w == nullptr) != (a.pool_b == nullptr) || (a.x_up && !a.pool_w)) return AS_EINVAL;
+    if (pool_u < 0 || (pool_u > 0 && !a.pool_w)) return AS_EINVAL;
     if ((reinterpret_cast<uintptr_t>(a.yh) & 15) != 0) return AS_EINVAL;
     if (a.N == 0) return AS_OK;
     AsProfScope prof__(AS_CLS_ADAIN, 0, 8.0 * a.C * (double)a.N, (hipStream_t)stream);
-    if (a.pool_w) hipLaunchKernelGGL(adain_image_kernel<true>, dim3(as_kbx(a.C) / 2, a.U), dim3(256), 0, (hipStream_t)stream, a);
-    else hipLaunchKernelGGL(adain_image_kernel<false>, dim3(as_kbx(a.C) / 2, a.U), dim3(256), 0, (hipStream_t)stream, a);
+    if (a.pool_w) hipLaunchKernelGGL(adain_image_kernel<true>, dim3(as_kbx(a.C) / 2, a.U), dim3(256), 0, (hipStream_t)stream, a, pool_u);
+    else hipLaunchKernelGGL(adain_image_kernel<false>, dim3(as_kbx(a.C) / 2, a.U), dim3(256), 0, (hipStream_t)stream, a, 0);
     AS_CHECK_LAUNCH();
     return AS_OK;
+}
+
+extern "C" int as_adain_image_f32(const AsAdainArgs* args_host, as_stream_t stream)
+{
+    return as_adain_image_sets_f32(args_host, 0, stream);
 }
 
 extern "C" int as_adain_split_f32(const float* x, int ldx, int C, const float* gamma_beta, int ldgb, const int32_t* col_off, int B,
diff --git a/artspeech_amd/csrc/elementwise.hip b/artspeech_amd/csrc/elementwise.hip
--- a/artspeech_amd/csrc/elementwise.hip
+++ b/artspeech_amd/csrc/elementwise.hip
@@ -54,17 +54,84 @@
     y[(size_t)c * ldy + j] = e[(size_t)t * C + c] * scale;
 }
 
+__global__ void __launch_bounds__(256)
+embed_image_kernel(const int* __restrict__ tok, int n_tok, const float* __restrict__ emb, const float* __restrict__ emb2, int n_split, int C,
+                   int N, int V, float scale, float* __restrict__ y, int ldy, u32x4_t* __restrict__ yh, unsigned* __restrict__ status, int vec)
+{
+    const int wcol = (blockIdx.x * 256 + (threadIdx.x & ~63)) * 4;
+    const int col = wcol + (threadIdx.x & 63);
+    const int g = blockIdx.y;
+    if (wcol > N) return;
+    const float* e[4];
+#pragma unroll
+    for (int c = 0; c < 4; ++c) {
+        const int j = min(col + 64 * c, N - 1);
+        const int grp = emb2 ? j / n_split : 0;
+        const int src = j - grp * n_split;
+        int t = src < n_tok ? tok[src] : 0;
+        if ((t < 0 || t >= V) && g == 0 && col + 64 * c < N) as_status_raise(status, AS_STATUS_BAD_TOKEN);
+        t = t < 0 ? 0 : (t >= V ? V - 1 : t);
+        e[c] = emb + (ptrdiff_t)grp * (emb2 - emb) + (size_t)t * C;
+    }
+    float v[4][8];
+    if (vec) {
+#pragma unroll
+        for (int c = 0; c < 4; ++c)
+#pragma unroll
+            for (int h = 0; h < 2; ++h) {
+                const int k = g * 8 + 4 * h;
+                const bool ok = k < C && col + 64 * c < N;
+                const float4 q = ok ? *reinterpret_cast<const float4*>(e[c] + k) : make_float4(0.f, 0.f, 0.f, 0.f);
+                v[c][4 * h + 0] = ok ? q.x * scale : 0.f; v[c][4 * h + 1] = ok ? q.y * scale : 0.f;
+                v[c][4 * h + 2] = ok ? q.z * scale : 0.f; v[c][4 * h + 3] = ok ? q.w * scale : 0.f;
+            }
+    } else {
+#pragma unroll
+        for (int c = 0; c < 4; ++c)
+#pragma unroll
+            for (int r = 0; r < 8; ++r) {
+                const int k = g * 8 + r;
+                v[c][r] = (k < C && col + 64 * c < N) ? e[c][k] * scale : 0.f;
+            }
+    }
+    const size_t NX = operand_image::rows(N);
+    const size_t base = operand_image::row(g, 0, col, NX);
+#pragma unroll
+    for (int c = 0; c < 4; ++c) {
+        const int j = col + 64 * c;
+        if (j > N) break;
+        if (j < N) {
+#pragma unroll
+            for (int r = 0; r < 8; ++r)
+                if (g * 8 + r < C) y[(size_t)(g * 8 + r) * ldy + j] = v[c][r];
+        }
+        oi_store(yh, base + 64 * c, NX, v[c]);
+    }
+}
+
+extern "C" int as_embed_groups_image_f32(const int32_t* tokens, int n_tok, const float* emb, const float* emb2, int n_split, int C, int N, int V,
+                                         float scale, float* y, int ldy, uint16_t* yh, as_stream_t stream)
+{
+    if (!tokens || !emb || !y || C <= 0 || N < 0 || V <= 0 || ldy < N || n_tok < 0 || n_tok > N) return AS_EINVAL;
+    if ((emb2 && n_split <= 0) || (n_tok < N && (!emb2 || n_split < n_tok))) return AS_EINVAL;
+    if ((reinterpret_cast<uintptr_t>(yh) & 15) != 0) return AS_EINVAL;
+    if (N == 0) return AS_OK;
+    AsProfScope prof__(AS_FILE_CLS, 0, 0, (hipStream_t)stream);
+    const int vec = (C & 3) == 0 && ((reinterpret_cast<uintptr_t>(emb) | reinterpret_cast<uintptr_t>(emb2)) & 15) == 0;
+    if (yh)
+        hipLaunchKernelGGL(embed_image_kernel, dim3(as_cdiv(N + 1, 1024), 2 * as_kbx(C)), dim3(256), 0, (hipStream_t)stream, tokens, n_tok, emb,
+                           emb2, n_split, C, N, V, scale, y, ldy, reinterpret_cast<u32x4_t*>(yh), as_status_words_device(), vec);
+    else
+        hipLaunchKernelGGL(embed_kernel, dim3(as_cdiv(N, 64), C), dim3(64), 0, (hipStream_t)stream, tokens, n_tok, emb, emb2, n_split, C, N, V,
+                           scale, y, ldy, as_status_words_device());
+    AS_CHECK_LAUNCH();
+    return AS_OK;
+}
+
 extern "C" int as_embed_groups_f32(const int32_t* tokens, int n_tok, const float* emb, const float* emb2, int n_split, int C, int N, int V,
                                    float scale, float* y, int ldy, as_stream_t stream)
 {
-    if (!tokens || !emb || !y || C <= 0 || N < 0 || V <= 0 || ldy < N || n_tok < 0 || n_tok > N) return AS_EINVAL;
-    if ((emb2 && n_split <= 0) || (n_tok < N && (!emb2 || n_split < n_tok))) return AS_EINVAL;
-    if (N == 0) return AS_OK;
-    AsProfScope prof__(AS_FILE_CLS, 0, 0, (hipStream_t)stream);
-    hipLaunchKernelGGL(embed_kernel, dim3(as_cdiv(N, 64), C), dim3(64), 0, (hipStream_t)stream, tokens, n_tok, emb, emb2, n_split, C, N, V,
-                       scale, y, ldy, as_status_words_device());
-    AS_CHECK_LAUNCH();
-    return AS_OK;
+    return as_embed_groups_image_f32(tokens, n_tok, emb, emb2, n_split, C, N, V, scale, y, ldy, nullptr, stream);
 }
 
 extern "C" int as_embed_f32(const int32_t* tokens, const float* emb, int C, int N, int V, float scale, float* y,
@@ -531,16 +598,63 @@
     y[(size_t)c * ldy + j] = x[(size_t)c * ldx + tok_of_frame[j / rep]];
 }
 
+__global__ void __launch_bounds__(256)
+expand_image_kernel(const float* __restrict__ x, int ldx, int C, const int* __restrict__ tok_of_frame, int N, int rep, float* __restrict__ y,
+                    int ldy, u32x4_t* __restrict__ yh)
+{
+    const int wcol = (blockIdx.x * 256 + (threadIdx.x & ~63)) * 4;
+    const int col = wcol + (threadIdx.x & 63);
+    const int g = blockIdx.y;
+    if (wcol > N) return;
+    int t[4];
+#pragma unroll
+    for (int c = 0; c < 4; ++c) t[c] = tok_of_frame[min(col + 64 * c, N - 1) / rep];
+    float v[4][8];
+#pragma unroll
+    for (int c = 0; c < 4; ++c)
+#pragma unroll
+        for (int r = 0; r < 8; ++r) {
+            const int k = g * 8 + r;
+            v[c][r] = (k < C && col + 64 * c < N) ? x[(size_t)k * ldx + t[c]] : 0.f;
+        }
+    const size_t NX = operand_image::rows(N);
+    const size_t base = operand_image::row(g, 0, col, NX);
+#pragma unroll
+    for (int c = 0; c < 4; ++c) {
+        const int j = col + 64 * c;
+        if (j > N) break;
+        if (j < N) {
+#pragma unroll
+            for (int r = 0; r < 8; ++r)
+                if (g * 8 + r < C) y[(size_t)(g * 8 + r) * ldy + j] = v[c][r];
+        }
+        oi_store(yh, base + 64 * c, NX, v[c]);
+    }
+}
+
+extern "C" int as_expand_image_f32(const float* x, int ldx, int C, const int32_t* tok_of_frame, int n_frames, int repeat, float* y, int ldy,
+                                   uint16_t* yh, as_stream_t stream)
+{
+    if (!x || !y || !tok_of_frame || C <= 0 || n_frames < 0 || repeat < 1 || (double)n_frames * repeat > 2147483647.0 - 1024.0 ||
+        ldy < n_frames * repeat)
+        return AS_EINVAL;
+    if ((reinterpret_cast<uintptr_t>(yh) & 15) != 0) return AS_EINVAL;
+    if (n_frames == 0) return AS_OK;
+    AsProfScope prof__(AS_FILE_CLS, 0, 0, (hipStream_t)stream);
+    if (yh)
+        hipLaunchKernelGGL(expand_image_kernel, dim3(as_cdiv((long)n_frames * repeat + 1, 1024), 2 * as_kbx(C)), dim3(256), 0, (hipStream_t)stream,
+                           x, ldx, C, tok_of_frame, n_frames * repeat, repeat, y, ldy, reinterpret_cast<u32x4_t*>(yh));
+    else
+        hipLaunchKernelGGL(expand_kernel, dim3(as_cdiv((long)n_frames * repeat, 256), C), dim3(256), 0, (hipStream_t)stream,
+                           x, ldx, C, tok_of_frame, n_frames, repeat, y, ldy);
+    AS_CHECK_LAUNCH();
+    return AS_OK;
+}
+
 extern "C" int as_expand_f32(const float* x, int ldx, int C, const int32_t* tok_of_frame, int n_frames, int repeat,
                              float* y, int ldy, as_stream_t stream)
 {
-    if (!x || !y || !tok_of_frame || C <= 0 || n_frames < 0 || repeat < 1 || ldy < n_frames * repeat) return AS_EINVAL;
-    if (n_frames == 0) return AS_OK;
-    AsProfScope prof__(AS_FILE_CLS, 0, 0, (hipStream_t)stream);
-    hipLaunchKernelGGL(expand_kernel, dim3(as_cdiv((long)n_frames * repeat, 256), C), dim3(256), 0, (hipStream_t)stream,
-                       x, ldx, C, tok_of_frame, n_frames, repeat, y, ldy);
-    AS_CHECK_LAUNCH();
-    return AS_OK;
+    return as_expand_image_f32(x, ldx, C, tok_of_frame, n_frames, repeat, y, ldy, nullptr, stream);
 }
 
 __global__ void __launch_bounds__(256)
@@ -598,13 +712,18 @@
     return AS_OK;
 }
 
-__global__ void crop_kernel(const float* __restrict__ src, int lds, const int* __restrict__ src_off, int start,
-                            float* __restrict__ dst, int ldd, const int* __restrict__ dst_off, int C)
-{
-    const int b = blockIdx.y, c = blockIdx.z;
+static __device__ __forceinline__ void crop_body(const float* __restrict__ src, int lds, const int* __restrict__ src_off, int start,
+                                                 float* __restrict__ dst, int ldd, const int* __restrict__ dst_off, int b, int c)
+{
     const int L = dst_off[b + 1] - dst_off[b];
     for (int i = blockIdx.x * blockDim.x + threadIdx.x; i < L; i += gridDim.x * blockDim.x)
         dst[(size_t)c * ldd + dst_off[b] + i] = src[(size_t)c * lds + src_off[b] + start + i];
+}
+
+__global__ void crop_kernel(const float* __restrict__ src, int lds, const int* __restrict__ src_off, int start,
+                            float* __restrict__ dst, int ldd, const int* __restrict__ dst_off, int C)
+{
+    crop_body(src, lds, src_off, start, dst, ldd, dst_off, blockIdx.y, blockIdx.z);
 }
 
 extern "C" int as_crop_f32(const float* src, int lds, const int32_t* src_off, int start, float* dst, int ldd,
@@ -619,13 +738,18 @@
     return AS_OK;
 }
 
-__global__ void rows_to_images_kernel(const float* __restrict__ src, int lds, const int* __restrict__ src_off, int start,
-                                      float* __restrict__ dst, const int* __restrict__ img_off, int H)
-{
-    const int b = blockIdx.y, h = blockIdx.z;
+static __device__ __forceinline__ void rows_to_images_body(const float* __restrict__ src, int lds, const int* __restrict__ src_off, int start,
+                                                           float* __restrict__ dst, const int* __restrict__ img_off, int H, int b, int h)
+{
     const int Wb = (img_off[b + 1] - img_off[b]) / H;
     for (int i = blockIdx.x * blockDim.x + threadIdx.x; i < Wb; i += gridDim.x * blockDim.x)
         dst[(size_t)img_off[b] + (size_t)h * Wb + i] = src[(size_t)h * lds + src_off[b] + start + i];
+}
+
+__global__ void rows_to_images_kernel(const float* __restrict__ src, int lds, const int* __restrict__ src_off, int start,
+                                      float* __restrict__ dst, const int* __restrict__ img_off, int H)
+{
+    rows_to_images_body(src, lds, src_off, start, dst, img_off, H, blockIdx.y, blockIdx.z);
 }
 
 extern "C" int as_rows_to_images_f32(const float* src, int lds, const int32_t* src_off, int start, int H, float* dst,
@@ -636,6 +760,32 @@
     AsProfScope prof__(AS_FILE_CLS, 0, 0, (hipStream_t)stream);
     hipLaunchKernelGGL(rows_to_images_kernel, dim3(as_cdiv(max_w, 256), B, H), dim3(256), 0, (hipStream_t)stream, src, lds,
                        src_off, start, dst, img_off, H);
+    AS_CHECK_LAUNCH();
+    return AS_OK;
+}
+
+__global__ void style_cuts_kernel(const float* __restrict__ rows, int ldr, int C, float* __restrict__ crop, int ldc, const int* __restrict__ crop_off,
+                                  const float* __restrict__ src1, int ld1, int H1, float* __restrict__ img1, const int* __restrict__ off1,
+                                  const float* __restrict__ src2, int ld2, int H2, float* __restrict__ img2, const int* __restrict__ off2,
+                                  const int* __restrict__ src_off, int start)
+{
+    const int b = blockIdx.y, z = blockIdx.z;
+    if (z < C) crop_body(rows, ldr, src_off, start, crop, ldc, crop_off, b, z);
+    else if (z < C + H1) rows_to_images_body(src1, ld1, src_off, start, img1, off1, H1, b, z - C);
+    else rows_to_images_body(src2, ld2, src_off, start, img2, off2, H2, b, z - C - H1);
+}
+
+extern "C" int as_style_cuts_f32(const float* rows, int ldr, int C, float* crop, int ldc, const int32_t* crop_off, const float* src1, int ld1,
+                                 int H1, float* img1, const int32_t* off1, const float* src2, int ld2, int H2, float* img2,
+                                 const int32_t* off2, const int32_t* src_off, int start, int B, int max_w, as_stream_t stream)
+{
+    if (!rows || !crop || !crop_off || !src1 || !img1 || !off1 || !src2 || !img2 || !off2 || !src_off || B < 0 || C <= 0 || H1 <= 0 ||
+        H2 <= 0 || C + H1 + H2 > 65535)
+        return AS_EINVAL;
+    if (B == 0 || max_w <= 0) return AS_OK;
+    AsProfScope prof__(AS_FILE_CLS, 0, 0, (hipStream_t)stream);
+    hipLaunchKernelGGL(style_cuts_kernel, dim3(as_cdiv(max_w, 256), B, C + H1 + H2), dim3(256), 0, (hipStream_t)stream, rows, ldr, C, crop, ldc,
+                       crop_off, src1, ld1, H1, img1, off1, src2, ld2, H2, img2, off2, src_off, start);
     AS_CHECK_LAUNCH();
     return AS_OK;
 }
@@ -1313,6 +1463,107 @@
     return AS_OK;
 }
 
+#define PL_THREADS 512
+#define PL_WAVES (PL_THREADS / 64)
+#define PL_MAX_K 4096
+#define PL_CH 16
+#define PL_OUT 4
+template <int KR>
+__global__ void __launch_bounds__(PL_THREADS)
+pool_linear_kernel(const float* __restrict__ x, int ldx, const int* __restrict__ col_off, int act, const float* __restrict__ w,
+                   const float* __restrict__ bias, int M, int K, int m_per_wg, float* __restrict__ y, int ldy)
+{
+    __shared__ __attribute__((aligned(16))) float pooled[PL_MAX_K];
+    const int lane = threadIdx.x & 63, wave = threadIdx.x >> 6;
+    const int b = blockIdx.x;
+    const int o0 = col_off[b], L = col_off[b + 1] - o0;
+    for (int k0 = wave * PL_CH; k0 < K; k0 += PL_WAVES * PL_CH) {
+        float s[PL_CH];
+#pragma unroll
+        for (int u = 0; u < PL_CH; ++u) s[u] = 0.f;
+        for (int i = lane; i - lane < L; i += 64) {
+            float v[PL_CH];
+#pragma unroll
+            for (int u = 0; u < PL_CH; ++u) {
+                const int k = min(k0 + u, K - 1);
+                v[u] = i < L ? x[(size_t)k * ldx + o0 + i] : 0.f;
+            }
+#pragma unroll
+            for (int u = 0; u < PL_CH; ++u) s[u] += act ? lrelu02(v[u]) : v[u];
+        }
+        float mine = 0.f;
+#pragma unroll
+        for (int u = 0; u < PL_CH; ++u) {
+            const float t = as_wave_sum(s[u]);
+            mine = lane == u ? t : mine;
+        }
+        if (lane < PL_CH && k0 + lane < K) pooled[k0 + lane] = mine / (float)L;
+    }
+    __syncthreads();
+    const int m_beg = blockIdx.y * m_per_wg, m_end = min(M, m_beg + m_per_wg);
+    for (int m0 = m_beg + wave * PL_OUT; m0 < m_end; m0 += PL_WAVES * PL_OUT) {
+        float s[PL_OUT];
+        if constexpr (KR > 0) {
+            const int nq = K >> 2;
+            float4 wq[PL_OUT][KR], pv[KR];
+#pragma unroll
+            for (int o = 0; o < PL_OUT; ++o) {
+                const float4* wr = reinterpret_cast<const float4*>(w + (size_t)min(m0 + o, M - 1) * K);
+#pragma unroll
+                for (int c = 0; c < KR; ++c) {
+                    const int q = lane + 64 * c;
+                    wq[o][c] = q < nq ? wr[q] : make_float4(0.f, 0.f, 0.f, 0.f);
+                }
+            }
+#pragma unroll
+            for (int c = 0; c < KR; ++c) {
+                const int q = lane + 64 * c;
+                pv[c] = reinterpret_cast<const float4*>(pooled)[q < nq ? q : 0];
+            }
+#pragma unroll
+            for (int o = 0; o < PL_OUT; ++o) {
+                s[o] = 0.f;
+#pragma unroll
+                for (int c = 0; c < KR; ++c) s[o] += wq[o][c].x * pv[c].x + wq[o][c].y * pv[c].y + wq[o][c].z * pv[c].z + wq[o][c].w * pv[c].w;
+            }
+        } else {
+#pragma unroll
+            for (int o = 0; o < PL_OUT; ++o) {
+                const float* wr = w + (size_t)min(m0 + o, M - 1) * K;
+                s[o] = 0.f;
+                for (int k = lane; k < K; k += 64) s[o] += wr[k] * pooled[k];
+            }
+        }
+#pragma unroll
+        for (int o = 0; o < PL_OUT; ++o) {
+            const float t = as_wave_sum(s[o]);
+            if (lane == 0 && m0 + o < m_end) y[(size_t)b * ldy + m0 + o] = t + (bias ? bias[m0 + o] : 0.f);
+        }
+    }
+}
+
+extern "C" int as_pool_linear_f32(const float* x, int ldx, const int32_t* col_off, int B, int K, int lrelu, const float* w, const float* bias,
+                                  int M, float* y, int ldy, as_stream_t stream)
+{
+    if (!x || !col_off || !w || !y || B < 0 || K <= 0 || K > PL_MAX_K || M <= 0 || ldy < M) return AS_EINVAL;
+    if (B == 0) return AS_OK;
+    AsProfScope prof__(AS_FILE_CLS, 0, 0, (hipStream_t)stream);
+    const int mb = std::max(1, std::min(as_cdiv(256, B), as_cdiv(M, PL_WAVES * PL_OUT)));
+    const int m_per_wg = as_cdiv(M, mb);
+    const dim3 grid(B, as_cdiv(M, m_per_wg)), block(PL_THREADS);
+    hipStream_t s_ = (hipStream_t)stream;
+    const bool vec = (K & 3) == 0 && (reinterpret_cast<uintptr_t>(w) & 15) == 0;
+#define PL_LAUNCH(KR) hipLaunchKernelGGL(pool_linear_kernel<KR>, grid, block, 0, s_, x, ldx, col_off, lrelu, w, bias, M, K, m_per_wg, y, ldy)
+    if (!vec || K > 2048) PL_LAUNCH(0);
+    else if (K <= 256) PL_LAUNCH(1);
+    else if (K <= 512) PL_LAUNCH(2);
+    else if (K <= 1024) PL_LAUNCH(4);
+    else PL_LAUNCH(8);
+#undef PL_LAUNCH
+    AS_CHECK_LAUNCH();
+    return AS_OK;
+}
+
 __global__ void __launch_bounds__(256)
 dyn_geometry_kernel(const AsDynGeo g)
 {
diff --git a/artspeech_amd/csrc/model.hip b/artspeech_amd/csrc/model.hip
--- a/artspeech_amd/csrc/model.hip
+++ b/artspeech_amd/csrc/model.hip
@@ -892,10 +892,12 @@
         return s0;
     };
     float* x = c.f32((size_t)C * ld);
+    uint16_t* x_img = c.records() ? c.image(C, lays[G]->N) : nullptr;
     {
         const float* e2 = nullptr;
         const float* e1 = stack2(".emb.weight", G, &e2);
-        if (lays[G]->N > 0) RUN(c, as_embed_groups_f32(tokens, N1, e1, e2, gc, C, lays[G]->N, V, sqrtf((float)C), x, ld, c.s));
+        if (lays[G]->N > 0)
+            RUN(c, as_embed_groups_image_f32(tokens, N1, e1, e2, gc, C, lays[G]->N, V, sqrtf((float)C), x, ld, x_img, c.s));
     }
     auto ln_image = [&](const float* xin, const std::string& ln, bool relu, int k) {
         const int N = lays[k]->N;
@@ -929,7 +931,8 @@
     {
         ConvOpt q0 = opt(".pre.conv_layers.0", G);
         xs_next = ln_post(q0, ".pre.norm_layers.0", true, G);
-        conv_x(c, cw(".pre.conv_layers.0", G), x, ld, C, lays[G], k5, h, ld, q0);
+        if (c.records()) conv_h(c, cw(".pre.conv_layers.0", G), x_img, C, lays[G], k5, h, ld, q0);
+        else conv_x(c, cw(".pre.conv_layers.0", G), x, ld, C, lays[G], k5, h, ld, q0);
         for (int i = 0; i < 3; ++i) {
             uint16_t* xs = xs_next;
             const std::string nxt = i < 2 ? ".pre.conv_layers." + std::to_string(i + 1) : std::string(".pre.proj");
@@ -1180,12 +1183,11 @@
     for (int a = 0; a < K; ++a)
         for (int d = 0; d < K; ++d) { tv.dh[a * K + d] = a; tv.dw[a * K + d] = d; }
     float* z = conv_h_new(c, wl, x.h, C, lout, tv, o2);
-    float* pooled = c.f32((size_t)lay->B * wl->M);
-    RUN(c, as_mean_pool_f32(z, lout->N, lout->d_off, lay->B, wl->M, 0, pooled, wl->M, c.s));
     const HostT* lw = m.host(linear + ".weight");
     if (!lw) return;
+    if (lw->dim(1) != wl->M) { c.fail(AS_EINVAL); return; }
     const float *lww = m.vec(linear + ".weight"), *lwb = m.vec(linear + ".bias");
-    RUN(c, as_linear_rows_f32(pooled, wl->M, lww, lwb, lay->B, lw->dim(0), lw->dim(1), y, ldy, c.s));
+    RUN(c, as_pool_linear_f32(z, lout->N, lout->d_off, lay->B, wl->M, 0, lww, lwb, lw->dim(0), y, ldy, c.s));
 }
 
 void tower1d(Ctx& c, const std::string& p, const float* X, int ldx, const Lay* lay, const std::string& linear, float* y, int ldy)
@@ -1198,12 +1200,11 @@
         x = resblk_down(c, p + "." + std::to_string(i), x, false, true, i < 4);
         if (!x.lay) return;
     }
-    float* pooled = c.f32((size_t)lay->B * x.C);
-    RUN(c, as_mean_pool_f32(x.p, x.ld, x.lay->d_off, lay->B, x.C, 1, pooled, x.C, c.s));
     const HostT* lw = m.host(linear + ".weight");
     if (!lw) return;
+    if (lw->dim(1) != x.C) { c.fail(AS_EINVAL); return; }
     const float *lww = m.vec(linear + ".weight"), *lwb = m.vec(linear + ".bias");
-    RUN(c, as_linear_rows_f32(pooled, x.C, lww, lwb, lay->B, lw->dim(0), lw->dim(1), y, ldy, c.s));
+    RUN(c, as_pool_linear_f32(x.p, x.ld, x.lay->d_off, lay->B, x.C, 1, lww, lwb, lw->dim(0), y, ldy, c.s));
 }
 
 struct StyleIn {
@@ -1224,11 +1225,10 @@
     if (!s.l1 || !s.lm || !s.le) return s;
     const int N1 = std::max(s.l1->N, 1);
     s.crop = c.f32((size_t)2 * N1);
-    RUN(c, as_crop_f32(feat12, ldf, ref->d_off, 0, s.crop, s.l1->N, s.l1->d_off, ref->B, 2, s.l1->max_cols(), c.s));
     s.mel_img = c.f32((size_t)std::max(s.lm->N, 1));
     s.ema_img = c.f32((size_t)std::max(s.le->N, 1));
-    RUN(c, as_rows_to_images_f32(mel, ldm, ref->d_off, 0, n_mels, s.mel_img, s.lm->d_off, ref->B, s.l1->max_cols(), c.s));
-    RUN(c, as_rows_to_images_f32(feat12 + (size_t)2 * ldf, ldf, ref->d_off, 0, 10, s.ema_img, s.le->d_off, ref->B, s.l1->max_cols(), c.s));
+    RUN(c, as_style_cuts_f32(feat12, ldf, 2, s.crop, s.l1->N, s.l1->d_off, mel, ldm, n_mels, s.mel_img, s.lm->d_off,
+                             feat12 + (size_t)2 * ldf, ldf, 10, s.ema_img, s.le->d_off, ref->d_off, 0, ref->B, s.l1->max_cols(), c.s));
     return s;
 }
 
@@ -1378,17 +1378,18 @@
         uint16_t* xs = c.image(C, NG2);
         float* up = c.f32((size_t)C * Nn);
         const Norm n1 = gnorm(0, ".norm1", C);
-        for (int g = 0; g < 3; ++g) {
-            const float *pw = m.vec(nm[g] + ".pool.weight"), *pb = m.vec(nm[g] + ".pool.bias");
-            if (!c.go() || NG2 == 0) continue;
+        const HostT* pwh = m.host(nm[0] + ".pool.weight");
+        const float *pw = m.vec_stack(sfx(".pool.weight")), *pb = m.vec_stack(sfx(".pool.bias"));
+        if (!pwh || (int)pwh->v.size() != C * 3) { c.fail(AS_EINVAL); return; }
+        if (c.go() && NG2 > 0) {
             AsAdainArgs q;
             memset(&q, 0, sizeof(q));
             q.x = a.p; q.ldx = a.ld; q.C = C;
-            q.gb = n1.gb; q.gb_off = n1.gb_off + g * B; q.ldgb = 1; q.gb_sc = n1.gb_sc;
-            q.col_off = layG1->d_off + g * B; q.src_off = src_off + g * B; q.U = B; q.N = NG2; q.lrelu = 1; q.yh = xs;
-            q.col_w = layG1->dyn ? layG1->d_w + g * B : nullptr;
+            q.gb = n1.gb; q.gb_off = n1.gb_off; q.ldgb = 1; q.gb_sc = n1.gb_sc;
+            q.col_off = layG1->d_off; q.src_off = src_off; q.U = 3 * B; q.N = NG2; q.lrelu = 1; q.yh = xs;
+            q.col_w = layG1->dyn ? layG1->d_w : nullptr;
             q.pool_w = pw; q.pool_b = pb; q.x_up = up; q.ld_up = NG2;
-            RUN(c, as_adain_image_f32(&q, c.s));
+            RUN(c, as_adain_image_sets_f32(&q, B, c.s));
         }
         ConvOpt q1;
         q1.bias = m.bias_stack(sfx(".conv1"));
@@ -1484,7 +1485,7 @@
     float* catb = nullptr;
     bool ok = false;
 };
-DecPre decoder_pre(Ctx& c, float* x0, const Lay* lay2)
+DecPre decoder_pre(Ctx& c, const float* t_en, int ld_en, const int32_t* tof, int n_frames, float* x0, const Lay* lay2)
 {
     const as_model& m = c.m;
     const std::string p = "decoder";
@@ -1496,7 +1497,8 @@
     d.catb = c.f32((size_t)cat * Nn2);
     d.cath = c.image(cat, N2);
     d.cath2 = c.image(cat, N2);
-    RUN(c, as_split_f16x2_f32(x0, N2, C, N2, 0, 0.f, d.x0h, c.s));
+    if (2 * n_frames != N2) { c.fail(AS_EINVAL); return d; }
+    RUN(c, as_expand_image_f32(t_en, ld_en, C, tof, n_frames, 2, x0, N2, d.x0h, c.s));
     ConvOpt q;
     q.bias = m.bias(p + ".asr_res.0");
     q.want_yh = true;
@@ -1770,9 +1772,8 @@
 DecPre text_half(Ctx& c, const PhaseA& A, const int32_t* tof, int N1, float* x0, const Lay* lay2)
 {
     const int C = c.m.cfg.hidden_dim, N2 = lay2->N;
-    c.hint(0, 4.0 * C * ((double)A.tok->N + N2));
-    RUN(c, as_expand_f32(A.t_en, A.ld_en, C, tof, N1, 2, x0, N2, c.s));
-    return decoder_pre(c, x0, lay2);
+    c.hint(0, 4.0 * C * ((double)A.tok->N + 2.0 * N2));
+    return decoder_pre(c, A.t_en, A.ld_en, tof, N1, x0, lay2);
 }
 
 void seg_scatter(Ctx& c, const as_segments* segs, const float* src, int ld_src, int rows, const int32_t* frame_off, int B)
@@ -1955,11 +1956,10 @@
     }
     const int C = c.m.cfg.hidden_dim, N2 = lay2->N, sd2 = 2 * c.m.cfg.style_dim;
     float* x0 = c.f32((size_t)(C + 128) * std::max(N2, 1));
-    RUN(c, as_expand_f32(asr, lda, C, ident, lay->N, 2, x0, N2, c.s));
     float* fne = c.f32((size_t)12 * std::max(N2, 1));
     track_rows(c, Tracks::FromCaller, fne, N2, F0, N, EMA, ldp);
     const FcOut fc = adain_fc_all(c, "style", style_norms(c.m), style, sd2, sd2, batch->B);
-    decoder(c, decoder_pre(c, x0, lay2), x0, lay2, fne, N2, fc, mel, ldo);
+    decoder(c, decoder_pre(c, asr, lda, ident, lay->N, x0, lay2), x0, lay2, fne, N2, fc, mel, ldo);
     return AS_OK;
 }
 
diff --git a/artspeech_amd/ops.py b/artspeech_amd/ops.py
--- a/artspeech_amd/ops.py
+++ b/artspeech_amd/ops.py
@@ -199,7 +199,7 @@
 
 
 def adain_image(X, lay, gb, gb_sc, N_out, ldgb=1, gb_off=None, src_off=None, pool_w=None, pool_b=None, x_up=None, col_w=None, col_off=None,
-                out=None):
+                out=None, pool_u=0):
     C = X.shape[0]
     xs = new_image(C, N_out, X.device) if out is None else out
     a = _lib.AdainArgs()
@@ -209,7 +209,10 @@
     a.col_off, a.src_off, a.U, a.N, a.lrelu, a.yh = _p(lay.col_off if col_off is None else col_off), _p(src_off), U, N_out, 1, _p(xs)
     a.pool_w, a.pool_b, a.x_up, a.ld_up = _p(pool_w), _p(pool_b), _p(x_up), (_ld(x_up) if x_up is not None else 0)
     a.col_w = _p(col_w)
-    check(_lib.lib().as_adain_image_f32(ctypes.byref(a), stream()), "as_adain_image_f32")
+    if pool_u:
+        check(_lib.lib().as_adain_image_sets_f32(ctypes.byref(a), pool_u, stream()), "as_adain_image_sets_f32")
+    else:
+        check(_lib.lib().as_adain_image_f32(ctypes.byref(a), stream()), "as_adain_image_f32")
     return xs
 
 
@@ -316,12 +319,12 @@
     check(_lib.lib().as_conv_gemm_multi_post_f32(arr, pa, mw, la, n, stream()), "as_conv_gemm_multi_post_f32")
 
 
-def embed(tokens_i32, emb, scale, Y, group2=None, n_cols=None):
+def embed(tokens_i32, emb, scale, Y, group2=None, n_cols=None, image=None):
     V, C = emb.shape
     emb2, n_split = group2 if group2 is not None else (None, 0)
     n_tok = tokens_i32.numel()
-    check(_lib.lib().as_embed_groups_f32(_p(tokens_i32), n_tok, _p(emb), _p(emb2), n_split, C, n_tok if n_cols is None else n_cols, V, scale,
-                                         _p(Y), _ld(Y), stream()), "as_embed_groups_f32")
+    check(_lib.lib().as_embed_groups_image_f32(_p(tokens_i32), n_tok, _p(emb), _p(emb2), n_split, C, n_tok if n_cols is None else n_cols, V,
+                                               scale, _p(Y), _ld(Y), _p(image), stream()), "as_embed_groups_image_f32")
     return Y
 
 
@@ -360,9 +363,9 @@
     return dur_i, frame_off, tof
 
 
-def expand(X, tok_of_frame, n_frames, repeat, Y):
-    check(_lib.lib().as_expand_f32(_p(X), _ld(X), X.shape[0], _p(tok_of_frame), n_frames, repeat, _p(Y), _ld(Y), stream()),
-          "as_expand_f32")
+def expand(X, tok_of_frame, n_frames, repeat, Y, image=None):
+    check(_lib.lib().as_expand_image_f32(_p(X), _ld(X), X.shape[0], _p(tok_of_frame), n_frames, repeat, _p(Y), _ld(Y), _p(image), stream()),
+          "as_expand_image_f32")
     return Y
 
 
@@ -390,6 +393,15 @@
     check(_lib.lib().as_rows_to_images_f32(_p(src), _ld(src), _p(src_lay.col_off), start, H, _p(dst), _p(img_lay.col_off),
                                            img_lay.B, src_lay.max_cols, stream()), "as_rows_to_images_f32")
     return dst
+
+
+def style_cuts(rows, crop, crop_lay, src1, img1_lay, src2, img2_lay, src_lay, start=0):
+    img1, img2 = img1_lay.new(1), img2_lay.new(1)
+    check(_lib.lib().as_style_cuts_f32(_p(rows), _ld(rows), rows.shape[0], _p(crop), _ld(crop), _p(crop_lay.col_off), _p(src1), _ld(src1),
+                                       src1.shape[0], _p(img1), _p(img1_lay.col_off), _p(src2), _ld(src2), src2.shape[0], _p(img2),
+                                       _p(img2_lay.col_off), _p(src_lay.col_off), start, crop_lay.B, crop_lay.max_cols, stream()),
+          "as_style_cuts_f32")
+    return crop, img1, img2
 
 
 def interleave_phases(Z, bias, C, u, n_in, Y):
@@ -528,6 +540,15 @@
     return y
 
 
+def pool_linear(X, lay, lrelu, w, bias, y=None):
+    K, M = X.shape[0], w.shape[0]
+    if y is None:
+        y = torch.empty((lay.B, M), dtype=torch.float32, device=X.device)
+    check(_lib.lib().as_pool_linear_f32(_p(X), _ld(X), _p(lay.col_off), lay.B, K, int(lrelu), _p(w), _p(bias), M, _p(y), _ld(y), stream()),
+          "as_pool_linear_f32")
+    return y
+
+
 def channel_layernorm_split(X, lay, gamma, beta, relu=False, eps=1e-4, group2=None, out=None):
     L = _lib.lib()
     C = X.shape[0]
diff --git a/include/artspeech_hip.h b/include/artspeech_hip.h
--- a/include/artspeech_hip.h
+++ b/include/artspeech_hip.h
@@ -103,6 +103,8 @@
                  as_stream_t stream);
 int as_embed_groups_f32(const int32_t* tokens, int n_tok, const float* emb, const float* emb2, int n_split, int C, int N, int V,
                         float scale, float* y, int ldy, as_stream_t stream);
+int as_embed_groups_image_f32(const int32_t* tokens, int n_tok, const float* emb, const float* emb2, int n_split, int C, int N, int V,
+                              float scale, float* y, int ldy, uint16_t* yh, as_stream_t stream);
 int as_channel_layernorm_groups_f32(const float* x, int ldx, int C, int N, const float* gamma, const float* beta, const float* gamma2,
                                     const float* beta2, int n_split, float eps, int relu, float* y, int ldy, as_stream_t stream);
 int as_channel_layernorm_split_f32(const float* x, int ldx, int C, int N, const float* gamma, const float* beta, const float* gamma2,
@@ -140,6 +142,7 @@
     const int32_t* col_w;
 } AsAdainArgs;
 int as_adain_image_f32(const AsAdainArgs* args_host, as_stream_t stream);
+int as_adain_image_sets_f32(const AsAdainArgs* args_host, int pool_u, as_stream_t stream);
 typedef struct AsLnArgs {
     const float *gamma, *beta, *gamma2, *beta2;
     int32_t n_split;
@@ -160,12 +163,17 @@
                      int32_t* frame_off, int32_t* tok_of_frame, int max_frames, as_stream_t stream);
 int as_expand_f32(const float* x, int ldx, int C, const int32_t* tok_of_frame, int n_frames, int repeat, float* y,
                   int ldy, as_stream_t stream);
+int as_expand_image_f32(const float* x, int ldx, int C, const int32_t* tok_of_frame, int n_frames, int repeat, float* y,
+                        int ldy, uint16_t* yh, as_stream_t stream);
 int as_ref_features_f32(const float* mel, int ldm, int n_mels, const float* f0_raw, const float* ema_raw, int lde,
                         int N, const float* stats24, float* feat, int ldf, as_stream_t stream);
 int as_crop_f32(const float* src, int lds, const int32_t* src_off, int start, float* dst, int ldd,
                 const int32_t* dst_off, int B, int C, int max_len, as_stream_t stream);
 int as_rows_to_images_f32(const float* src, int lds, const int32_t* src_off, int start, int H, float* dst,
                           const int32_t* img_off, int B, int max_w, as_stream_t stream);
+int as_style_cuts_f32(const float* rows, int ldr, int C, float* crop, int ldc, const int32_t* crop_off, const float* src1, int ld1,
+                      int H1, float* img1, const int32_t* off1, const float* src2, int ld2, int H2, float* img2,
+                      const int32_t* off2, const int32_t* src_off, int start, int B, int max_w, as_stream_t stream);
 int as_dwconv_down_f32(const float* x, int ldx, const int32_t* in_off, const int32_t* in_w, int Hin, float* y, int ldy,
                        const int32_t* out_off, const int32_t* out_w, int Hout, const float* w, const float* bias,
                        int kh, int B, int C, int max_out, int lrelu, as_stream_t stream);
@@ -205,6 +213,8 @@
                               const int32_t* out_w, int K, int stride, int lrelu, int B, int C, uint16_t* yh, as_stream_t stream);
 int as_mean_pool_f32(const float* x, int ldx, const int32_t* col_off, int B, int C, int lrelu, float* y, int ldy,
                      as_stream_t stream);
+int as_pool_linear_f32(const float* x, int ldx, const int32_t* col_off, int B, int K, int lrelu, const float* w, const float* bias,
+                       int M, float* y, int ldy, as_stream_t stream);
 
 int as_frame_signal_f32(const float* wave, const int32_t* wav_off, const int32_t* frame_off, int B, int max_frames, int n_fft, int hop,
                         float* X, int ldx, as_stream_t stream);
```

New measurement: 1.832 million, median of 6. No clear change (+0.6%).
